# zhangyp15/MonoFlex

Measured on AMD Instinct MI355X. Metric: images/sec at 1280x384, DLA-34+DCNv2 forward+decode, higher is better.
Workload: dtype bf16; 1 GPU; DLA-34+DCNv2+9 heads+edge fusion forward + NMS/top-K/3D decode, batch 8 per GPU, 1280x384, bf16 (BASELINE.json configs[1]); batch_per_gpu=8, launch=hipGraph, parallelism=replicas x1 (no collective on the inference path), sub_batch_streams=1, detections_last_step=400, h2d_excluded=True, d2h_excluded=True

## Files before the change

### include/monoflex_hip.h

```cpp
#ifndef MONOFLEX_HIP_H
#define MONOFLEX_HIP_H

#include <stddef.h>
#include <stdint.h>

#ifdef __cplusplus
extern "C" {
#endif

#define MFX_ABI_VERSION 3

enum { MFX_F32 = 0, MFX_BF16 = 1, MFX_F16 = 2 ,
       MFX_F16X2 = 3  };
enum { MFX_ACT_NONE = 0, MFX_ACT_RELU = 1, MFX_ACT_LEAKY = 2 , MFX_ACT_DCN_OFFMASK = 3  };
enum { MFX_OK = 0, MFX_ERR_ARG = -1, MFX_ERR_UNSUPPORTED = -2, MFX_ERR_LAUNCH = -3, MFX_ERR_WORKSPACE = -4 };

int mfx_abi_version(void);
const char* mfx_last_error(void);
int mfx_set_option(const char* name, int value);
int mfx_reset_options(void);
int mfx_commit_options(void);
long mfx_get_counter(const char* name);

int mfx_f16x2_range_check(int reset);


size_t mfx_dcn_v2_workspace_bytes(int B, int C, int H, int W, int Cout, int kh, int kw,
                                  int stride_h, int stride_w, int pad_h, int pad_w, int dil_h, int dil_w,
                                  int backward);
size_t mfx_dcn_v2_workspace_bytes_g(int B, int C, int H, int W, int Cout, int kh, int kw,
                                    int stride_h, int stride_w, int pad_h, int pad_w, int dil_h, int dil_w,
                                    int deformable_group, int backward);

int mfx_dcn_v2_forward(const float* input, const float* weight, const float* bias,
                       const float* offset, const float* mask, float* output,
                       int B, int C, int H, int W, int Cout, int kh, int kw,
                       int stride_h, int stride_w, int pad_h, int pad_w, int dil_h, int dil_w,
                       int deformable_group, void* workspace, size_t workspace_bytes, void* stream);

int mfx_dcn_v2_backward(const float* input, const float* weight, const float* bias,
                        const float* offset, const float* mask, const float* grad_output,
                        float* grad_input, float* grad_offset, float* grad_mask,
                        float* grad_weight, float* grad_bias,
                        int B, int C, int H, int W, int Cout, int kh, int kw,
                        int stride_h, int stride_w, int pad_h, int pad_w, int dil_h, int dil_w,
                        int deformable_group, void* workspace, size_t workspace_bytes, void* stream);

int mfx_dcn_v2_psroi_pooling_forward(const float* input, const float* bbox, const float* trans, float* output, float* output_count,
                                     int B, int C, int H, int W, int N, int trans_rois, int trans_channels,
                                     int no_trans, float spatial_scale, int output_dim, int group_size, int pooled_size, int part_size,
                                     int sample_per_part, float trans_std, void* stream);

int mfx_dcn_v2_psroi_pooling_backward(const float* out_grad, const float* input, const float* bbox, const float* trans, const float* top_count,
                                      float* grad_input, float* grad_trans,
                                      int B, int C, int H, int W, int N, int trans_rois, int trans_channels,
                                      int no_trans, float spatial_scale, int output_dim, int group_size, int pooled_size, int part_size,
                                      int sample_per_part, float trans_std, void* stream);


#define MFX_MAX_SEG 9

typedef struct {
    const void* x;
    const void* w;
    const void* w_frag;
    const float* scale;
    const float* shift;
    const void* res;
    void* y;
    const int32_t* rowmap;
    int32_t B, H, W;
    int32_t x_pixstride;
    int32_t Ck;
    int32_t kh, kw, stride, pad_h, pad_w, dil_w;
    int32_t Ho, Wo;
    int32_t M;
    int32_t Cout;
    int32_t Cout_pad;
    int32_t K_pad;
    int32_t ldy, ldres;
    int32_t act;
    int32_t dtype, out_dtype;
    void* workspace;
    int64_t workspace_bytes;
    float* stats;
    int stats_ncopy;
    int* stats_done;
    const void* w_frag_pair;
} mfx_conv_desc;
int mfx_conv2d_nhwc(const mfx_conv_desc* d, void* stream);

typedef struct {
    const void* src[MFX_MAX_SEG];
    int32_t stride[MFX_MAX_SEG];
    int32_t off[MFX_MAX_SEG];
    int32_t nseg, Cseg;
    const void* w; const float* scale; const float* shift; const void* res; void* y;
    int32_t M, Cout, Cout_pad, K_pad, ldy, ldres, act, dtype;
} mfx_cat_desc;
int mfx_cat_conv1x1_nhwc(const mfx_cat_desc* d, void* stream);

typedef struct {
    const void* x; const float* offmask; const void* w; const float* scale; const float* shift; void* y;
    const void* w_frag;
    int32_t B, H, W, C;
    int32_t kh, kw, stride, pad, dil;
    int32_t Ho, Wo, Cout, Cout_pad, K_pad, ldy, act, dtype;
    const void* w_frag_f16;
    void* workspace;
    int64_t workspace_bytes;
    const void* off_w_frag_f16;
    const float* off_shift;
    float* offmask_out;
    int32_t nonsquare, stride_w, pad_w, dil_w;
    const void* w_pair_f16;
} mfx_dcn_desc;
int mfx_dcn_nhwc(const mfx_dcn_desc* d, void* stream);
int mfx_dcn_fuses_offset_conv(const mfx_dcn_desc* d);
int mfx_dcn_module_group(const mfx_conv_desc* off, const mfx_dcn_desc* dcn, int n, void* stream);

int mfx_dcn_sample_nhwc(const void* P, const float* offmask, const float* scale, const float* shift, void* y,
                        int B, int H, int W, int N, int ldy, int act, int dtype, void* stream);
int mfx_project_nhwc(const void* x, const void* w, void* y, int M, int K, int N, int ldx, int ldy, int dtype, void* stream);

int mfx_stem_conv7x7_nchw(const float* images, const void* w, const float* scale, const float* shift, void* y,
                          int B, int H, int W, int Cout, int K_pad, int act, int dtype, void* stream);

int mfx_f1_fused(const float* images, const void* w_stem, const float* sc_stem, const float* sh_stem,
                 const void* w_l0, const float* sc_l0, const float* sh_l0, const void* w_l1, const float* sc_l1, const float* sh_l1,
                 void* y, int B, int H, int W, int stem_kpad , int dtype, void* stream);

int mfx_maxpool2x2_nhwc(const void* x, void* y, int B, int H, int W, int C, int dtype, void* stream);

int mfx_upsample_add_nhwc(const void* x, const float* w, const void* skip, void* y,
                          int B, int H, int W, int C, int f, int dtype, void* stream);

int mfx_nchw_to_nhwc(const float* x, void* y, int B, int C, int H, int W, int ldy, int dtype, void* stream);
int mfx_nhwc_to_nchw(const void* x, float* y, int B, int C, int H, int W, int ldx, int dtype, void* stream);
int mfx_pack_image_nhwc4(const float* x, void* y, int B, int H, int W, int pad_h, int pad_w_left, int pad_w_right,
                         int dtype, void* stream);

typedef struct {
    const void* x;
    const void* w1;
    const float* scale1; const float* shift1;
    const void* w2;
    const float* bias2;
    float* out;
    float* planar;
    int32_t B, H, W, nbranch, K_pad, ld_out, dtype, planar_c;
    int32_t ch_off[16]; int32_t c_out[16];
    float w2_scale[16];
    const void* w1_32; const void* w2_32;
} mfx_heads_desc;
int mfx_heads_fused(const mfx_heads_desc* d, void* stream);
int mfx_heads_fused_act(const mfx_heads_desc* d, int act, void* stream);

int mfx_edge_scatter_add(float* out, int ld_out, int ch_off, int C, const float* v, int ldv,
                         const int32_t* edge_xy, const int32_t* edge_len, int B, int L, int H, int W,
                         float* planar , void* stream);

typedef struct {
    const void* x;
    const int32_t* edge_xy;
    const void* w_trunk;
    const float* scale_trunk; const float* shift_trunk;
    const void* w_conv;
    const float* scale_conv; const float* shift_conv;
    const void* w_out;
    const float* bias_out;
    float* out;
    int32_t B, H, W, C, L, head_conv, ksize, relu , dtype;
} mfx_edge_chain_desc;
int mfx_edge_chain(const mfx_edge_chain_desc* d, void* stream);
int mfx_edge_chain_act(const mfx_edge_chain_desc* d, int act, void* stream);
int mfx_edge_chain_applies(const mfx_edge_chain_desc* d);
int mfx_edge_chain_ks(const mfx_edge_chain_desc* d, int act, void* stream);
int mfx_edge_chain_ks_applies(const mfx_edge_chain_desc* d);

size_t mfx_decode_topk_workspace_bytes(int ncls, int B, int K);
int mfx_decode_topk(const float* hmap, long b_stride, long c_stride, long p_stride, int ncls, int B, int H, int W, int K,
                    float* scores, int32_t* index, void* workspace, size_t workspace_bytes, void* stream);

int mfx_decode_boxes(const float* hmap, int ld, int reg_off, const float* scores, const int32_t* index,
                     int ncls, int B, int H, int W, int K, const float* calib, const int32_t* pad,
                     const int32_t* img_size, float threshold, float* det, float* topk, int32_t* valid,
                     void* stream);
enum { MFX_DEPTH_SOFT = 0, MFX_DEPTH_HARD = 1, MFX_DEPTH_MEAN = 2, MFX_DEPTH_DIRECT = 3, MFX_DEPTH_KEYPOINTS_AVG = 4,
       MFX_DEPTH_KEYPOINTS_CENTER = 5, MFX_DEPTH_KEYPOINTS_02 = 6, MFX_DEPTH_KEYPOINTS_13 = 7 };
int mfx_decode_boxes_mode(const float* hmap, int ld, int reg_off, const float* scores, const int32_t* index,
                          int ncls, int B, int H, int W, int K, const float* calib, const int32_t* pad,
                          const int32_t* img_size, float threshold, int depth_mode, float* det, float* topk, int32_t* valid,
                          void* stream);
typedef struct mfx_decode_cfg {
    float dim_mean[9], dim_std[9];
    float depth_ref[2], depth_range[2];
    float down_ratio, eps;
    int depth_decode;
    int dim_exp, dim_use_std;
    int uncertainty_as_conf;
    int output_depth;
} mfx_decode_cfg;
int mfx_decode_boxes_cfg(const float* hmap, int ld, int reg_off, const float* scores, const int32_t* index,
                         int ncls, int B, int H, int W, int K, const float* calib, const int32_t* pad,
                         const int32_t* img_size, float threshold, const mfx_decode_cfg* cfg, float* det, float* topk, int32_t* valid,
                         float* unc, void* stream);
typedef struct mfx_head_layout {
    int ch[9];
    int reg_width;
} mfx_head_layout;
int mfx_decode_boxes_heads(const float* hmap, int ld, int reg_off, const float* scores, const int32_t* index,
                           int ncls, int B, int H, int W, int K, const float* calib, const int32_t* pad,
                           const int32_t* img_size, float threshold, const mfx_decode_cfg* cfg, const mfx_head_layout* heads,
                           float* det, float* topk, int32_t* valid, float* unc, void* stream);
enum { MFX_DEPTH_ORACLE = 8 };
int mfx_decode_boxes_multi(const float* hmap, int ld, int reg_off, const float* scores, const int32_t* index,
                           int ncls, int B, int H, int W, int K, const float* calib, const int32_t* pad,
                           const int32_t* img_size, float threshold, const mfx_decode_cfg* cfg, const mfx_head_layout* heads,
                           uint32_t modes, const float* gt_rows, int M, float* det, float* topk, int32_t* valid, float* unc,
                           int32_t* oracle_choice, void* stream);


int mfx_conv_wgrad_nhwc(const void* x, const void* dy, float* dw, int B, int H, int W, int x_pixstride, int Ck,
                        int kh, int kw, int stride, int pad_h, int pad_w, int Ho, int Wo, int Cout, int ldy,
                        int dtype, void* stream);
int mfx_conv_wgrad_nhwc_dil(const void* x, const void* dy, float* dw, int B, int H, int W, int x_pixstride, int Ck,
                            int kh, int kw, int stride, int pad_h, int pad_w, int dil_w, int Ho, int Wo, int Cout, int ldy,
                            int dtype, void* stream);
int mfx_conv_wgrad_oihw(const void* x, const void* dy, float* dw, int B, int H, int W, int x_pixstride, int Ck,
                        int kh, int kw, int stride, int pad_h, int pad_w, int Ho, int Wo, int Cout, int ldy,
                        int Cout_real, int Cin_real, int dtype, void* workspace, size_t workspace_bytes, void* stream);
int mfx_stem_wgrad_bf16(const void* xp, const void* dy, float* dw, int B, int H, int W, int Hp, int Wp, void* workspace,
                        size_t workspace_bytes, void* stream);
int mfx_stem_wgrad_16(const void* xp, const void* dy, float* dw, int B, int H, int W, int Hp, int Wp, int dtype, void* workspace,
                      size_t workspace_bytes, void* stream);
int mfx_pack_conv_weight(const float* w_oihw, int Cout, int Cin, int kh, int kw, int mode, void* packed, void* frag,
                         int rows_pad, int K_pad, int ck, int dtype, void* stream);
int mfx_pack_chunk_elems(void);
typedef struct mfx_pack_desc {
    const float* w;
    void* packed;
    void* frag;
    int Cout, Cin, kh, kw, mode, rows_pad, K_pad, ck;
} mfx_pack_desc;
int mfx_pack_conv_weights_batched(const mfx_pack_desc* descs_dev, const long long* prefix_dev, int n, long long total_chunks,
                                  int dtype, void* stream);
typedef struct mfx_adamw_desc {
    void* p;
    const void* g;
    void* m;
    void* v;
    float* step;
    long long numel;
    int group;
    int pad_;
} mfx_adamw_desc;
typedef struct mfx_adamw_group {
    const float* lr;
    float beta1, beta2, eps, weight_decay;
} mfx_adamw_group;
int mfx_adamw_chunk_elems(void);
int mfx_adamw_multi(const mfx_adamw_desc* descs_dev, const long long* prefix_dev, int n, long long total_chunks,
                    const mfx_adamw_group* groups_dev, const float* found_inf, void* stream);
#define MFX_OPTIM_ADAMW 0
#define MFX_OPTIM_ADAM_L2 1
int mfx_optim_multi(const mfx_adamw_desc* descs_dev, const long long* prefix_dev, int n, long long total_chunks,
                    const mfx_adamw_group* groups_dev, int rule, const float* grad_coef, const float* found_inf, void* stream);
#define MFX_OPTIM_ADAM_TRUE_WD 2
int mfx_optim_multi_sched(const mfx_adamw_desc* descs_dev, const long long* prefix_dev, int n, long long total_chunks,
                          const mfx_adamw_group* groups_dev, const float* const* beta1_dev, int rule, const float* grad_coef, const float* found_inf,
                          void* stream);
size_t mfx_grad_norm_workspace_bytes(long long total_chunks);
// ... 226 lines not shown
```

### monoflex_amd/csrc/dcn_lds.hip

```cpp
#include "../../include/monoflex_hip.h"
#include "err.h"
#include "internal.h"
#include "igemm.h"
#include "dcn_sample_math.h"

namespace mfx {

struct DcnLGeom { int B, H, W, C, tiles_x, tiles_y, nslice, fsteps_pair, fsteps_far, cpt_far; };
struct DcnLOffArgs { const u32x4* wfm; const float* shift; float* om_out; };

typedef _Float16 lh2_t __attribute__((ext_vector_type(2)));
typedef _Float16 lh8_t __attribute__((ext_vector_type(8)));

__device__ __forceinline__ uint32_t l_bf2_to_h2(uint32_t d) {
    return __builtin_bit_cast(uint32_t, __builtin_amdgcn_cvt_pkrtz(__uint_as_float(d << 16), __uint_as_float(d & 0xffff0000u)));
}
template <typename TX> __device__ __forceinline__ u32x4 l_to_h8(const u32x4& v);
template <> __device__ __forceinline__ u32x4 l_to_h8<bf16_t>(const u32x4& v) { return u32x4{l_bf2_to_h2(v.x), l_bf2_to_h2(v.y), l_bf2_to_h2(v.z), l_bf2_to_h2(v.w)}; }
template <> __device__ __forceinline__ u32x4 l_to_h8<half_t>(const u32x4& v) { return v; }

#ifdef MFX_PROBES
__device__ unsigned long long mfx_dcn_lds_probe[1024 * 4 * 16];
#define LPROBE(k) do { if (lane == 0 && blockIdx.x < 1024) mfx_dcn_lds_probe[(blockIdx.x * 4 + wv) * 16 + (k)] = (unsigned long long)clock64(); } while (0)
#else
#define LPROBE(k) do { } while (0)
#endif

template <int R, int TR> struct DcnLSmem {
    static constexpr int PW = 16 + 2 * (R + 1), PH = TR + 2 * (R + 1);
    static constexpr int PB = 48;
    static constexpr int patch_bytes = PW * PH * PB;
    static constexpr int NPIX = TR * 16;
    static constexpr int NG = 9 * NPIX;
    static constexpr int GW_OFF = patch_bytes;
    static constexpr int GB_OFF = GW_OFF + (NG + 64) * 8;
    static constexpr int bytes = GB_OFF + (NG + 64) * 4;
    static constexpr int ZBYTES = (TR + 2) * 18 * 144;
    static constexpr int TBUF_OFF = (ZBYTES + 4 * 2304 <= patch_bytes) ? ZBYTES : GB_OFF;
    static_assert(ZBYTES <= patch_bytes && (TBUF_OFF != GB_OFF || 4 * 2304 <= (NG + 64) * 4), "offset-conv scratch fits");
};

template <int R, int TR, typename TX, bool OF>
__global__ __launch_bounds__(256, TR == 8 ? 3 : 2) void dcn_lds_kernel(const TX* __restrict__ x, const float* __restrict__ om, const u32x4* __restrict__ wpair,
                                                        const u32x4* __restrict__ wfar, DcnLGeom g, EpiArgs ep, DcnLOffArgs oa) {
    using SM = DcnLSmem<R, TR>;
    constexpr int PW = SM::PW, PH = SM::PH, PB = SM::PB, FM = TR / 4, FN = 4, NPIX = SM::NPIX;
    constexpr int OWN = 4 / FM;
    constexpr int TPT = (9 + OWN - 1) / OWN;
    constexpr int ROWB = PW * PB;
    extern __shared__ __attribute__((aligned(16))) char smem[];
    const int tid = threadIdx.x, lane = tid & 63;
    const int wv = __builtin_amdgcn_readfirstlane(tid >> 6);
    const int xl = lane & 15, kq = lane >> 4;

    LPROBE(0);
    int tile = xcd_remap(blockIdx.x, gridDim.x);
    const int tx = tile % g.tiles_x; tile /= g.tiles_x;
    const int ty = tile % g.tiles_y, b = tile / g.tiles_y;
    const int ty0 = ty * TR, tx0 = tx * 16;
    const int py0 = ty0 - (R + 1), px0 = tx0 - (R + 1);
    const TX* xb = x + (size_t)b * g.H * g.W * g.C;
    const char* xbb = reinterpret_cast<const char*>(xb);

    const int oi = kq % FM, tg = kq / FM;
    const int opix = (wv * FM + oi) * 16 + xl;
    const int yo = ty0 + wv * FM + oi, xo = tx0 + xl;
    const bool own_ok = yo < g.H && xo < g.W;

    constexpr int PU = PW * PH * 2 / 256;
    static_assert(PW * PH * 2 % 256 == 0, "patch chunks per thread");
    uint32_t poff[PU]; uint32_t pin = 0;
#pragma unroll
    for (int u = 0; u < PU; ++u) {
        const int idx = u * 256 + tid, p = idx >> 1, col = idx & 1;
        const int ry = p / PW, rx = p - ry * PW;
        const int gy = py0 + ry, gx = px0 + rx;
        const bool in = gy >= 0 && gy < g.H && gx >= 0 && gx < g.W;
        const int cy = min(max(gy, 0), g.H - 1), cx = min(max(gx, 0), g.W - 1);
        poff[u] = (uint32_t)((cy * g.W + cx) * g.C + col * 8) * 2u;
        pin |= in ? (1u << u) : 0u;
    }
    const int pw_addr = (tid >> 1) * PB + (tid & 1) * 16;
    u32x4 pr[PU];
    auto patch_fetch = [&](int sl) {
#pragma unroll
        for (int u = 0; u < PU; ++u) pr[u] = *reinterpret_cast<const u32x4*>(xbb + poff[u] + (uint32_t)sl * 32u);
    };
    auto patch_write = [&]() {
#pragma unroll
        for (int u = 0; u < PU; ++u) {
            const u32x4 v = (pin >> u) & 1u ? pr[u] : u32x4{0u, 0u, 0u, 0u};
            *reinterpret_cast<u32x4*>(smem + pw_addr + u * (128 * PB)) = l_to_h8<TX>(v);
        }
    };

    float odh[TPT], odw[TPT], omk[TPT];
    const int tap0 = TPT * tg;
    if constexpr (!OF) {
        const float* r = om + ((size_t)(b * g.H + min(yo, g.H - 1)) * g.W + min(xo, g.W - 1)) * dcns::kRow;
#pragma unroll
        for (int tt = 0; tt < TPT; ++tt) {
            const int tap = min(tap0 + tt, 8);
            odh[tt] = r[dcns::off_h(tap)]; odw[tt] = r[dcns::off_w(tap)]; omk[tt] = r[dcns::mask_at(tap)];
        }
        patch_fetch(0);
    } else {
        constexpr int ZW = 18, ZPS = 144, TLD = 36;
        float* tbuf = reinterpret_cast<float*>(smem + SM::TBUF_OFF) + wv * (16 * TLD);
        {
            constexpr int ZN = (TR + 2) * ZW * 8, ZU = (ZN + 255) / 256;
#pragma unroll
            for (int base = 0; base < ZN; base += 256 * ZU) {
                u32x4 zr[ZU];
#pragma unroll
                for (int u = 0; u < ZU; ++u) {
                    int idx = base + u * 256 + tid;
                    if (base + u * 256 + 256 > ZN) idx = idx < ZN ? idx : ZN - 1;
                    const int p = idx >> 3, col = idx & 7;
                    const int ry = p / ZW, rx = p - ry * ZW;
                    const int gy = ty0 - 1 + ry, gx = tx0 - 1 + rx;
                    const bool in = gy >= 0 && gy < g.H && gx >= 0 && gx < g.W;
                    const int cy = min(max(gy, 0), g.H - 1), cx = min(max(gx, 0), g.W - 1);
                    const u32x4 v = *reinterpret_cast<const u32x4*>(xb + (uint32_t)((cy * g.W + cx) * g.C + col * 8));
                    zr[u] = in ? v : u32x4{0u, 0u, 0u, 0u};
                }
#pragma unroll
                for (int u = 0; u < ZU; ++u) {
                    const int idx = base + u * 256 + tid;
                    if (base + u * 256 + 256 <= ZN || idx < ZN) *reinterpret_cast<u32x4*>(smem + (idx >> 3) * ZPS + ((idx & 7) << 4)) = l_to_h8<TX>(zr[u]);
                }
            }
        }
        f32x4 ao[FM][2];
#pragma unroll
        for (int i = 0; i < FM; ++i) { ao[i][0] = f32x4{0.f, 0.f, 0.f, 0.f}; ao[i][1] = f32x4{0.f, 0.f, 0.f, 0.f}; }
        constexpr int OR = 6;
        u32x4 ow[OR][2];
        const u32x4* owl = oa.wfm + lane;
#pragma unroll
        for (int u = 0; u < OR - 1; ++u) { ow[u][0] = owl[(0 * 18 + u) * 64]; ow[u][1] = owl[(1 * 18 + u) * 64]; }
        patch_fetch(0);
        __syncthreads();
        LPROBE(1);
#pragma unroll
        for (int s_ = 0; s_ < 18; ++s_) {
            if (s_ + OR - 1 < 18) { ow[(s_ + OR - 1) % OR][0] = owl[(0 * 18 + s_ + OR - 1) * 64]; ow[(s_ + OR - 1) % OR][1] = owl[(1 * 18 + s_ + OR - 1) * 64]; }
            const int tap = s_ >> 1, th = tap / 3, tw = tap - th * 3;
            const char* ap = smem + ((wv * FM + th) * ZW + xl + tw) * ZPS + ((s_ & 1) * 32 + kq * 8) * 2;
#pragma unroll
            for (int i = 0; i < FM; ++i) {
                const u32x4 af = *reinterpret_cast<const u32x4*>(ap + i * ZW * ZPS);
#pragma unroll
                for (int j = 0; j < 2; ++j)
                    ao[i][j] = __builtin_amdgcn_mfma_f32_16x16x32_f16(__builtin_bit_cast(lh8_t, af), __builtin_bit_cast(lh8_t, ow[s_ % OR][j]), ao[i][j], 0, 0, 0);
            }
        }
        LPROBE(2);
        const float b0 = oa.shift[xl], b1 = oa.shift[16 + xl];
#pragma unroll
        for (int i = 0; i < FM; ++i) {
#pragma unroll
            for (int r = 0; r < 4; ++r) {
                float v0 = ao[i][0][r] + b0, v1 = ao[i][1][r] + b1;
                if (xl >= 2) v1 = 1.f / (1.f + __expf(-v1));
                tbuf[(kq * 4 + r) * TLD + xl] = v0;
                tbuf[(kq * 4 + r) * TLD + 16 + xl] = (xl < 11) ? v1 : 0.f;
            }
            __builtin_amdgcn_wave_barrier();
            if (oi == i) {
#pragma unroll
                for (int tt = 0; tt < TPT; ++tt) {
                    const int tap = min(tap0 + tt, 8);
                    const float2 d2 = *reinterpret_cast<const float2*>(tbuf + xl * TLD + dcns::off_h(tap));
                    odh[tt] = d2.x; odw[tt] = d2.y; omk[tt] = tbuf[xl * TLD + dcns::mask_at(tap)];
                }
                if (oa.om_out && own_ok && tg == 0) {
                    float* o = oa.om_out + ((size_t)(b * g.H + yo) * g.W + xo) * dcns::kRow;
#pragma unroll
                    for (int q = 0; q < 32; q += 4) *reinterpret_cast<f32x4*>(o + q) = *reinterpret_cast<const f32x4*>(tbuf + xl * TLD + q);
                }
            }
            __builtin_amdgcn_wave_barrier();
        }
    }

    LPROBE(3);
    uint32_t gb[TPT];
    unsigned long long farm[TPT];
#pragma unroll
    for (int tt = 0; tt < TPT; ++tt) {
        const int tap = tap0 + tt;
        const bool has = tap < 9;
        const float mk = (own_ok && has) ? omk[tt] : 0.f;
        const dcns::Tap t = dcns::tap3x3(tap);
        const float h = dcns::pos3x3(yo, t.th, odh[tt]), w = dcns::pos3x3(xo, t.tw, odw[tt]);
        const dcns::Sample s = dcns::sample(h, w);
        const float lh = s.lh, lw = s.lw, hh = s.hh, hw_ = s.hw;
        const int h0 = s.h0, w0 = s.w0;
        const float m_ = dcns::inside(h, w, g.H, g.W) ? mk : 0.f;
        uint32_t wa = __builtin_bit_cast(uint32_t, __builtin_amdgcn_cvt_pkrtz(hh * hw_ * m_, hh * lw * m_));
        uint32_t wb_ = __builtin_bit_cast(uint32_t, __builtin_amdgcn_cvt_pkrtz(lh * hw_ * m_, lh * lw * m_));
        const int ry = h0 - py0, rx = w0 - px0;
        const bool in_patch = ry >= 0 && ry + 1 < PH && rx >= 0 && rx + 1 < PW;
        const bool live = m_ != 0.f;
        const bool far = live && !in_patch;
        uint32_t base = in_patch ? (uint32_t)((ry * PW + rx) * PB) : 0u;
        if (far) { base = 0x80000000u | (uint32_t)(h0 + 32) | ((uint32_t)(w0 + 32) << 16); wa |= 0x80008000u; wb_ |= 0x80008000u; }
        if (!live) { wa = 0u; wb_ = 0u; }
        if (has) *reinterpret_cast<uint2*>(smem + SM::GW_OFF + (tap * NPIX + opix) * 8) = uint2{wa, wb_};
        gb[tt] = base;
        farm[tt] = __builtin_amdgcn_ballot_w64(far);
    }
    if (tid < 4) *reinterpret_cast<uint2*>(smem + SM::GW_OFF + (SM::NG + 16 * tid) * 8) = uint2{0u, 0u};
    LPROBE(4);
    __syncthreads();
    LPROBE(5);
#pragma unroll
    for (int tt = 0; tt < TPT; ++tt)
        if (tt + TPT * tg < 9) *reinterpret_cast<uint32_t*>(smem + SM::GB_OFF + ((tt + TPT * tg) * NPIX + opix) * 4) = gb[tt];
    if (tid < 4) *reinterpret_cast<uint32_t*>(smem + SM::GB_OFF + (SM::NG + 16 * tid) * 4) = 0u;
    patch_write();
    __syncthreads();
    LPROBE(6);

    f32x4 acc[FM][FN];
#pragma unroll
    for (int i = 0; i < FM; ++i)
#pragma unroll
        for (int j = 0; j < FN; ++j) acc[i][j] = f32x4{0.f, 0.f, 0.f, 0.f};

    const int gent = (kq >> 1) * NPIX + wv * (FM * 16) + xl;
    const int gw_a = SM::GW_OFF + gent * 8, gb_a = SM::GB_OFF + gent * 4;
    const int gw_z = (kq >> 1) ? SM::GW_OFF + (SM::NG - 8 * NPIX) * 8 : gw_a;
    const int gb_z = (kq >> 1) ? SM::GB_OFF + (SM::NG - 8 * NPIX) * 4 : gb_a;
    const int ccol = (kq & 1) * 16;
    const u32x4* wpl = wpair + lane;
    auto wfetch = [&](int step, u32x4 (&wf)[FN]) {
#pragma unroll
        for (int j = 0; j < FN; ++j) wf[j] = wpl[((size_t)j * g.fsteps_pair + step) * 64];
    };
    u32x4 wq[2][FN];
    wfetch(0, wq[0]);

    constexpr int NF = 5 * FM;
    for (int sl = 0; sl < g.nslice; ++sl) {
        if (sl + 1 < g.nslice) patch_fetch(sl + 1);
        uint2 gwv[3]; uint32_t gbv[3];
        u32x4 cv[2][4];
        auto geo_read = [&](int f, int slot) {
            const int j = f / FM, i = f % FM;
            if (j < 4) {
                gwv[slot] = *reinterpret_cast<const uint2*>(smem + gw_a + (2 * NPIX * j + 16 * i) * 8);
                gbv[slot] = *reinterpret_cast<const uint32_t*>(smem + gb_a + (2 * NPIX * j + 16 * i) * 4);
            } else {
                gwv[slot] = *reinterpret_cast<const uint2*>(smem + gw_z + (8 * NPIX + 16 * i) * 8);
                gbv[slot] = *reinterpret_cast<const uint32_t*>(smem + gb_z + (8 * NPIX + 16 * i) * 4);
            }
        };
        auto corner_read = [&](int slot_g, int slot_c) {
            const int base = max((int)gbv[slot_g], 0) + ccol;
            cv[slot_c][0] = *reinterpret_cast<const u32x4*>(smem + base);
            cv[slot_c][1] = *reinterpret_cast<const u32x4*>(smem + base + PB);
            cv[slot_c][2] = *reinterpret_cast<const u32x4*>(smem + base + ROWB);
            cv[slot_c][3] = *reinterpret_cast<const u32x4*>(smem + base + ROWB + PB);
        };
        auto blend = [&](int slot_g, int slot_c) -> u32x4 {
            typedef short ls2_t __attribute__((ext_vector_type(2)));
            const ls2_t z2 = {0, 0};
            const lh2_t wa = __builtin_bit_cast(lh2_t, __builtin_elementwise_max(__builtin_bit_cast(ls2_t, gwv[slot_g].x), z2));
            const lh2_t wb_ = __builtin_bit_cast(lh2_t, __builtin_elementwise_max(__builtin_bit_cast(ls2_t, gwv[slot_g].y), z2));
            const lh2_t w0 = {wa[0], wa[0]}, w1 = {wa[1], wa[1]}, w2 = {wb_[0], wb_[0]}, w3 = {wb_[1], wb_[1]};
            u32x4 o;
#pragma unroll
            for (int d = 0; d < 4; ++d) {
                const uint32_t a0 = cv[slot_c][0][d], a1 = cv[slot_c][1][d], a2 = cv[slot_c][2][d], a3 = cv[slot_c][3][d];
                const lh2_t r = __builtin_bit_cast(lh2_t, a0) * w0 + __builtin_bit_cast(lh2_t, a1) * w1 +
                                __builtin_bit_cast(lh2_t, a2) * w2 + __builtin_bit_cast(lh2_t, a3) * w3;
                o[d] = __builtin_bit_cast(uint32_t, r);
            }
            return o;
        };
        geo_read(0, 0);
        geo_read(1, 1);
        corner_read(0, 0);
#pragma unroll
        for (int f = 0; f < NF; ++f) {
            const int j = f / FM, i = f % FM;
            if (i == 0) {
                const int nstep = sl * 5 + j + 1;
                wfetch(min(nstep, g.fsteps_pair - 1), wq[(j + 1) & 1]);
            }
            if (f + 2 < NF) geo_read(f + 2, (f + 2) % 3);
            if (f + 1 < NF) corner_read((f + 1) % 3, (f + 1) & 1);
            __builtin_amdgcn_sched_barrier(0);
            const u32x4 af = blend(f % 3, f & 1);
#pragma unroll
            for (int n = 0; n < FN; ++n)
                acc[i][n] = __builtin_amdgcn_mfma_f32_16x16x32_f16(__builtin_bit_cast(lh8_t, af), __builtin_bit_cast(lh8_t, wq[j & 1][n]), acc[i][n], 0, 0, 0);
            __builtin_amdgcn_sched_barrier(0);
        }
#pragma unroll
        for (int n = 0; n < FN; ++n) wq[0][n] = wq[1][n];
        if (sl < 4) LPROBE(7 + 2 * sl);
        if (sl + 1 < g.nslice) {
            __syncthreads();
            patch_write();
            __syncthreads();
        }
        if (sl < 3) LPROBE(8 + 2 * sl);
    }

    __syncthreads();
    float sc[FN], sh[FN];
#pragma unroll
    for (int j = 0; j < FN; ++j) {
        sc[j] = ep.scale ? ep.scale[j * 16 + xl] : 1.f;
        sh[j] = ep.shift ? ep.shift[j * 16 + xl] : 0.f;
    }
    {
        unsigned long long any = 0;
#pragma unroll
        for (int tt = 0; tt < TPT; ++tt) any |= farm[tt];
        if (any) {
            const u32x4* wfl = wfar + lane;
            for (int tap = 0; tap < 9; ++tap) {
                const int ftt = tap % TPT, ftg = tap / TPT;
                unsigned long long fm_ = 0;
#pragma unroll
                for (int t = 0; t < TPT; ++t) fm_ = (t == ftt) ? farm[t] : fm_;
                fm_ >>= (ftg * FM) * 16;
                if (!(fm_ & (FM == 4 ? ~0ull : 0xffffffffull))) continue;
#pragma unroll
                for (int i = 0; i < FM; ++i) {
                    if (!((fm_ >> (16 * i)) & 0xffffull)) continue;
                    const int ent = tap * NPIX + (wv * FM + i) * 16 + xl;
                    const uint2 gw = *reinterpret_cast<const uint2*>(smem + SM::GW_OFF + ent * 8);
                    const uint32_t gbase = *reinterpret_cast<const uint32_t*>(smem + SM::GB_OFF + ent * 4);
                    const bool isfar = (gbase >> 31) != 0u;
                    const int h0 = (int)(gbase & 0xffffu) - 32, w0 = (int)((gbase >> 16) & 0x7fffu) - 32;
                    const uint32_t wau = isfar ? (gw.x & 0x7fff7fffu) : 0u, wbu = isfar ? (gw.y & 0x7fff7fffu) : 0u;
                    const lh2_t wa = __builtin_bit_cast(lh2_t, wau), wb_ = __builtin_bit_cast(lh2_t, wbu);
                    const lh2_t w0_ = {wa[0], wa[0]}, w1_ = {wa[1], wa[1]}, w2_ = {wb_[0], wb_[0]}, w3_ = {wb_[1], wb_[1]};
                    for (int ks = 0; ks < g.cpt_far; ++ks) {
                        u32x4 v[4];
#pragma unroll
                        for (int q = 0; q < 4; ++q) {
                            const int hc = h0 + (q >> 1), wc = w0 + (q & 1);
                            const bool ok = isfar && hc >= 0 && hc < g.H && wc >= 0 && wc < g.W;
                            v[q] = u32x4{0u, 0u, 0u, 0u};
                            if (ok) v[q] = l_to_h8<TX>(*reinterpret_cast<const u32x4*>(xb + ((size_t)hc * g.W + wc) * g.C + ks * 32 + kq * 8));
                        }
                        u32x4 af;
#pragma unroll
                        for (int d = 0; d < 4; ++d) {
                            const uint32_t a0 = v[0][d], a1 = v[1][d], a2 = v[2][d], a3 = v[3][d];
                            const lh2_t r = __builtin_bit_cast(lh2_t, a0) * w0_ + __builtin_bit_cast(lh2_t, a1) * w1_ +
                                            __builtin_bit_cast(lh2_t, a2) * w2_ + __builtin_bit_cast(lh2_t, a3) * w3_;
                            af[d] = __builtin_bit_cast(uint32_t, r);
                        }
#pragma unroll
                        for (int n = 0; n < FN; ++n) {
                            const u32x4 wf = wfl[((size_t)n * g.fsteps_far + tap * g.cpt_far + ks) * 64];
                            acc[i][n] = __builtin_amdgcn_mfma_f32_16x16x32_f16(__builtin_bit_cast(lh8_t, af), __builtin_bit_cast(lh8_t, wf), acc[i][n], 0, 0, 0);
                        }
                    }
                }
            }
        }
    }

    LPROBE(14);
    constexpr int LDS_ = FN * 16 + 4;
    constexpr int GPR = FN * 16 / 8;
    float* stage = reinterpret_cast<float*>(smem) + wv * (16 * LDS_);
    TX* y = reinterpret_cast<TX*>(ep.y);
#pragma unroll
    for (int i = 0; i < FM; ++i) {
#pragma unroll
        for (int j = 0; j < FN; ++j)
#pragma unroll
            for (int r = 0; r < 4; ++r) stage[(kq * 4 + r) * LDS_ + j * 16 + xl] = acc[i][j][r] * sc[j] + sh[j];
        __builtin_amdgcn_wave_barrier();
        const int yg = ty0 + wv * FM + i;
        for (int it = lane; it < 16 * GPR; it += 64) {
            const int px = it / GPR, ng = it - px * GPR;
            const int gx = tx0 + px, gn = ng * 8;
            if (yg < g.H && gx < g.W && gn < ep.Cout) {
                float v[8];
#pragma unroll
                for (int e = 0; e < 8; e += 4) {
                    const f32x4 t = *reinterpret_cast<const f32x4*>(stage + px * LDS_ + ng * 8 + e);
                    v[e] = t[0]; v[e + 1] = t[1]; v[e + 2] = t[2]; v[e + 3] = t[3];
                }
                apply_act_chunk<8>(v, ep.act, gn);
                *reinterpret_cast<u32x4*>(y + ((size_t)(b * g.H + yg) * g.W + gx) * ep.ldy + gn) = ElemTraits<TX>::pack(v);
            }
        }
        __builtin_amdgcn_wave_barrier();
    }
    LPROBE(15);
}

#ifdef MFX_PROBES
}
extern "C" int mfx_dcn_lds_probe_read(unsigned long long* host, int n) {
    return hipMemcpyFromSymbol(host, HIP_SYMBOL(mfx::mfx_dcn_lds_probe), sizeof(unsigned long long) * (size_t)n) == hipSuccess ? 0 : -1;
}
namespace mfx {
#endif

template <int R>
__global__ __launch_bounds__(256, 2) void dcn_lds_split_kernel(const float* __restrict__ x, const float* __restrict__ om, const u32x4* __restrict__ wpair,
                                                              const u32x4* __restrict__ wfar, size_t pair_lo, size_t far_lo, DcnLGeom g, EpiArgs ep) {
    constexpr int TR = 8, FM = 2, FN = 4, NPIX = TR * 16, OWN = 2, TPT = 5;
    constexpr int PW = 16 + 2 * (R + 1), PH = TR + 2 * (R + 1), PB = 80, ROWB = PW * PB;
    constexpr int patch_bytes = PW * PH * PB, NG = 9 * NPIX, GT_OFF = patch_bytes;
    extern __shared__ __attribute__((aligned(16))) char smem[];
    const int tid = threadIdx.x, lane = tid & 63;
    const int wv = __builtin_amdgcn_readfirstlane(tid >> 6);
    const int xl = lane & 15, kq = lane >> 4;

    int tile = xcd_remap(blockIdx.x, gridDim.x);
    const int tx = tile % g.tiles_x; tile /= g.tiles_x;
    const int ty = tile % g.tiles_y, b = tile / g.tiles_y;
    const int ty0 = ty * TR, tx0 = tx * 16;
    const int py0 = ty0 - (R + 1), px0 = tx0 - (R + 1);
    const float* xb = x + (size_t)b * g.H * g.W * g.C;
    const char* xbb = reinterpret_cast<const char*>(xb);

    const int oi = kq % FM, tg = kq / FM;
    const int opix = (wv * FM + oi) * 16 + xl;
    const int yo = ty0 + wv * FM + oi, xo = tx0 + xl;
    const bool own_ok = yo < g.H && xo < g.W;

    constexpr int PU = PW * PH * 4 / 256;
    static_assert(PW * PH * 4 % 256 == 0, "patch chunks per thread");
    auto patch_load = [&](int sl) {
#pragma unroll
        for (int half = 0; half < 2; ++half) {
            u32x4 pr[PU / 2];
#pragma unroll
            for (int u = 0; u < PU / 2; ++u) {
                const int idx = (half * (PU / 2) + u) * 256 + tid, p = idx >> 2, col = idx & 3;
                const int ry = p / PW, rx = p - ry * PW;
                const int gy = py0 + ry, gx = px0 + rx;
                const bool in = gy >= 0 && gy < g.H && gx >= 0 && gx < g.W;
                const int cy = min(max(gy, 0), g.H - 1), cx = min(max(gx, 0), g.W - 1);
                const u32x4 v = *reinterpret_cast<const u32x4*>(xbb + (uint32_t)(((cy * g.W + cx) * g.C + sl * 16 + col * 4) * 4));
                pr[u] = in ? v : u32x4{0u, 0u, 0u, 0u};
            }
#pragma unroll
            for (int u = 0; u < PU / 2; ++u) {
                const int idx = (half * (PU / 2) + u) * 256 + tid;
                *reinterpret_cast<u32x4*>(smem + (idx >> 2) * PB + (idx & 3) * 16) = pr[u];
            }
        }
    };

    {
        const float* r = om + ((size_t)(b * g.H + min(yo, g.H - 1)) * g.W + min(xo, g.W - 1)) * dcns::kRow;
        const int tap0 = TPT * tg;
        float odh[TPT], odw[TPT], omk[TPT];
#pragma unroll
        for (int tt = 0; tt < TPT; ++tt) {
            const int tap = min(tap0 + tt, 8);
            odh[tt] = r[dcns::off_h(tap)]; odw[tt] = r[dcns::off_w(tap)]; omk[tt] = r[dcns::mask_at(tap)];
        }
        patch_load(0);
#pragma unroll
        for (int tt = 0; tt < TPT; ++tt) {
            const int tap = tap0 + tt;
            const bool has = tap < 9;
            const float mk = (own_ok && has) ? omk[tt] : 0.f;
            const dcns::Tap t = dcns::tap3x3(tap);
            const float h = dcns::pos3x3(yo, t.th, odh[tt]), w = dcns::pos3x3(xo, t.tw, odw[tt]);
            const dcns::Sample s = dcns::sample(h, w);
            const int h0 = s.h0, w0 = s.w0;
            const float m_ = dcns::inside(h, w, g.H, g.W) ? mk : 0.f;
            const int ry = h0 - py0, rx = w0 - px0;
            const bool in_patch = ry >= 0 && ry + 1 < PH && rx >= 0 && rx + 1 < PW;
            const bool far = m_ != 0.f && !in_patch;
            uint32_t base = in_patch ? (uint32_t)((ry * PW + rx) * PB) : 0u;
            if (far) base = 0x80000000u | (uint32_t)(h0 + 32) | ((uint32_t)(w0 + 32) << 16);
            if (has) *reinterpret_cast<f32x4*>(smem + GT_OFF + (tap * NPIX + opix) * 16) = f32x4{s.lh, s.lw, far ? -m_ : m_, __uint_as_float(base)};
        }
        if (tid < FM) *reinterpret_cast<f32x4*>(smem + GT_OFF + (NG + 16 * tid) * 16) = f32x4{0.f, 0.f, 0.f, 0.f};
    }
    unsigned long long farm[TPT];
    __syncthreads();
    {
#pragma unroll
        for (int tt = 0; tt < TPT; ++tt) {
            const int tap = TPT * tg + tt;
            const float mk = tap < 9 ? reinterpret_cast<const float*>(smem + GT_OFF + (min(tap, 8) * NPIX + opix) * 16)[2] : 0.f;
            farm[tt] = __builtin_amdgcn_ballot_w64(mk < 0.f);
        }
    }

    f32x4 acc[FM][FN];
#pragma unroll
    for (int i = 0; i < FM; ++i)
#pragma unroll
        for (int j = 0; j < FN; ++j) acc[i][j] = f32x4{0.f, 0.f, 0.f, 0.f};

    const int gent = (kq >> 1) * NPIX + wv * (FM * 16) + xl;
    const int gt_a = GT_OFF + gent * 16;
    const int gt_z = (kq >> 1) ? GT_OFF + (NG - 8 * NPIX) * 16 : gt_a;
    const int ccol = (kq & 1) * 32;
    const u32x4* wph = wpair + lane;
    const u32x4* wpl = wpair + pair_lo + lane;
    auto wfetch = [&](int step, u32x4 (&wh)[FN], u32x4 (&wl)[FN]) {
#pragma unroll
        for (int j = 0; j < FN; ++j) { wh[j] = wph[((size_t)j * g.fsteps_pair + step) * 64]; wl[j] = wpl[((size_t)j * g.fsteps_pair + step) * 64]; }
    };
    u32x4 wqh[2][FN], wql[2][FN];
    wfetch(0, wqh[0], wql[0]);

    constexpr int NF = 5 * FM;
    for (int sl = 0; sl < g.nslice; ++sl) {
        f32x4 gv[3];
        u32x4 cv[2][4][2];
        auto geo_read = [&](int f, int slot) {
            const int j = f / FM, i = f % FM;
            gv[slot] = j < 4 ? *reinterpret_cast<const f32x4*>(smem + gt_a + (2 * NPIX * j + 16 * i) * 16)
                             : *reinterpret_cast<const f32x4*>(smem + gt_z + (8 * NPIX + 16 * i) * 16);
        };
        auto corner_read = [&](int slot_g, int slot_c) {
            const int base = max((int)__float_as_uint(gv[slot_g][3]), 0) + ccol;
#pragma unroll
            for (int q = 0; q < 4; ++q) {
                cv[slot_c][q][0] = *reinterpret_cast<const u32x4*>(smem + base + (q >> 1) * ROWB + (q & 1) * PB);
                cv[slot_c][q][1] = *reinterpret_cast<const u32x4*>(smem + base + (q >> 1) * ROWB + (q & 1) * PB + 16);
            }
        };
        auto blend = [&](int slot_g, int slot_c, u32x4& ah, u32x4& al) {
            const float lh = gv[slot_g][0], lw = gv[slot_g][1], m_ = fmaxf(gv[slot_g][2], 0.f);
            const float hh = 1.f - lh, hw_ = 1.f - lw;
            const float w0 = hh * hw_ * m_, w1 = hh * lw * m_, w2 = lh * hw_ * m_, w3 = lh * lw * m_;
            u32x4 sp[2];
#pragma unroll
            for (int c2 = 0; c2 < 2; ++c2) {
                float o[4];
#pragma unroll
                for (int e = 0; e < 4; e += 2) {
                    f32x2 t = f32x2{__uint_as_float(cv[slot_c][0][c2][e]), __uint_as_float(cv[slot_c][0][c2][e + 1])} * w0;
                    t = __builtin_elementwise_fma(f32x2{__uint_as_float(cv[slot_c][1][c2][e]), __uint_as_float(cv[slot_c][1][c2][e + 1])}, f32x2{w1, w1}, t);
                    t = __builtin_elementwise_fma(f32x2{__uint_as_float(cv[slot_c][2][c2][e]), __uint_as_float(cv[slot_c][2][c2][e + 1])}, f32x2{w2, w2}, t);
                    t = __builtin_elementwise_fma(f32x2{__uint_as_float(cv[slot_c][3][c2][e]), __uint_as_float(cv[slot_c][3][c2][e + 1])}, f32x2{w3, w3}, t);
                    o[e] = t[0]; o[e + 1] = t[1];
                }
                sp[c2] = lds_operand<f32s_t>(ElemTraits<float>::pack(o));
            }
            ah = u32x4{sp[0].x, sp[0].y, sp[1].x, sp[1].y};
            al = u32x4{sp[0].z, sp[0].w, sp[1].z, sp[1].w};
        };
        geo_read(0, 0);
        geo_read(1, 1);
        corner_read(0, 0);
#pragma unroll
        for (int f = 0; f < NF; ++f) {
            const int j = f / FM, i = f % FM;
            if (i == 0) wfetch(min(sl * 5 + j + 1, g.fsteps_pair - 1), wqh[(j + 1) & 1], wql[(j + 1) & 1]);
            if (f + 2 < NF) geo_read(f + 2, (f + 2) % 3);
            if (f + 1 < NF) corner_read((f + 1) % 3, (f + 1) & 1);
            __builtin_amdgcn_sched_barrier(0);
            u32x4 ah, al;
            blend(f % 3, f & 1, ah, al);
#pragma unroll
            for (int n = 0; n < FN; ++n) {
                acc[i][n] = __builtin_amdgcn_mfma_f32_16x16x32_f16(__builtin_bit_cast(lh8_t, ah), __builtin_bit_cast(lh8_t, wqh[j & 1][n]), acc[i][n], 0, 0, 0);
                acc[i][n] = __builtin_amdgcn_mfma_f32_16x16x32_f16(__builtin_bit_cast(lh8_t, ah), __builtin_bit_cast(lh8_t, wql[j & 1][n]), acc[i][n], 0, 0, 0);
                acc[i][n] = __builtin_amdgcn_mfma_f32_16x16x32_f16(__builtin_bit_cast(lh8_t, al), __builtin_bit_cast(lh8_t, wqh[j & 1][n]), acc[i][n], 0, 0, 0);
            }
            __builtin_amdgcn_sched_barrier(0);
        }
#pragma unroll
        for (int n = 0; n < FN; ++n) { wqh[0][n] = wqh[1][n]; wql[0][n] = wql[1][n]; }
        __syncthreads();
        if (sl + 1 < g.nslice) {
            patch_load(sl + 1);
            __syncthreads();
        }
    }

    float sc[FN], sh[FN];
#pragma unroll
    for (int j = 0; j < FN; ++j) {
        sc[j] = ep.scale ? ep.scale[j * 16 + xl] : 1.f;
        sh[j] = ep.shift ? ep.shift[j * 16 + xl] : 0.f;
    }
    {
        unsigned long long any = 0;
#pragma unroll
        for (int tt = 0; tt < TPT; ++tt) any |= farm[tt];
        if (any) {
            const u32x4* wfh = wfar + lane;
            const u32x4* wfl = wfar + far_lo + lane;
            for (int tap = 0; tap < 9; ++tap) {
                const int ftt = tap % TPT, ftg = tap / TPT;
                unsigned long long fm_ = 0;
#pragma unroll
                for (int t = 0; t < TPT; ++t) fm_ = (t == ftt) ? farm[t] : fm_;
                fm_ >>= (ftg * FM) * 16;
                if (!(fm_ & 0xffffffffull)) continue;
#pragma unroll
                for (int i = 0; i < FM; ++i) {
                    if (!((fm_ >> (16 * i)) & 0xffffull)) continue;
                    const f32x4 ge = *reinterpret_cast<const f32x4*>(smem + GT_OFF + (tap * NPIX + (wv * FM + i) * 16 + xl) * 16);
                    const uint32_t gbase = __float_as_uint(ge[3]);
                    const bool isfar = ge[2] < 0.f;
                    const int h0 = (int)(gbase & 0xffffu) - 32, w0 = (int)((gbase >> 16) & 0x7fffu) - 32;
                    const float m_ = isfar ? -ge[2] : 0.f, lh = ge[0], lw = ge[1], hh = 1.f - lh, hw_ = 1.f - lw;
                    const float wq4[4] = {hh * hw_ * m_, hh * lw * m_, lh * hw_ * m_, lh * lw * m_};
                    for (int ks = 0; ks < g.cpt_far; ++ks) {
                        float o[8];
#pragma unroll
                        for (int e = 0; e < 8; ++e) o[e] = 0.f;
#pragma unroll
                        for (int q = 0; q < 4; ++q) {
                            const int hc = h0 + (q >> 1), wc = w0 + (q & 1);
                            const bool ok = isfar && hc >= 0 && hc < g.H && wc >= 0 && wc < g.W;
                            if (ok) {
                                const float* p = xb + ((size_t)hc * g.W + wc) * g.C + ks * 32 + kq * 8;
                                const f32x4 a = *reinterpret_cast<const f32x4*>(p), c4 = *reinterpret_cast<const f32x4*>(p + 4);
#pragma unroll
                                for (int e = 0; e < 4; ++e) { o[e] = fmaf(wq4[q], a[e], o[e]); o[4 + e] = fmaf(wq4[q], c4[e], o[4 + e]); }
                            }
                        }
                        const float o0[4] = {o[0], o[1], o[2], o[3]}, o1[4] = {o[4], o[5], o[6], o[7]};
                        const u32x4 s0 = lds_operand<f32s_t>(ElemTraits<float>::pack(o0)), s1 = lds_operand<f32s_t>(ElemTraits<float>::pack(o1));
                        const u32x4 ah = {s0.x, s0.y, s1.x, s1.y}, al = {s0.z, s0.w, s1.z, s1.w};
#pragma unroll
                        for (int n = 0; n < FN; ++n) {
                            const size_t wi = ((size_t)n * g.fsteps_far + tap * g.cpt_far + ks) * 64;
                            const u32x4 wh = wfh[wi], wl = wfl[wi];
                            acc[i][n] = __builtin_amdgcn_mfma_f32_16x16x32_f16(__builtin_bit_cast(lh8_t, ah), __builtin_bit_cast(lh8_t, wh), acc[i][n], 0, 0, 0);
                            acc[i][n] = __builtin_amdgcn_mfma_f32_16x16x32_f16(__builtin_bit_cast(lh8_t, ah), __builtin_bit_cast(lh8_t, wl), acc[i][n], 0, 0, 0);
                            acc[i][n] = __builtin_amdgcn_mfma_f32_16x16x32_f16(__builtin_bit_cast(lh8_t, al), __builtin_bit_cast(lh8_t, wh), acc[i][n], 0, 0, 0);
                        }
                    }
                }
            }
        }
    }

    constexpr int LDS_ = FN * 16 + 4;
    float* stage = reinterpret_cast<float*>(smem) + wv * (16 * LDS_);
    float* y = reinterpret_cast<float*>(ep.y);
#pragma unroll
    for (int i = 0; i < FM; ++i) {
#pragma unroll
        for (int j = 0; j < FN; ++j)
#pragma unroll
            for (int r = 0; r < 4; ++r) stage[(kq * 4 + r) * LDS_ + j * 16 + xl] = acc[i][j][r] * sc[j] + sh[j];
        __builtin_amdgcn_wave_barrier();
        const int yg = ty0 + wv * FM + i;
        for (int it = lane; it < 16 * 16; it += 64) {
            const int px = it >> 4, ng = it & 15;
            const int gx = tx0 + px, gn = ng * 4;
            if (yg < g.H && gx < g.W && gn < ep.Cout) {
                float v[4];
                const f32x4 t = *reinterpret_cast<const f32x4*>(stage + px * LDS_ + gn);
                v[0] = t[0]; v[1] = t[1]; v[2] = t[2]; v[3] = t[3];
                apply_act_chunk<4>(v, ep.act, gn);
                *reinterpret_cast<f32x4*>(y + ((size_t)(b * g.H + yg) * g.W + gx) * ep.ldy + gn) = f32x4{v[0], v[1], v[2], v[3]};
            }
        }
        __builtin_amdgcn_wave_barrier();
    }
}


static bool dcn_lds_shape_ok(const mfx_dcn_desc* d) {
    if (!d->w_pair_f16 || !d->w_frag_f16 || (d->dtype != MFX_BF16 && d->dtype != MFX_F16)) return false;
    if (d->kh != 3 || d->kw != 3 || d->stride != 1 || d->pad != 1 || d->dil != 1 || d->Ho != d->H || d->Wo != d->W || d->nonsquare) return false;
    if (d->C % 32 != 0 || d->K_pad != 9 * d->C || d->Cout_pad != 64) return false;
    return true;
}
static bool dcn_lds_auto(const mfx_dcn_desc* d) {
    if (!g_opt_dcn_lds || !dcn_lds_shape_ok(d)) return false;
    if (g_opt_dcn_lds >= 2) return true;
    return d->C == 64 && (long)d->B * d->H * d->W >= 65536;
}
bool dcn_lds_takes_16bit(const mfx_dcn_desc* d) { return dcn_lds_auto(d); }
bool dcn_lds_fuses_offset_conv(const mfx_dcn_desc* d) {
    return g_opt_dcn_fuse_off && d->off_w_frag_f16 && d->off_shift && d->C == 64 && dcn_lds_auto(d);
}

template <int TR, typename TX, bool OF> static int launch_dcn_lds(const mfx_dcn_desc* d, hipStream_t st) {
    constexpr int R = 7;
    DcnLGeom g;
    g.B = d->B; g.H = d->H; g.W = d->W; g.C = d->C;
    g.tiles_x = (d->W + 15) / 16; g.tiles_y = (d->H + TR - 1) / TR;
    g.nslice = d->C / 16; g.fsteps_pair = g.nslice * 5; g.fsteps_far = d->K_pad / 32; g.cpt_far = d->C / 32;
    EpiArgs ep;
    ep.scale = d->scale; ep.shift = d->shift; ep.res = nullptr; ep.y = d->y; ep.ldy = d->ldy; ep.ldres = 0;
    ep.Cout = d->Cout; ep.act = d->act; ep.K_pad = d->K_pad; ep.nk = 0; ep.tiles_n = 1;
    const int tiles = d->B * g.tiles_y * g.tiles_x;
    constexpr int smem = DcnLSmem<R, TR>::bytes;
    static bool attr_done = false;
    if (!attr_done) {
        MFX_HIP_CHECK(hipFuncSetAttribute(reinterpret_cast<const void*>(&dcn_lds_kernel<R, TR, TX, OF>), hipFuncAttributeMaxDynamicSharedMemorySize, smem));
        attr_done = true;
    }
    DcnLOffArgs oa;
    oa.wfm = reinterpret_cast<const u32x4*>(d->off_w_frag_f16); oa.shift = d->off_shift; oa.om_out = d->offmask_out;
    if (!OF && !d->offmask) return mfx_fail(MFX_ERR_ARG, "dcn: offmask is NULL and this kernel does not compute the offsets itself");
    hipLaunchKernelGGL((dcn_lds_kernel<R, TR, TX, OF>), dim3(tiles), dim3(256), smem, st, reinterpret_cast<const TX*>(d->x), d->offmask,
                       reinterpret_cast<const u32x4*>(d->w_pair_f16), reinterpret_cast<const u32x4*>(d->w_frag_f16), g, ep, oa);
    MFX_HIP_CHECK(hipGetLastError());
    return MFX_OK;
}

static int launch_dcn_lds_split(const mfx_dcn_desc* d, hipStream_t st) {
    constexpr int R = 7, TR = 8;
    DcnLGeom g;
    g.B = d->B; g.H = d->H; g.W = d->W; g.C = d->C;
    g.tiles_x = (d->W + 15) / 16; g.tiles_y = (d->H + TR - 1) / TR;
    g.nslice = d->C / 16; g.fsteps_pair = g.nslice * 5; g.fsteps_far = d->K_pad / 32; g.cpt_far = d->C / 32;
    EpiArgs ep;
    ep.scale = d->scale; ep.shift = d->shift; ep.res = nullptr; ep.y = d->y; ep.ldy = d->ldy; ep.ldres = 0;
    ep.Cout = d->Cout; ep.act = d->act; ep.K_pad = d->K_pad; ep.nk = 0; ep.tiles_n = 1;
    constexpr int smem = (16 + 2 * (R + 1)) * (TR + 2 * (R + 1)) * 80 + (9 * TR * 16 + 32) * 16;
    static bool attr_done = false;
    if (!attr_done) {
        MFX_HIP_CHECK(hipFuncSetAttribute(reinterpret_cast<const void*>(&dcn_lds_split_kernel<R>), hipFuncAttributeMaxDynamicSharedMemorySize, smem));
        attr_done = true;
    }
    if (!d->offmask) return mfx_fail(MFX_ERR_ARG, "dcn: offmask is NULL (the split-precision LDS kernel does not compute the offsets itself)");
    const size_t pair_lo = (size_t)(d->Cout_pad / 16) * g.fsteps_pair * 64, far_lo = (size_t)(d->Cout_pad / 16) * g.fsteps_far * 64;
    hipLaunchKernelGGL((dcn_lds_split_kernel<R>), dim3(d->B * g.tiles_y * g.tiles_x), dim3(256), smem, st, reinterpret_cast<const float*>(d->x), d->offmask,
                       reinterpret_cast<const u32x4*>(d->w_pair_f16), reinterpret_cast<const u32x4*>(d->w_frag_f16), pair_lo, far_lo, g, ep);
    MFX_HIP_CHECK(hipGetLastError());
    return MFX_OK;
}

int try_dcn_lds(const mfx_dcn_desc* d, hipStream_t st) {
    if (d->dtype == MFX_F16X2) {
        if (!g_opt_dcn_lds || !d->w_pair_f16 || !d->w_frag_f16 || d->nonsquare) return 0;
        if (d->kh != 3 || d->kw != 3 || d->stride != 1 || d->pad != 1 || d->dil != 1 || d->Ho != d->H || d->Wo != d->W) return 0;
        if (d->C % 32 != 0 || d->K_pad != 9 * d->C || d->Cout_pad != 64 || d->Cout % 4 != 0) return 0;
        if (g_opt_dcn_lds < 2 && !(d->C == 64 && (long)d->B * d->H * d->W >= 65536)) return 0;
        const int rc = launch_dcn_lds_split(d, st);
        return rc == MFX_OK ? 1 : rc;
    }
    if (!dcn_lds_auto(d)) return 0;
    const bool of = dcn_lds_fuses_offset_conv(d);
    int rc;
    if (g_opt_dcn_lds_rows == 16) {
        if (d->dtype == MFX_F16) rc = of ? launch_dcn_lds<16, half_t, true>(d, st) : launch_dcn_lds<16, half_t, false>(d, st);
        else rc = of ? launch_dcn_lds<16, bf16_t, true>(d, st) : launch_dcn_lds<16, bf16_t, false>(d, st);
    } else {
        if (d->dtype == MFX_F16) rc = of ? launch_dcn_lds<8, half_t, true>(d, st) : launch_dcn_lds<8, half_t, false>(d, st);
        else rc = of ? launch_dcn_lds<8, bf16_t, true>(d, st) : launch_dcn_lds<8, bf16_t, false>(d, st);
    }
    return rc == MFX_OK ? 1 : rc;
}

}

MFX_RANGE_FLAG_ACCESSOR(dcn_lds)
```

### monoflex_amd/csrc/misc_kernels.hip

```cpp
#include "../../include/monoflex_hip.h"
#include "common.h"
#include "err.h"

namespace mfx {

static inline int cdiv_i(long a, long b) { return (int)((a + b - 1) / b); }

template <typename T>
__global__ void maxpool2x2_kernel(const T* x, T* y, int B, int H, int W, int C) {
    constexpr int E = ElemTraits<T>::ELEMS;
    const int Ho = H / 2, Wo = W / 2, CG = C / E;
    const long total = (long)B * Ho * Wo * CG;
    for (long i = blockIdx.x * (long)blockDim.x + threadIdx.x; i < total; i += (long)gridDim.x * blockDim.x) {
        const int cg = (int)(i % CG);
        long p = i / CG;
        const int ow = (int)(p % Wo); p /= Wo;
        const int oh = (int)(p % Ho);
        const int b = (int)(p / Ho);
        const T* src = x + ((size_t)(b * H + oh * 2) * W + ow * 2) * C + cg * E;
        float a[E], t[E];
        ElemTraits<T>::unpack(*reinterpret_cast<const u32x4*>(src), a);
        ElemTraits<T>::unpack(*reinterpret_cast<const u32x4*>(src + C), t);
#pragma unroll
        for (int e = 0; e < E; ++e) a[e] = fmaxf(a[e], t[e]);
        ElemTraits<T>::unpack(*reinterpret_cast<const u32x4*>(src + (size_t)W * C), t);
#pragma unroll
        for (int e = 0; e < E; ++e) a[e] = fmaxf(a[e], t[e]);
        ElemTraits<T>::unpack(*reinterpret_cast<const u32x4*>(src + (size_t)W * C + C), t);
#pragma unroll
        for (int e = 0; e < E; ++e) a[e] = fmaxf(a[e], t[e]);
        *reinterpret_cast<u32x4*>(y + ((size_t)(b * Ho + oh) * Wo + ow) * C + cg * E) = ElemTraits<T>::pack(a);
    }
}

template <typename T, int F = 0>
__global__ void upsample_add_kernel(const T* __restrict__ x, const float* __restrict__ w, const T* __restrict__ skip, T* __restrict__ y,
                                    int B, int H, int W, int C, int f_rt) {
    constexpr int E = ElemTraits<T>::ELEMS;
    const int f = F > 0 ? F : f_rt;
    const int Ho = H * f, Wo = W * f, CG = C / E, p_ = f / 2, k = 2 * f;
    const long total = (long)B * Ho * Wo * CG;
    for (long i = blockIdx.x * (long)blockDim.x + threadIdx.x; i < total; i += (long)gridDim.x * blockDim.x) {
        const int cg = (int)(i % CG);
        long p = i / CG;
        const int ow = (int)(p % Wo); p /= Wo;
        const int oh = (int)(p % Ho);
        const int b = (int)(p / Ho);
        float acc[E];
#pragma unroll
        for (int e = 0; e < E; ++e) acc[e] = 0.f;
        const int th = oh + p_, tw = ow + p_;
        const size_t o = ((size_t)(b * Ho + oh) * Wo + ow) * C + cg * E;
        u32x4 sv = {0u, 0u, 0u, 0u};
        if (skip) sv = *reinterpret_cast<const u32x4*>(skip + o);
        u32x4 xv[2][2]; f32x4 wv[2][2][E / 4];
#pragma unroll
        for (int a = 0; a < 2; ++a) {
            const int kh = th % f + a * f, dh = th - kh, ih = dh / f;
            const bool vh = dh >= 0 && ih < H;
            const int ihc = min(max(ih, 0), H - 1);
#pragma unroll
            for (int c2 = 0; c2 < 2; ++c2) {
                const int kw = tw % f + c2 * f, dw = tw - kw, iw = dw / f;
                const bool vw = dw >= 0 && iw < W;
                const int iwc = min(max(iw, 0), W - 1);
                const u32x4 v = *reinterpret_cast<const u32x4*>(x + ((size_t)(b * H + ihc) * W + iwc) * C + cg * E);
                xv[a][c2] = (vh && vw) ? v : u32x4{0u, 0u, 0u, 0u};
                const float* wp = w + (size_t)(kh * k + kw) * C + cg * E;
#pragma unroll
                for (int e = 0; e < E; e += 4) wv[a][c2][e / 4] = *reinterpret_cast<const f32x4*>(wp + e);
            }
        }
#pragma unroll
        for (int a = 1; a >= 0; --a)
#pragma unroll
            for (int c2 = 1; c2 >= 0; --c2) {
                float v[E];
                ElemTraits<T>::unpack(xv[a][c2], v);
#pragma unroll
                for (int e = 0; e < E; e += 4) {
                    const f32x4 w4 = wv[a][c2][e / 4];
                    acc[e] += v[e] * w4[0]; acc[e + 1] += v[e + 1] * w4[1]; acc[e + 2] += v[e + 2] * w4[2]; acc[e + 3] += v[e + 3] * w4[3];
                }
            }
        if (skip) {
            float s[E];
            ElemTraits<T>::unpack(sv, s);
#pragma unroll
            for (int e = 0; e < E; ++e) acc[e] += s[e];
        }
        *reinterpret_cast<u32x4*>(y + o) = ElemTraits<T>::pack(acc);
    }
}

template <typename T>
__global__ void nchw_to_nhwc_kernel(const float* x, T* y, int C, int HW, int ldy) {
    __shared__ float tile[32][33];
    const int b = blockIdx.z, p0 = blockIdx.x * 32, c0 = blockIdx.y * 32;
    const int tx = threadIdx.x, ty = threadIdx.y;
#pragma unroll
    for (int j = 0; j < 32; j += 8) {
        const int c = c0 + ty + j, p = p0 + tx;
        tile[ty + j][tx] = (c < C && p < HW) ? x[((size_t)b * C + c) * HW + p] : 0.f;
    }
    __syncthreads();
#pragma unroll
    for (int j = 0; j < 32; j += 8) {
        const int p = p0 + ty + j, c = c0 + tx;
        if (p < HW && c < ldy) ElemTraits<T>::store(y + ((size_t)b * HW + p) * ldy + c, c < C ? tile[tx][ty + j] : 0.f);
    }
}
template <typename T>
__global__ void nhwc_to_nchw_kernel(const T* x, float* y, int C, int HW, int ldx) {
    __shared__ float tile[32][33];
    const int b = blockIdx.z, p0 = blockIdx.x * 32, c0 = blockIdx.y * 32;
    const int tx = threadIdx.x, ty = threadIdx.y;
#pragma unroll
    for (int j = 0; j < 32; j += 8) {
        const int p = p0 + ty + j, c = c0 + tx;
        tile[ty + j][tx] = (p < HW && c < C) ? ElemTraits<T>::load(x + ((size_t)b * HW + p) * ldx + c) : 0.f;
    }
    __syncthreads();
#pragma unroll
    for (int j = 0; j < 32; j += 8) {
        const int c = c0 + ty + j, p = p0 + tx;
        if (c < C && p < HW) y[((size_t)b * C + c) * HW + p] = tile[tx][ty + j];
    }
}

template <typename T>
__global__ void pack_image_kernel(const float* x, T* y, int B, int H, int W, int ph, int pwl, int pwr) {
    const int Hp = H + 2 * ph, Wp = W + pwl + pwr;
    const long total = (long)B * Hp * Wp;
    for (long i = blockIdx.x * (long)blockDim.x + threadIdx.x; i < total; i += (long)gridDim.x * blockDim.x) {
        const int wp = (int)(i % Wp);
        long p = i / Wp;
        const int hp = (int)(p % Hp);
        const int b = (int)(p / Hp);
        const int h = hp - ph, w = wp - pwl;
        float v[4] = {0.f, 0.f, 0.f, 0.f};
        if (h >= 0 && h < H && w >= 0 && w < W) {
            const size_t o = ((size_t)b * 3 * H + h) * W + w;
            v[0] = x[o]; v[1] = x[o + (size_t)H * W]; v[2] = x[o + 2 * (size_t)H * W];
        }
        T* d = y + (size_t)i * 4;
#pragma unroll
        for (int e = 0; e < 4; ++e) ElemTraits<T>::store(d + e, v[e]);
    }
}

__global__ void edge_scatter_add_kernel(float* out, int ld_out, int ch_off, int C, const float* v, int ldv,
                                        const int* edge_xy, const int* edge_len, int B, int L, int H, int W, float* planar) {
    const int total = B * L * C;
    for (int i = blockIdx.x * blockDim.x + threadIdx.x; i < total; i += gridDim.x * blockDim.x) {
        const int c = i % C, j = (i / C) % L, b = i / (C * L);
        if (j >= edge_len[b]) continue;
        const int x = edge_xy[(b * L + j) * 2], y = edge_xy[(b * L + j) * 2 + 1];
        const float add = v[(size_t)(b * L + j) * ldv + c];
        out[((size_t)(b * H + y) * W + x) * ld_out + ch_off + c] += add;
        if (planar) planar[((size_t)b * C + c) * H * W + y * W + x] += add;
    }
}

}
using namespace mfx;

#define MFX_GRID(total, threads) dim3((unsigned)(cdiv_i((total), (threads)) < 16384 ? cdiv_i((total), (threads)) : 16384))

extern "C" int mfx_maxpool2x2_nhwc(const void* x, void* y, int B, int H, int W, int C, int dtype, void* stream) {
    if (!x || !y) return mfx_fail(MFX_ERR_ARG, "maxpool: null pointer");
    const int E = dtype == MFX_F32 ? 4 : 8;
    if (C % E != 0 || (H & 1) || (W & 1)) return mfx_fail(MFX_ERR_ARG, "maxpool: C must be a multiple of 16 bytes, H/W even");
    const long total = (long)B * (H / 2) * (W / 2) * (C / E);
    if (total == 0) return MFX_OK;
    hipStream_t st = reinterpret_cast<hipStream_t>(stream);
    if (dtype == MFX_F32) hipLaunchKernelGGL(maxpool2x2_kernel<float>, MFX_GRID(total, 256), dim3(256), 0, st, (const float*)x, (float*)y, B, H, W, C);
    else if (dtype == MFX_F16) hipLaunchKernelGGL(maxpool2x2_kernel<half_t>, MFX_GRID(total, 256), dim3(256), 0, st, (const half_t*)x, (half_t*)y, B, H, W, C);
    else hipLaunchKernelGGL(maxpool2x2_kernel<bf16_t>, MFX_GRID(total, 256), dim3(256), 0, st, (const bf16_t*)x, (bf16_t*)y, B, H, W, C);
    MFX_HIP_CHECK(hipGetLastError());
    return MFX_OK;
}

extern "C" int mfx_upsample_add_nhwc(const void* x, const float* w, const void* skip, void* y,
                                     int B, int H, int W, int C, int f, int dtype, void* stream) {
    if (!x || !w || !y) return mfx_fail(MFX_ERR_ARG, "upsample: null pointer");
    const int E = dtype == MFX_F32 ? 4 : 8;
    if (C % E != 0 || f < 1) return mfx_fail(MFX_ERR_ARG, "upsample: bad C or f");
    const long total = (long)B * H * f * W * f * (C / E);
    if (total == 0) return MFX_OK;
    hipStream_t st = reinterpret_cast<hipStream_t>(stream);
#define MFX_UP_LAUNCH(T, F_)                                                                                                                   \
    hipLaunchKernelGGL((upsample_add_kernel<T, F_>), MFX_GRID(total, 256), dim3(256), 0, st, (const T*)x, w, (const T*)skip, (T*)y, B, H, W, C, f)
#define MFX_UP_DISPATCH(T)                                                                                                                     \
    do { if (f == 2) MFX_UP_LAUNCH(T, 2); else if (f == 4) MFX_UP_LAUNCH(T, 4); else MFX_UP_LAUNCH(T, 0); } while (0)
    if (dtype == MFX_F32) MFX_UP_DISPATCH(float);
    else if (dtype == MFX_F16) MFX_UP_DISPATCH(half_t);
    else MFX_UP_DISPATCH(bf16_t);
#undef MFX_UP_DISPATCH
#undef MFX_UP_LAUNCH
    MFX_HIP_CHECK(hipGetLastError());
    return MFX_OK;
}

extern "C" int mfx_nchw_to_nhwc(const float* x, void* y, int B, int C, int H, int W, int ldy, int dtype, void* stream) {
    if (!x || !y || ldy < C) return mfx_fail(MFX_ERR_ARG, "nchw_to_nhwc: bad arguments");
    if (B * C * H * W == 0) return MFX_OK;
    hipStream_t st = reinterpret_cast<hipStream_t>(stream);
    dim3 grid(cdiv_i((long)H * W, 32), cdiv_i(ldy, 32), B), block(32, 8);
    if (dtype == MFX_F32) hipLaunchKernelGGL(nchw_to_nhwc_kernel<float>, grid, block, 0, st, x, (float*)y, C, H * W, ldy);
    else if (dtype == MFX_F16) hipLaunchKernelGGL(nchw_to_nhwc_kernel<half_t>, grid, block, 0, st, x, (half_t*)y, C, H * W, ldy);
    else hipLaunchKernelGGL(nchw_to_nhwc_kernel<bf16_t>, grid, block, 0, st, x, (bf16_t*)y, C, H * W, ldy);
    MFX_HIP_CHECK(hipGetLastError());
    return MFX_OK;
}

extern "C" int mfx_nhwc_to_nchw(const void* x, float* y, int B, int C, int H, int W, int ldx, int dtype, void* stream) {
    if (!x || !y || ldx < C) return mfx_fail(MFX_ERR_ARG, "nhwc_to_nchw: bad arguments");
    if (B * C * H * W == 0) return MFX_OK;
    hipStream_t st = reinterpret_cast<hipStream_t>(stream);
    dim3 grid(cdiv_i((long)H * W, 32), cdiv_i(C, 32), B), block(32, 8);
    if (dtype == MFX_F32) hipLaunchKernelGGL(nhwc_to_nchw_kernel<float>, grid, block, 0, st, (const float*)x, y, C, H * W, ldx);
    else if (dtype == MFX_F16) hipLaunchKernelGGL(nhwc_to_nchw_kernel<half_t>, grid, block, 0, st, (const half_t*)x, y, C, H * W, ldx);
    else hipLaunchKernelGGL(nhwc_to_nchw_kernel<bf16_t>, grid, block, 0, st, (const bf16_t*)x, y, C, H * W, ldx);
    MFX_HIP_CHECK(hipGetLastError());
    return MFX_OK;
}

extern "C" int mfx_pack_image_nhwc4(const float* x, void* y, int B, int H, int W, int pad_h, int pad_w_left,
                                    int pad_w_right, int dtype, void* stream) {
    if (!x || !y) return mfx_fail(MFX_ERR_ARG, "pack_image: null pointer");
    const long total = (long)B * (H + 2 * pad_h) * (W + pad_w_left + pad_w_right);
    if (total == 0) return MFX_OK;
    hipStream_t st = reinterpret_cast<hipStream_t>(stream);
    if (dtype == MFX_F32) hipLaunchKernelGGL(pack_image_kernel<float>, MFX_GRID(total, 256), dim3(256), 0, st, x, (float*)y, B, H, W, pad_h, pad_w_left, pad_w_right);
    else if (dtype == MFX_F16) hipLaunchKernelGGL(pack_image_kernel<half_t>, MFX_GRID(total, 256), dim3(256), 0, st, x, (half_t*)y, B, H, W, pad_h, pad_w_left, pad_w_right);
    else hipLaunchKernelGGL(pack_image_kernel<bf16_t>, MFX_GRID(total, 256), dim3(256), 0, st, x, (bf16_t*)y, B, H, W, pad_h, pad_w_left, pad_w_right);
    MFX_HIP_CHECK(hipGetLastError());
    return MFX_OK;
}

extern "C" int mfx_edge_scatter_add(float* out, int ld_out, int ch_off, int C, const float* v, int ldv,
                                    const int32_t* edge_xy, const int32_t* edge_len, int B, int L, int H, int W,
                                    float* planar, void* stream) {
    if (!out || !v || !edge_xy || !edge_len) return mfx_fail(MFX_ERR_ARG, "edge_scatter_add: null pointer");
// ... 8 lines not shown
```

### monoflex_amd/csrc/options.h

```cpp
#pragma once

#define MFX_NOLO (-2147483647 - 1)
#define MFX_NOHI 2147483647

#define MFX_OPTION_LIST(X) \
     \
    X(conv_tile, 0, MFX_NOLO, MFX_NOHI, "implicit-GEMM tile of mfx_conv2d_nhwc: 0 = automatic, else a tile id (conv_kernels.hip: 1 = 256x16, 2 = 256x32, 3 = 128x64, " \
        "4 = 64x64, 5 = 128x128, 6 = 64x128, 7 = 256x64, 8 = 256x128 / 8 waves, 9 = 128x128 / 8 waves), taken where it fits Cout_pad") \
    X(dcn_tile, 0, MFX_NOLO, MFX_NOHI, "the same for the fused gather DCN kernel") \
    X(cat_tile, 0, MFX_NOLO, MFX_NOHI, "the same for mfx_cat_conv1x1_nhwc") \
    X(kc, 0, MFX_NOLO, MFX_NOHI, "16-byte chunks per LDS row of the implicit-GEMM main loop: 0 = automatic (8 where K_pad allows), 4 = force 4") \
    X(ksplit, 0, MFX_NOLO, MFX_NOHI, "split-K of mfx_conv2d_nhwc: 0 = automatic (never: measured neutral-to-slower on DLA level4/5), 1 = never split, " \
        "n = force n splits where legal") \
    X(dcn_ksplit, 0, MFX_NOLO, MFX_NOHI, "the same for the fused DCN kernel") \
    X(halo, 1, MFX_NOLO, MFX_NOHI, "LDS-staged halo kernels for 3x3 convs: 0 = generic kernel only, 1 = automatic, >= 2 = force variant (value - 1)") \
    X(halo_cg, 0, MFX_NOLO, MFX_NOHI, "max channels per patch pass of the halo kernel (0 = default)") \
    X(halo_s2, 1, MFX_NOLO, MFX_NOHI, "0 = stride-2 3x3 convs stay on the generic implicit-GEMM kernel") \
    X(halo_pair, 1, MFX_NOLO, MFX_NOHI, "split precision walks K in step pairs where mfx_conv_desc.w_frag_pair is given (0 = two mma_chunk per pair)") \
    X(halo_cw, 1, MFX_NOLO, MFX_NOHI, "0 = conv3x3_wave_kernel only, 1 = the compile-time-geometry kernel (conv_cw.hip) where an instantiation exists") \
    X(cw_rows6, 1, MFX_NOLO, MFX_NOHI, "0 = 8-row tiles everywhere in conv_cw.hip (1: 6-row tiles where Ho % 6 == 0, Ho % 8 != 0, Ho <= 48)") \
    X(halo_cws, 1, MFX_NOLO, MFX_NOHI, "0 = conv3x3_wave_kernel<f32s_t> only, 1 = the compile-time-geometry split-precision kernel (conv_cws.hip) where an instantiation exists") \
     \
    X(dcn_wave, 1, MFX_NOLO, MFX_NOHI, "0 = first-generation kernel only, 1 = automatic, 2.. = force variant") \
    X(dcn_patch, 1, MFX_NOLO, MFX_NOHI, "LDS-patch DCN kernel: 0 = off, 1 = automatic, 2 = force (FM 4), 3 = force FM 2, 4 = force FM 1, 5-7 = wide margin FM 4/2/1, " \
        "8 = padded layout") \
    X(dcn_patch_fn8, 1, MFX_NOLO, MFX_NOHI, "1 = one workgroup of the LDS-patch kernel covers 128 output channels where Cout_pad % 128 == 0") \
    X(dcn_fuse_off, 1, MFX_NOLO, MFX_NOHI, "1 = the LDS-patch kernel computes the offset/mask conv itself where the caller supplies its weights") \
    X(dcn_lds, 1, MFX_NOLO, MFX_NOHI, "0 = off, 1 = automatic (64 -> 64 on large 16-bit maps), 2 = wherever the kernel applies") \
    X(dcn_lds_rows, 16, MFX_NOLO, MFX_NOHI, "tile rows, 16 | 8 (three workgroups per CU; measured slower: 2.570 vs 2.551 ms per step, profiles/r06_dcn_lds.md)") \
    X(dcn_group, 1, 0, 1, "1 = mfx_dcn_module_group runs same-shape 16-bit gather-kernel DCN modules as one offset-conv launch and one gather launch " \
        "(bit-identical output), 0 = it refuses every group and the caller launches module by module") \
     \
    X(heads_persist, 1, MFX_NOLO, MFX_NOHI, "1 = one workgroup per resident slot (n > 1: n workgroups), each a contiguous range of (tile, branch) units; " \
        "0 = one workgroup per tile.  B=8 bf16: 516 -> 503 us (tools/probes/heads_probe.py), bit-identical output") \
    X(heads_mfma32, 0, MFX_NOLO, MFX_NOHI, "1 = the v_mfma_f32_32x32x16 form of the kernel where the caller supplies its packs (mfx_heads_desc.w1_32 / w2_32)") \
    X(heads_planes, 0, MFX_NOLO, MFX_NOHI, "1 = four k-group planes (no LDS bank conflicts: 48 % -> 11 % of the LDS cycles, LDS-active cycles -42 %), " \
        "0 = one 144-byte record per pixel.  Same kernel time (555 vs 555 us, A/B in one run): not LDS-bound") \
    X(edge_chain, 1, MFX_NOLO, MFX_NOHI, "1 = the edge fusion's conv chain (trunk, Conv1d, 1x1 of both branches) as one kernel where mfx_edge_chain applies " \
        "(edge_chain.hip: 16-bit modes, bit-identical output), 0 = five mfx_conv2d_nhwc launches") \
    X(topk_strips, 8, MFX_NOLO, MFX_NOHI, "row strips per (class, image) map when a workspace is supplied; 1 = single-workgroup kernel") \
    X(topk_merge_z, 16, MFX_NOLO, MFX_NOHI, "workgroups per (class, image) map in the merge; values outside 1..64 are an error") \
    X(topk_merge_threads, 512, MFX_NOLO, MFX_NOHI, "their size; must be a multiple of 64 in 64..512 (the merge ranks by whole wavefronts; 512 = its __launch_bounds__)") \
     \
    X(wgrad_mfma, 1, MFX_NOLO, MFX_NOHI, "0 = VALU kernel for bf16 too, 1 = 64x64 MFMA tiles, 3 = 128x128 where they fit") \
    X(wgrad_blocks, 600, MFX_NOLO, MFX_NOHI, "target workgroup count of the MFMA weight-gradient kernel (measured, B=8 step: 64 -> 146 ms, 150 -> 90, 300 -> 78, " \
        "600 -> 73, 2048 -> 75, 8192 -> 81: the tile atomics of every slab cost more than the extra workgroups hide)") \
    X(wgrad_ws, 1, MFX_NOLO, MFX_NOHI, "0 = always accumulate the tiles with atomics") \
    X(wgrad_ws_blocks, 1200, MFX_NOLO, MFX_NOHI, "target workgroup count when partial tiles go to the workspace (step: 1200 -> 58.0 ms, 2400 -> 58.3, 4800 -> 58.6; " \
        "atomics: 59.6)") \
    X(wgrad_min_m, 128, MFX_NOLO, MFX_NOHI, "fewest pixels of a slab of the MFMA weight-gradient kernel.  r06: 1024 left the 1x1 / Root layers of the 24x80 and 12x40 " \
        "maps with 8-16 slabs (120-240 workgroups of 32 iterations each: 31 us per layer for 4 GFLOP); same-box step 17.50 (1024) / 17.31 (512) / 17.27 (256) / " \
        "17.23-17.31 (128) / 17.26 (64) ms") \
    X(wgrad_tr, 1, MFX_NOLO, MFX_NOHI, "0 = first-generation kernel everywhere (2: the transposed-read kernel also where Cout % 128 != 0)") \
    X(wgrad_tr_blocks, 512, 1, MFX_NOHI, "target workgroup count (tiles x pixel slabs)") \
    X(wgrad_patch, 1, MFX_NOLO, MFX_NOHI, "0 = off (the 3x3 / s1 / p1 weight-gradient form with the input patch in LDS)") \
    X(wgrad_patch_blocks, 256, 1, MFX_NOHI, "target workgroup count") \
    X(wgrad_patch_waves, 12, MFX_NOLO, MFX_NOHI, "6 (64 x 96 block per wave) or 12 (64 x 48)") \
    X(stem_wgrad_blocks, 512, 1, MFX_NOHI, "target workgroup count of the stem's weight-gradient kernel (mfx_stem_wgrad_16)") \
     \
    X(bn_apply_blocks, 1024, MFX_NOLO, MFX_NOHI, "workgroup cap of the two-launch forms' streaming kernels") \
    X(bn_blocks, 768, MFX_NOLO, MFX_NOHI, "target workgroup count of the column reductions (BN statistics / backward sums / bias sums)") \
    X(bn_onepass, 3, MFX_NOLO, MFX_NOHI, "bit 0 = backward, bit 1 = forward in one launch where the map fits (0 = the two-launch forms everywhere)") \
    X(bn_onepass_min_chunks, 200000, MFX_NOLO, MFX_NOHI, "smaller maps keep the two launches (backward)") \
    X(bn_onepass_fwd_min_chunks, 900000, MFX_NOLO, MFX_NOHI, "the same for the forward") \
    X(bn_onepass_grid, 0, MFX_NOLO, MFX_NOHI, "workgroup cap (0 = by map size, see bn_onepass_plan)") \
     \
    X(dcn_wgrad_m, 512, 64, MFX_NOHI, "pixels per workgroup slab of the DCN weight-gradient kernel (step: 512 -> 73.1 ms, 2048 -> 73.8, 8192 -> 83.6)") \
    X(ext_bwd_fast, 1, MFX_NOLO, MFX_NOHI, "0 = the first-generation scatter backward for every geometry of the `_ext` boundary") \
    X(dcn_bt_fuse_blocks, 170, MFX_NOLO, MFX_NOHI, "workgroups per tap group of the fused kernel; a value <= 0 means 170") \
    X(dcn_bt_fly_bias, 1, MFX_NOLO, MFX_NOHI, "the gcol-free sample kernel also sums grad_bias from the dy rows it loads (0: a separate column-sum pass)") \
    X(dcn_bt_gcol_as, 1, MFX_NOLO, MFX_NOHI, "d(columns) = dy . W^T of the 16-bit layers on the activation-stationary GEMM (gemm_as.hip); 0: the tiled 1x1 kernel") \
    X(dcn_bt_fly, 1, MFX_NOLO, MFX_NOHI, "64 -> 64 16-bit layers rebuild d(columns) from dy inside both consumers (no [M][9C] matrix in memory)") \
    X(dcn_bt_fuse_wgrad, 1, MFX_NOLO, MFX_NOHI, "64 -> 64 bf16 layers accumulate grad_weight inside the sample kernel (no columns in memory)") \
    X(dcn_bt_fuse_min_chunks, 1024, 1, MFX_NOHI, "fewer 32-pixel chunks than this keep the unfused kernels (tests lower it)") \
    X(dcn_bt_cs, 0, MFX_NOLO, MFX_NOHI, "channel slice of the tile kernel for C >= 128 (0 = by workgroup count, 64, 128)") \
    X(dcn_bt_cs_wgs, 1000, MFX_NOLO, MFX_NOHI, "below this many 128-channel workgroups the tile kernel takes 64-channel slices") \
     \
    X(deterministic, 0, MFX_NOLO, MFX_NOHI, "any non-zero value = 1: every floating-point reduction of the training path runs in a fixed order (single-writer partial " \
        "sums, one pixel slab per weight-gradient tile, 64-bit fixed-point accumulation of the DCN input gradient) so that two runs -- eager or replayed from a " \
        "hipGraph -- produce bit-identical results.  Slower; the default (0) keeps the atomics")

#define MFX_PROBE_OPTION_LIST(X) \
    X(dcn_bt_dbg, 0, MFX_NOLO, MFX_NOHI, "experiment switches of dcn_bwd_tile_kernel (0 in production)") \
    X(heads_dbg, 0, MFX_NOLO, MFX_NOHI, "timing probes of the bf16 heads kernel (see DBG in heads.hip)")

#define MFX_COUNTER_LIST(X) \
     \
    X(dcn_lds, "launches of the fourth-generation DCN kernel (dcn_lds.hip) on 16-bit maps") \
    X(dcn_lds_of, "those of dcn_lds that computed the offset/mask conv themselves") \
    X(dcn_lds_split, "launches of dcn_lds.hip in split precision (not counted in dcn_lds)") \
    X(dcn_patch, "launches of the third-generation, LDS-patch DCN kernel (dcn_patch.hip)") \
    X(dcn_wave, "launches of the second-generation DCN kernel (dcn_wave.hip)") \
    X(dcn_gather, "launches of the first-generation fused gather DCN kernel (conv_kernels.hip)") \
    X(dcn_group, "calls of mfx_dcn_module_group that ran a group (two launches: the grouped offset/mask conv, the grouped gather kernel; " \
        "neither is counted in conv_cw / dcn_gather)") \
    X(conv_cw, "launches of the compile-time-geometry 3x3 kernel (conv_cw.hip)") \
    X(conv_cws, "launches of its split-precision form (conv_cws.hip)") \
    X(conv_halo, "launches of the LDS-staged halo kernel (conv_halo.hip)") \
    X(conv_igemm, "launches of the generic implicit-GEMM kernel (conv_kernels.hip)") \
    X(conv_splitk, "those that ran split-K") \
    X(conv_bn_stats, "convolutions whose epilogue accumulated the BatchNorm statistics") \
    X(edge_chain, "launches of the edge fusion's one-kernel conv chain (edge_chain.hip)") \
    X(box_nms, "launches of the duplicate suppression (box_nms.hip): one per mfx_box_nms call that had rows, whatever B") \
    X(decode_multi, "launches of the several-modes-and-oracle box decode (decode_multi.hip): one per mfx_decode_boxes_multi call with B > 0") \
     \
    X(wgrad_patch, "weight gradients by the LDS-patch kernel (wgrad_tr.hip)") \
    X(wgrad_tr, "weight gradients by the transposed-read kernel (wgrad_tr.hip)") \
    X(wgrad_mfma, "weight gradients by the first-generation MFMA kernel (train_kernels.hip)") \
    X(wgrad_valu, "weight gradients by the VALU kernel") \
    X(wgrad_reduce, "launches of the pass that sums their partial tiles (wgrad_reduce_kernel)") \
    X(stem_wgrad, "launches of the stem's weight-gradient kernel") \
    X(bn_fwd_onepass, "train-mode BatchNorm forwards in one launch") \
    X(bn_bwd_onepass, "BatchNorm backwards in one launch") \
    X(bn_fwd_two, "BatchNorm forwards in the two-launch form") \
    X(bn_bwd_two, "BatchNorm backwards in the two-launch form") \
    X(dcn_bt_fly, "DCN backward calls that took the gcol-free form") \
    X(dcn_bt_fused, "launches of dcn_bwd_sample_wgrad_kernel") \
    X(dcn_bt_tile, "launches of dcn_bwd_tile_kernel") \
    X(dcn_bt_sample, "launches of dcn_bwd_sample_kernel") \
    X(dcn_bt_far, "launches of dcn_bwd_far_kernel + dcn_bwd_far_fly_kernel") \
    X(gram, "phase calls of mfx_gram_heads on 16-bit maps") \
    X(adamw_multi, "calls of mfx_adamw_multi") \
    X(optim_multi, "calls of mfx_optim_multi (the one-launch update with a rule / a gradient coefficient)") \
    X(optim_multi_sched, "calls of mfx_optim_multi_sched (the one-launch update reading beta1 from the device)") \
    X(grad_norm_multi, "calls of mfx_grad_norm_multi")

#define MFX_DECLARE_OPTION(name, def, lo, hi, doc) extern int g_opt_##name;
#define MFX_DECLARE_COUNTER(name, doc) extern long g_cnt_##name;
MFX_OPTION_LIST(MFX_DECLARE_OPTION)
MFX_PROBE_OPTION_LIST(MFX_DECLARE_OPTION)
MFX_COUNTER_LIST(MFX_DECLARE_COUNTER)
#undef MFX_DECLARE_OPTION
#undef MFX_DECLARE_COUNTER
```

### monoflex_amd/lib.py

```python
import ctypes
import os

HERE = os.path.dirname(os.path.abspath(__file__))
LIB_PATH = os.environ.get("MFX_LIB_PATH") or os.path.join(HERE, "csrc", "libmonoflex_hip.so")

MFX_F32, MFX_BF16, MFX_F16, MFX_F16X2 = 0, 1, 2, 3
ACT_NONE, ACT_RELU, ACT_LEAKY, ACT_DCN_OFFMASK = 0, 1, 2, 3
MAX_SEG = 9

c_int, c_void_p, c_float, c_size_t = ctypes.c_int32, ctypes.c_void_p, ctypes.c_float, ctypes.c_size_t


class ConvDesc(ctypes.Structure):
    _fields_ = [("x", c_void_p), ("w", c_void_p), ("w_frag", c_void_p), ("scale", c_void_p), ("shift", c_void_p), ("res", c_void_p),
                ("y", c_void_p), ("rowmap", c_void_p),
                ("B", c_int), ("H", c_int), ("W", c_int), ("x_pixstride", c_int), ("Ck", c_int),
                ("kh", c_int), ("kw", c_int), ("stride", c_int), ("pad_h", c_int), ("pad_w", c_int), ("dil_w", c_int),
                ("Ho", c_int), ("Wo", c_int), ("M", c_int), ("Cout", c_int), ("Cout_pad", c_int), ("K_pad", c_int),
                ("ldy", c_int), ("ldres", c_int), ("act", c_int), ("dtype", c_int), ("out_dtype", c_int),
                ("workspace", c_void_p), ("workspace_bytes", ctypes.c_int64),
                ("stats", c_void_p), ("stats_ncopy", c_int), ("stats_done", ctypes.POINTER(c_int)), ("w_frag_pair", c_void_p)]


class CatDesc(ctypes.Structure):
    _fields_ = [("src", c_void_p * MAX_SEG), ("stride", c_int * MAX_SEG), ("off", c_int * MAX_SEG),
                ("nseg", c_int), ("Cseg", c_int),
                ("w", c_void_p), ("scale", c_void_p), ("shift", c_void_p), ("res", c_void_p), ("y", c_void_p),
                ("M", c_int), ("Cout", c_int), ("Cout_pad", c_int), ("K_pad", c_int), ("ldy", c_int),
                ("ldres", c_int), ("act", c_int), ("dtype", c_int)]


class DcnDesc(ctypes.Structure):
    _fields_ = [("x", c_void_p), ("offmask", c_void_p), ("w", c_void_p), ("scale", c_void_p), ("shift", c_void_p),
                ("y", c_void_p), ("w_frag", c_void_p),
                ("B", c_int), ("H", c_int), ("W", c_int), ("C", c_int),
                ("kh", c_int), ("kw", c_int), ("stride", c_int), ("pad", c_int), ("dil", c_int),
                ("Ho", c_int), ("Wo", c_int), ("Cout", c_int), ("Cout_pad", c_int), ("K_pad", c_int),
                ("ldy", c_int), ("act", c_int), ("dtype", c_int), ("w_frag_f16", c_void_p),
                ("workspace", c_void_p), ("workspace_bytes", ctypes.c_int64),
                ("off_w_frag_f16", c_void_p), ("off_shift", c_void_p), ("offmask_out", c_void_p),
                ("nonsquare", c_int), ("stride_w", c_int), ("pad_w", c_int), ("dil_w", c_int), ("w_pair_f16", c_void_p)]


class HeadsDesc(ctypes.Structure):
    _fields_ = [("x", c_void_p), ("w1", c_void_p), ("scale1", c_void_p), ("shift1", c_void_p), ("w2", c_void_p),
                ("bias2", c_void_p), ("out", c_void_p), ("planar", c_void_p),
                ("B", c_int), ("H", c_int), ("W", c_int), ("nbranch", c_int), ("K_pad", c_int), ("ld_out", c_int),
                ("dtype", c_int), ("planar_c", c_int), ("ch_off", c_int * 16), ("c_out", c_int * 16), ("w2_scale", ctypes.c_float * 16),
                ("w1_32", c_void_p), ("w2_32", c_void_p)]


class EdgeChainDesc(ctypes.Structure):
    _fields_ = [(n, c_void_p) for n in ("x", "edge_xy", "w_trunk", "scale_trunk", "shift_trunk", "w_conv", "scale_conv", "shift_conv",
                                        "w_out", "bias_out", "out")] + \
        [(n, c_int) for n in ("B", "H", "W", "C", "L", "head_conv", "ksize", "relu", "dtype")]


class KittiDesc(ctypes.Structure):
    _fields_ = [(n, c_void_p) for n in (
        "records", "n_obj", "P", "img_wh", "flip", "hm", "cls_ids", "target_centers", "keypoints", "keypoints_depth_mask",
        "dimensions", "locations", "reg_mask", "reg_weight", "offset_3D", "bboxes", "gt_bboxes", "rotys", "trunc_mask", "alphas",
        "orientations", "occlusions", "truncations", "pad_size", "edge_indices", "edge_len", "P_out", "heat_radius", "status")] + \
        [(n, c_int) for n in ("B", "max_objs", "in_w", "in_h", "down", "num_classes")] + \
        [(n, ctypes.c_double) for n in ("filter_trunc", "filter_size", "edge_ratio")]


class KittiEncodeCfg(ctypes.Structure):
    _fields_ = [(n, ctypes.c_int32) for n in ("consider_outside_objs", "adjust_boundary_heatmap", "keypoint_visible_modify",
                                              "heatmap_center_2d")]


class KittiEvalDesc(ctypes.Structure):
    _fields_ = [(n, c_void_p) for n in ("gt", "dt", "gt_off", "dt_off", "pair_off", "classes", "min_overlaps", "overlaps", "tp_scores",
                                        "num_valid_gt", "thresholds", "num_thresholds", "pr")] + \
        [(n, c_int) for n in ("B", "n_gt", "n_dt", "num_classes", "num_k", "compute_aos")] + [("n_pairs", ctypes.c_int64)]


class AdamWDesc(ctypes.Structure):
    _fields_ = [("p", c_void_p), ("g", c_void_p), ("m", c_void_p), ("v", c_void_p), ("step", c_void_p), ("numel", ctypes.c_longlong),
                ("group", c_int), ("pad_", c_int)]


class AdamWGroup(ctypes.Structure):
    _fields_ = [("lr", c_void_p), ("beta1", c_float), ("beta2", c_float), ("eps", c_float), ("weight_decay", c_float)]


class PackDesc(ctypes.Structure):
    _fields_ = [("w", c_void_p), ("packed", c_void_p), ("frag", c_void_p)] + \
        [(n, c_int) for n in ("Cout", "Cin", "kh", "kw", "mode", "rows_pad", "K_pad", "ck")]


HEAD_MAX_BRANCH = 8


class HeadSparseDesc(ctypes.Structure):
    _fields_ = [(n, c_int) for n in ("nbranch", "N", "B", "H", "W", "C", "dtype", "ld_out")] + [("rows", c_void_p)] + \
        [(n, c_void_p * HEAD_MAX_BRANCH) for n in ("y", "mean", "rstd", "gamma", "beta", "w2", "b2")] + \
        [("k", c_int * HEAD_MAX_BRANCH), ("out_off", c_int * HEAD_MAX_BRANCH), ("out", c_void_p), ("dout", c_void_p), ("g", c_void_p)] + \
        [(n, c_void_p * HEAD_MAX_BRANCH) for n in ("sums", "dw2", "db2", "dx")] + [("arena", c_void_p), ("arena_bytes", c_size_t)]


class GramDesc(ctypes.Structure):
    _fields_ = [("x", c_void_p), ("rows", c_void_p), ("extra_rows", c_void_p)] + \
        [(n, c_int) for n in ("B", "H", "W", "C", "N", "Ne", "F", "nbranch", "extra_branch", "ld_out", "dtype", "nring", "ring_width", "arena_bytes")] + \
        [("momentum", c_float), ("Mt", c_float)] + \
        [(n, c_void_p * HEAD_MAX_BRANCH) for n in ("wk", "gamma", "beta", "w2", "b2", "run_mean", "run_var", "nbt", "dgamma", "dbeta", "dw2", "db2", "dwt")] + \
        [("eps", c_float * HEAD_MAX_BRANCH), ("k", c_int * HEAD_MAX_BRANCH), ("off", c_int * HEAD_MAX_BRANCH)] + \
        [(n, c_void_p) for n in ("A", "Wkc", "WkT", "R5", "S0", "P", "csA", "G", "m", "Tm", "sums", "stat", "Y", "Ye", "act", "act_e", "out",
                                 "dout", "dact_e", "dYh", "dYl", "dYeh", "dYel", "dsum", "ds", "scal", "Dw16", "dm", "dGs", "Kx", "Gn16", "cscale", "cshift",
                                 "dAf", "dArows", "dx", "ring_inv", "ring_idx", "dwo", "dwe")]


OBJ_ROW, OBJ_TERMS, OBJ_VALUES = 72, 10, 24


class ObjectLossCfg(ctypes.Structure):
    _fields_ = [("w", c_float * OBJ_TERMS), ("dim_mean", c_float * 9), ("dim_std", c_float * 9), ("dim_weight", c_float * 3),
                ("depth_ref", c_float * 2), ("depth_range", c_float * 2)] + \
        [(n, c_float) for n in ("unc_lo", "unc_hi", "down_ratio", "eps")] + \
        [(n, c_int) for n in ("depth_mode", "has_depth_range", "dim_exp", "dim_use_std", "iou_type", "corner_depth_mode",
                              "separate_trunc", "trunc_log", "modify_invalid")] + [("ch", c_int * 9), ("reg_width", c_int)]
    reg_loss = 0
    depth_loss = 0


class DecodeCfg(ctypes.Structure):
    _fields_ = [("dim_mean", c_float * 9), ("dim_std", c_float * 9), ("depth_ref", c_float * 2), ("depth_range", c_float * 2),
                ("down_ratio", c_float), ("eps", c_float)] + \
        [(n, c_int) for n in ("depth_decode", "dim_exp", "dim_use_std", "uncertainty_as_conf", "output_depth")]


class HeadLayout(ctypes.Structure):
    _fields_ = [("ch", c_int * 9), ("reg_width", c_int)]


_P, _I, _F, _S = c_void_p, c_int, c_float, c_size_t
SYMBOLS = {
    "mfx_abi_version": (_I, []),
    "mfx_last_error": (ctypes.c_char_p, []),
    "mfx_stem_conv7x7_nchw": (_I, [_P, _P, _P, _P, _P, _I, _I, _I, _I, _I, _I, _I, _P]),
    "mfx_f1_fused": (_I, [_P] * 11 + [_I, _I, _I, _I, _I, _P]),
    "mfx_set_option": (_I, [ctypes.c_char_p, _I]),
    "mfx_reset_options": (_I, []),
    "mfx_commit_options": (_I, []),
    "mfx_get_counter": (ctypes.c_long, [ctypes.c_char_p]),
    "mfx_f16x2_range_check": (ctypes.c_int, [ctypes.c_int]),
    "mfx_dcn_v2_workspace_bytes": (_S, [_I] * 14),
    "mfx_dcn_v2_workspace_bytes_g": (_S, [_I] * 15),
    "mfx_dcn_v2_forward": (_I, [_P] * 6 + [_I] * 14 + [_P, _S, _P]),
    "mfx_dcn_v2_backward": (_I, [_P] * 11 + [_I] * 14 + [_P, _S, _P]),
    "mfx_dcn_v2_psroi_pooling_forward": (_I, [_P] * 5 + [_I] * 8 + [_F] + [_I] * 5 + [_F, _P]),
    "mfx_dcn_v2_psroi_pooling_backward": (_I, [_P] * 7 + [_I] * 8 + [_F] + [_I] * 5 + [_F, _P]),
    "mfx_conv2d_nhwc": (_I, [ctypes.POINTER(ConvDesc), _P]),
    "mfx_cat_conv1x1_nhwc": (_I, [ctypes.POINTER(CatDesc), _P]),
    "mfx_dcn_nhwc": (_I, [ctypes.POINTER(DcnDesc), _P]),
    "mfx_dcn_sample_nhwc": (_I, [_P, _P, _P, _P, _P, _I, _I, _I, _I, _I, _I, _I, _P]),
    "mfx_project_nhwc": (_I, [_P, _P, _P, _I, _I, _I, _I, _I, _I, _P]),
    "mfx_maxpool2x2_nhwc": (_I, [_P, _P, _I, _I, _I, _I, _I, _P]),
    "mfx_upsample_add_nhwc": (_I, [_P, _P, _P, _P, _I, _I, _I, _I, _I, _I, _P]),
    "mfx_nchw_to_nhwc": (_I, [_P, _P, _I, _I, _I, _I, _I, _I, _P]),
    "mfx_nhwc_to_nchw": (_I, [_P, _P, _I, _I, _I, _I, _I, _I, _P]),
    "mfx_pack_image_nhwc4": (_I, [_P, _P, _I, _I, _I, _I, _I, _I, _I, _P]),
    "mfx_heads_fused": (_I, [ctypes.POINTER(HeadsDesc), _P]),
    "mfx_heads_fused_act": (_I, [ctypes.POINTER(HeadsDesc), _I, _P]),
    "mfx_dcn_fuses_offset_conv": (_I, [ctypes.POINTER(DcnDesc)]),
    "mfx_dcn_module_group": (_I, [ctypes.POINTER(ConvDesc), ctypes.POINTER(DcnDesc), _I, _P]),
    "mfx_edge_scatter_add": (_I, [_P, _I, _I, _I, _P, _I, _P, _P, _I, _I, _I, _I, _P, _P]),
    "mfx_edge_chain": (_I, [ctypes.POINTER(EdgeChainDesc), _P]),
    "mfx_edge_chain_act": (_I, [ctypes.POINTER(EdgeChainDesc), _I, _P]),
    "mfx_edge_chain_applies": (_I, [ctypes.POINTER(EdgeChainDesc)]),
    "mfx_edge_chain_ks": (_I, [ctypes.POINTER(EdgeChainDesc), _I, _P]),
    "mfx_edge_chain_ks_applies": (_I, [ctypes.POINTER(EdgeChainDesc)]),
    "mfx_decode_topk_workspace_bytes": (_S, [_I, _I, _I]),
    "mfx_decode_topk": (_I, [_P, ctypes.c_long, ctypes.c_long, ctypes.c_long, _I, _I, _I, _I, _I, _P, _P, _P, _S, _P]),
    "mfx_conv_wgrad_nhwc": (_I, [_P, _P, _P] + [_I] * 15 + [_P]),
    "mfx_conv_wgrad_nhwc_dil": (_I, [_P, _P, _P] + [_I] * 16 + [_P]),
    "mfx_conv_wgrad_oihw": (_I, [_P, _P, _P] + [_I] * 17 + [_P, _S, _P]),
    "mfx_pack_conv_weight": (_I, [_P, _I, _I, _I, _I, _I, _P, _P, _I, _I, _I, _I, _P]),
    "mfx_adamw_chunk_elems": (_I, []),
    "mfx_adamw_multi": (_I, [_P, _P, _I, ctypes.c_longlong, _P, _P, _P]),
    "mfx_optim_multi": (_I, [_P, _P, _I, ctypes.c_longlong, _P, _I, _P, _P, _P]),
    "mfx_optim_multi_sched": (_I, [_P, _P, _I, ctypes.c_longlong, _P, _P, _I, _P, _P, _P]),
    "mfx_grad_norm_workspace_bytes": (_S, [ctypes.c_longlong]),
    "mfx_grad_norm_multi": (_I, [_P, _P, _I, ctypes.c_longlong, _F, _P, _S, _P, _P, _P]),
    "mfx_colsum": (_I, [_P, _P, ctypes.c_long, _I, _I, _I, _P]),
    "mfx_colsum_add": (_I, [_P, _P, ctypes.c_long, _I, _I, _I, _P]),
    "mfx_bn_stats": (_I, [_P, _P, _P, ctypes.c_long, _I, _I, _P]),
    "mfx_bn_finalize": (_I, [_P, _P, _P, _P, _P, _P, _F, _F, ctypes.c_long, _P, _P, _P, _P, _I, _P]),
    "mfx_bn_act_fwd": (_I, [_P, _P, _P, _P, _P, ctypes.c_long, _I, _I, _I, _P]),
    "mfx_bn_act_bwd": (_I, [_P] * 10 + [ctypes.c_long, _I, _I, _I, _P]),
    "mfx_stem_wgrad_bf16": (_I, [_P, _P, _P, _I, _I, _I, _I, _I, _P, _S, _P]),
    "mfx_stem_wgrad_16": (_I, [_P, _P, _P, _I, _I, _I, _I, _I, _I, _P, _S, _P]),
    "mfx_pack_chunk_elems": (_I, []),
    "mfx_pack_conv_weights_batched": (_I, [_P, _P, _I, ctypes.c_longlong, _I, _P]),
    "mfx_head_sparse_fwd": (_I, [ctypes.POINTER(HeadSparseDesc), _P]),
    "mfx_head_sparse_bwd": (_I, [ctypes.POINTER(HeadSparseDesc), _P]),
    "mfx_gram_heads": (_I, [ctypes.POINTER(GramDesc), _I, _P]),
    "mfx_head_sparse_fwd_act": (_I, [ctypes.POINTER(HeadSparseDesc), _I, _P]),
    "mfx_head_sparse_bwd_act": (_I, [ctypes.POINTER(HeadSparseDesc), _I, _P]),
    "mfx_gram_heads_act": (_I, [ctypes.POINTER(GramDesc), _I, _I, _P]),
    "mfx_bn_train_stats": (_I, [_P] * 6 + [_F, _F, ctypes.c_long, _I, _I, _P, _P, _P, _I, _P]),
    "mfx_bn_scratch_bytes": (_S, []),
    "mfx_bn_ncopy": (_I, [_I]),
    "mfx_bn_train_fwd": (_I, [_P] * 8 + [_F, _F, ctypes.c_long, _I, _I, _I, _P, _P, _P, _I, _P]),
    "mfx_bn_train_bwd": (_I, [_P] * 11 + [ctypes.c_long, _I, _I, _I, _P, _P]),
    "mfx_bn_bwd_reduce": (_I, [_P] * 7 + [ctypes.c_long, _I, _I, _I, _P]),
    "mfx_bn_bwd_apply": (_I, [_P] * 10 + [ctypes.c_long, ctypes.c_long, _I, _I, _I, _P]),
    "mfx_maxpool2x2_bwd_nhwc": (_I, [_P, _P, _P, _I, _I, _I, _I, _I, _P]),
    "mfx_bn_onepass_stuck": (_I, [_I]),
    "mfx_upsample_bwd_workspace_bytes": (_S, [_I, _I, _I, _I]),
    "mfx_upsample_bwd_nhwc": (_I, [_P, _P, _P, _P, _P, _I, _I, _I, _I, _I, _I, _P, _S, _P]),
    "mfx_upsample_bwd_nhwc_oihw": (_I, [_P, _P, _P, _P, _P, _I, _I, _I, _I, _I, _I, _P, _S, _P]),
    "mfx_zero_insert2_nhwc": (_I, [_P, _P, _I, _I, _I, _I, _I, _I, _I, _P]),
    "mfx_dcn_backward_nhwc_workspace_bytes": (_S, [_I] * 10),
    "mfx_dcn_backward_nhwc": (_I, [_P] * 8 + [_I] * 10 + [_P, _S, _P]),
    "mfx_dcn_backward_nhwc_bf16": (_I, [_P] * 8 + [_I] * 10 + [_P, _S, _P]),
    "mfx_dcn_backward_v2_workspace_bytes": (_S, [_I] * 6),
    "mfx_dcn_backward_v2": (_I, [_P] * 8 + [_I] * 6 + [_P, _S, _P]),
    "mfx_dcn_backward_v2_rt": (_I, [_P] * 6 + [_I] + [_P] * 2 + [_I] * 6 + [_P, _S, _P]),
    "mfx_focal_loss": (_I, [_P, _P, _I, _I, _I, _I, _F, _F, _P, _P, _P]),
    "mfx_object_loss": (_I, [_P, _I, _I, _I, _I, _I, _P, _I, ctypes.POINTER(ObjectLossCfg), _P, _P, _P]),
    "mfx_object_loss_types": (_I, [_P, _I, _I, _I, _I, _I, _P, _I, ctypes.POINTER(ObjectLossCfg), _I, _I, _P, _P, _P]),
    "mfx_object_loss_backward": (_I, [_P, _P, _P, _I, _I, _I, _I, _P, _I, _I, _P]),
    "mfx_object_loss_backward_width": (_I, [_P, _P, _P, _I, _I, _I, _I, _P, _I, _I, _I, _P]),
    "mfx_box3d_iou_pairs": (_I, [_P, _P, _I, _I, _P, _P]),
    "mfx_box_nms": (_I, [_P, _P, _I, _I, _I, _F, _I, _P, _P]),
    "mfx_eval_diagnostics": (_I, [_P, _I, _I, _P, _I, _I, _I, _I, _P, _P, ctypes.POINTER(DecodeCfg), ctypes.POINTER(HeadLayout), _I, _P, _P, _P, _P]),
    "mfx_kitti_encode_targets": (_I, [ctypes.POINTER(KittiDesc), _P]),
    "mfx_kitti_encode_targets_views": (_I, [ctypes.POINTER(KittiDesc), _P, _P]),
    "mfx_kitti_encode_targets_cfg": (_I, [ctypes.POINTER(KittiDesc), _P, ctypes.POINTER(KittiEncodeCfg), _P]),
    "mfx_kitti_preprocess_u8": (_I, [_P, _P, _P, _P, _P, _I, _I, _I, ctypes.POINTER(c_float), ctypes.POINTER(c_float), _P]),
    "mfx_kitti_preprocess_u8_bgr": (_I, [_P, _P, _P, _P, _P, _I, _I, _I, ctypes.POINTER(c_float), ctypes.POINTER(c_float), _P]),
    "mfx_kitti_preprocess_u8_indexed": (_I, [_P, _P, _P, _P, _P, _P, _I, _I, _I, _I, ctypes.POINTER(c_float), ctypes.POINTER(c_float), _I, _P]),
    "mfx_kitti_encode_targets_indexed": (_I, [ctypes.POINTER(KittiDesc), _P, ctypes.c_int32, _P, ctypes.POINTER(KittiEncodeCfg), _P]),
    "mfx_kitti_eval_overlaps": (_I, [ctypes.POINTER(KittiEvalDesc), _P]),
    "mfx_kitti_eval_match_pass1": (_I, [ctypes.POINTER(KittiEvalDesc), _P]),
    "mfx_kitti_eval_thresholds": (_I, [ctypes.POINTER(KittiEvalDesc), _P, _P]),
    "mfx_kitti_eval_match_pass2": (_I, [ctypes.POINTER(KittiEvalDesc), _P]),
    "mfx_kitti_eval_pack_count": (_I, [_P, _I, _I, _I, _I, _P, _P, _P, _P]),
    "mfx_kitti_eval_pack_rows": (_I, [_P, _P, _I, _I, _I, _I, _P, _P, _P]),
    "mfx_decode_boxes": (_I, [_P, _I, _I, _P, _P, _I, _I, _I, _I, _I, _P, _P, _P, _F, _P, _P, _P, _P]),
    "mfx_decode_boxes_mode": (_I, [_P, _I, _I, _P, _P, _I, _I, _I, _I, _I, _P, _P, _P, _F, _I, _P, _P, _P, _P]),
    "mfx_decode_boxes_cfg": (_I, [_P, _I, _I, _P, _P, _I, _I, _I, _I, _I, _P, _P, _P, _F, ctypes.POINTER(DecodeCfg), _P, _P, _P, _P, _P]),
    "mfx_decode_boxes_heads": (_I, [_P, _I, _I, _P, _P, _I, _I, _I, _I, _I, _P, _P, _P, _F, ctypes.POINTER(DecodeCfg), ctypes.POINTER(HeadLayout),
                                    _P, _P, _P, _P, _P]),
    "mfx_decode_boxes_multi": (_I, [_P, _I, _I, _P, _P, _I, _I, _I, _I, _I, _P, _P, _P, _F, ctypes.POINTER(DecodeCfg), ctypes.POINTER(HeadLayout),
                                    ctypes.c_uint32, _P, _I, _P, _P, _P, _P, _P, _P]),
}

DEPTH_MODES = {"soft": 0, "hard": 1, "mean": 2, "direct": 3, "keypoints_avg": 4, "keypoints_center": 5, "keypoints_02": 6, "keypoints_13": 7}
DEPTH_ORACLE = 8

NMS_KINDS = {"2d": 1, "3d": 2}
NMS_MAX_ROWS = 128

DEPTH_DECODES = {"exp": 0, "linear": 1, "inv_sigmoid": 2}


def head_decode_settings(cfg):
    H = cfg.MODEL.HEAD
    return dict(depth_mode=H.DEPTH_MODE, depth_range=None if H.DEPTH_RANGE is None else tuple(float(v) for v in H.DEPTH_RANGE),
                depth_ref=tuple(float(v) for v in H.DEPTH_REFERENCE),
                dim_mean=tuple(tuple(float(v) for v in row) for row in H.DIMENSION_MEAN),
                dim_std=tuple(tuple(float(v) for v in row) for row in H.DIMENSION_STD),
                dim_modes=list(H.DIMENSION_REG), down_ratio=cfg.MODEL.BACKBONE.DOWN_RATIO, eps=1e-3)


HEAD_KEYS = ('2d_dim', '3d_offset', 'corner_offset', 'corner_uncertainty', '3d_dim', 'ori_cls', 'ori_offset', 'depth', 'depth_uncertainty')
HEAD_WIDTHS = dict(zip(HEAD_KEYS, (4, 2, 20, 3, 3, 8, 8, 1, 1)))
HEAD_OPTIONAL = ('depth_uncertainty', 'corner_offset', 'corner_uncertainty')
REG_LOSSES = ('L1', 'smooth_l1')
DEPTH_LOSSES = ('L1', 'log', 'inv_sig')
OPTIM_ADAMW, OPTIM_ADAM_L2 = 0, 1
OPTIM_ADAM_TRUE_WD = 2
CORNER_DEPTHS = ('direct', 'keypoint_mean', 'soft_combine', 'hard_combine')
LOSS_REQUIRED = ('hm_loss', 'bbox_loss', 'depth_loss', 'offset_loss', 'orien_loss', 'dims_loss')
LOSS_OPTIONAL = ('corner_loss', 'trunc_offset_loss', 'keypoint_loss', 'keypoint_depth_loss', 'weighted_avg_depth_loss')


class HeadSet:

    def __init__(self, regression_heads, regression_channels):
        names = [n for group in regression_heads for n in group]
        widths = [int(w) for group in regression_channels for w in group]
        if len(names) != len(widths) or [len(g) for g in regression_heads] != [len(g) for g in regression_channels]:
            raise NotImplementedError("head set: REGRESSION_HEADS and REGRESSION_CHANNELS do not pair up: %r / %r" % (regression_heads, regression_channels))
        bad = [n for n in names if n not in HEAD_KEYS] + [n for n in set(names) if names.count(n) > 1]
        if bad:
            raise NotImplementedError("head set: unknown or repeated regression keys %s (known: %s)" % (sorted(set(bad)), ", ".join(HEAD_KEYS)))
        missing = [k for k in HEAD_KEYS if k not in names and k not in HEAD_OPTIONAL]
        if missing:
            raise NotImplementedError("head set %s: the required keys %s are missing" % (names, missing))
        wrong = ["%s(%d)" % (n, w) for n, w in zip(names, widths) if HEAD_WIDTHS[n] != w]
        if wrong:
            raise NotImplementedError("head set: channel counts %s differ from the reference's %s" % (wrong, [HEAD_WIDTHS[n] for n in names]))
        self.names, self.widths = names, widths
        self.starts, start = {}, 0
        for n, w in zip(names, widths):
            self.starts[n] = start
            start += w
        self.R = start
        self.du, self.kp, self.cu = ('depth_uncertainty' in names), ('corner_offset' in names), ('corner_uncertainty' in names)
        if self.cu and not self.kp:
            raise NotImplementedError("head set %s: corner_uncertainty without corner_offset" % (names,))
        self.full = self.du and self.kp and self.cu

    def describe(self):
        return "head set (depth_uncertainty %d, corner_offset %d, corner_uncertainty %d; %d channels)" % (self.du, self.kp, self.cu, self.R)

    def ch(self, key):
        return self.starts.get(key, -1)

    def corner_depths(self):
        return CORNER_DEPTHS[:1] + (CORNER_DEPTHS[1:2] if self.kp else ()) + (CORNER_DEPTHS[2:] if self.full else ())

    def output_depths(self):
        out = ('direct',)
        if self.kp:
            out += ('keypoints_avg', 'keypoints_center', 'keypoints_02', 'keypoints_13')
# ... 130 lines not shown
```

### monoflex_amd/model/backbone/DCNv2/dcn_v2.py

```python
import math

import torch
from torch import nn
from torch.autograd import Function
from torch.autograd.function import once_differentiable
from torch.nn.modules.utils import _pair

from . import _ext as _backend
from .... import lib as L
from .... import ops


class _DCNv2(Function):
    @staticmethod
    def forward(ctx, input, offset, mask, weight, bias, stride, padding, dilation, deformable_groups):
        ctx.stride = _pair(stride)
        ctx.padding = _pair(padding)
        ctx.dilation = _pair(dilation)
        ctx.kernel_size = _pair(weight.shape[2:4])
        ctx.deformable_groups = deformable_groups
        output = _backend.dcn_v2_forward(input, weight, bias, offset, mask,
                                         ctx.kernel_size[0], ctx.kernel_size[1], ctx.stride[0], ctx.stride[1],
                                         ctx.padding[0], ctx.padding[1], ctx.dilation[0], ctx.dilation[1],
                                         ctx.deformable_groups)
        ctx.save_for_backward(input, offset, mask, weight, bias)
        return output

    @staticmethod
    @once_differentiable
    def backward(ctx, grad_output):
        input, offset, mask, weight, bias = ctx.saved_tensors
        grad_input, grad_offset, grad_mask, grad_weight, grad_bias = _backend.dcn_v2_backward(
            input, weight, bias, offset, mask, grad_output,
            ctx.kernel_size[0], ctx.kernel_size[1], ctx.stride[0], ctx.stride[1],
            ctx.padding[0], ctx.padding[1], ctx.dilation[0], ctx.dilation[1], ctx.deformable_groups)
        return grad_input, grad_offset, grad_mask, grad_weight, grad_bias, None, None, None, None


dcn_v2_conv = _DCNv2.apply


class DCNv2(nn.Module):
    def __init__(self, in_channels, out_channels, kernel_size, stride, padding, dilation=1, deformable_groups=1):
        super().__init__()
        self.in_channels, self.out_channels = in_channels, out_channels
        self.kernel_size, self.stride = _pair(kernel_size), _pair(stride)
        self.padding, self.dilation = _pair(padding), _pair(dilation)
        self.deformable_groups = deformable_groups
        self.weight = nn.Parameter(torch.Tensor(out_channels, in_channels, *self.kernel_size))
        self.bias = nn.Parameter(torch.Tensor(out_channels))
        self.reset_parameters()

    def reset_parameters(self):
        n = self.in_channels
        for k in self.kernel_size:
            n *= k
        stdv = 1.0 / math.sqrt(n)
        self.weight.data.uniform_(-stdv, stdv)
        self.bias.data.zero_()

    def forward(self, input, offset, mask):
        assert 2 * self.deformable_groups * self.kernel_size[0] * self.kernel_size[1] == offset.shape[1]
        assert self.deformable_groups * self.kernel_size[0] * self.kernel_size[1] == mask.shape[1]
        return dcn_v2_conv(input, offset, mask, self.weight, self.bias, self.stride, self.padding,
                           self.dilation, self.deformable_groups)


OFFSET_CONV_FP32 = [False]


class DCN(DCNv2):

    def __init__(self, in_channels, out_channels, kernel_size, stride, padding, dilation=1, deformable_groups=1):
        super().__init__(in_channels, out_channels, kernel_size, stride, padding, dilation, deformable_groups)
        channels_ = self.deformable_groups * 3 * self.kernel_size[0] * self.kernel_size[1]
        self.conv_offset_mask = nn.Conv2d(self.in_channels, channels_, kernel_size=self.kernel_size,
                                          stride=self.stride, padding=self.padding, bias=True)
        self.init_offset()
        self._packs = {}

    def init_offset(self):
        self.conv_offset_mask.weight.data.zero_()
        self.conv_offset_mask.bias.data.zero_()

    def packed_offset(self, dtype):
        key = ("off", dtype)
        if key not in self._packs:
            c = self.conv_offset_mask
            p = ops.pack_conv(c.weight, dtype, None, c.bias, stride=self.stride[0], pad=self.padding[0],
                              act=L.ACT_DCN_OFFMASK, cout=32)
            self._packs[key] = ops.add_f16_fragments(p, c.weight)
        return self._packs[key]

    def packed_main(self, dtype, bn=None, act=L.ACT_NONE):
        key = ("main", dtype, id(bn), act)
        if key not in self._packs:
            if bn is not None:
                scale, shift = ops.fold_bn(bn, self.bias)
            else:
                scale, shift = None, self.bias
            p = ops.pack_conv(self.weight, dtype, scale, shift, stride=self.stride[0], pad=self.padding[0], act=act)
            p.dil_w = self.dilation[0]
            ops.add_f16_fragments(p, self.weight)
            self._packs[key] = p
        return self._packs[key]

    def forward_nhwc(self, x, bn=None, act=L.ACT_NONE, done=None):
        if OFFSET_CONV_FP32[0] and x.dtype != torch.float32:
            offmask = ops.conv2d(x.float(), self.packed_offset(torch.float32), out_dtype=torch.float32)
        else:
            tag = ops.compute_tag(self, x.dtype)
            return ops.dcn_module(x, self.packed_offset(tag), self.packed_main(tag, bn, act), done=done)[0]
        return ops.dcn(x, offmask, self.packed_main(ops.compute_tag(self, x.dtype), bn, act))

    def forward_nhwc_train(self, x):
        from .... import autograd as AG
        c = self.conv_offset_mask
        return AG.dcn_module(x, c.weight, c.bias, self.weight, self.bias, self.stride[0], self.padding[0], self.dilation[0])

    def forward(self, input):
        from .... import autograd as AG
        kh, kw = self.kernel_size
        square = self.stride[0] == self.stride[1] and self.padding[0] == self.padding[1] and self.dilation[0] == self.dilation[1]
        recording = torch.is_grad_enabled() and (input.requires_grad or any(p.requires_grad for p in self.parameters()))
        if not square:
            raise RuntimeError("DCN: stride / padding / dilation must be square on this build (the MonoFlex model only builds square "
                               "3x3 DCNs, dla_dcn.py:391; `_ext.dcn_v2_forward` reports the same)")
        if self.deformable_groups == 1 and not recording:
            dtype = torch.float32 if input.dtype == torch.float32 else torch.bfloat16
            x = ops.nchw_to_nhwc(input, dtype)
            return ops.nhwc_to_nchw(self.forward_nhwc(x))
        x = input.float().permute(0, 2, 3, 1).contiguous()
        c = self.conv_offset_mask
        if self.deformable_groups == 1:
            y = AG.dcn_module(x, c.weight, c.bias, self.weight, self.bias, self.stride[0], self.padding[0], self.dilation[0])
            return y.permute(0, 3, 1, 2).contiguous()
        out = AG.conv2d(x, c.weight, c.bias, self.stride[0], self.padding[0], out_dtype=torch.float32).permute(0, 3, 1, 2)
        n = self.deformable_groups * kh * kw
        offset, mask = out[:, :2 * n].contiguous(), torch.sigmoid(out[:, 2 * n:3 * n]).contiguous()
        return dcn_v2_conv(input.float(), offset, mask, self.weight, self.bias, self.stride, self.padding, self.dilation, self.deformable_groups)


class _DCNv2Pooling(Function):

    @staticmethod
    def forward(ctx, input, rois, offset, spatial_scale, pooled_size, output_dim, no_trans, group_size=1, part_size=None,
                sample_per_part=4, trans_std=.0):
        ctx.geometry = (int(no_trans), spatial_scale, output_dim, group_size, pooled_size,
                        pooled_size if part_size is None else part_size, sample_per_part, trans_std)
        output, output_count = _backend.dcn_v2_psroi_pooling_forward(input, rois, offset, *ctx.geometry)
        ctx.save_for_backward(input, rois, offset, output_count)
        return output

    @staticmethod
    @once_differentiable
    def backward(ctx, grad_output):
        input, rois, offset, output_count = ctx.saved_tensors
        grad_input, grad_offset = _backend.dcn_v2_psroi_pooling_backward(grad_output, input, rois, offset, output_count, *ctx.geometry)
        return (grad_input, None, grad_offset) + (None,) * 8


dcn_v2_pooling = _DCNv2Pooling.apply


class DCNv2Pooling(nn.Module):

    def __init__(self, spatial_scale, pooled_size, output_dim, no_trans, group_size=1, part_size=None, sample_per_part=4, trans_std=.0):
        super().__init__()
        self.spatial_scale, self.pooled_size, self.output_dim, self.no_trans = spatial_scale, pooled_size, output_dim, no_trans
        self.group_size = group_size
        self.part_size = pooled_size if part_size is None else part_size
        self.sample_per_part, self.trans_std = sample_per_part, trans_std

    def _pool(self, input, rois, offset, no_trans):
        return dcn_v2_pooling(input, rois, offset, self.spatial_scale, self.pooled_size, self.output_dim, no_trans, self.group_size,
                              self.part_size, self.sample_per_part, self.trans_std)

    def forward(self, input, rois, offset):
        assert input.shape[1] == self.output_dim
        return self._pool(input, rois, input.new() if self.no_trans else offset, self.no_trans)


class DCNPooling(DCNv2Pooling):

    def __init__(self, spatial_scale, pooled_size, output_dim, no_trans, group_size=1, part_size=None, sample_per_part=4, trans_std=.0,
                 deform_fc_dim=1024):
        super().__init__(spatial_scale, pooled_size, output_dim, no_trans, group_size, part_size, sample_per_part, trans_std)
        self.deform_fc_dim = deform_fc_dim
        if not no_trans:
            bins = self.pooled_size * self.pooled_size
            self.offset_mask_fc = nn.Sequential(nn.Linear(bins * self.output_dim, self.deform_fc_dim), nn.ReLU(inplace=True),
                                                nn.Linear(self.deform_fc_dim, self.deform_fc_dim), nn.ReLU(inplace=True),
                                                nn.Linear(self.deform_fc_dim, bins * 3))
            self.offset_mask_fc[4].weight.data.zero_()
            self.offset_mask_fc[4].bias.data.zero_()

    def forward(self, input, rois):
        if self.no_trans:
            return self._pool(input, rois, input.new(), self.no_trans)
        n = rois.shape[0]
        plain = self._pool(input, rois, input.new(), True)
        offset_mask = self.offset_mask_fc(plain.view(n, -1)).view(n, 3, self.pooled_size, self.pooled_size)
        o1, o2, mask = torch.chunk(offset_mask, 3, dim=1)
        return self._pool(input, rois, torch.cat((o1, o2), dim=1), self.no_trans) * torch.sigmoid(mask)
```

### monoflex_amd/model/backbone/dla_dcn.py

```python
import math
import os

import numpy as np
import torch
from torch import nn

from ... import autograd as AG
from ... import lib as L
from ... import ops
from .DCNv2.dcn_v2 import DCN

BN_MOMENTUM = 0.1


def build_backbone(cfg):
    return DLASeg(base_name=cfg.MODEL.BACKBONE.CONV_BODY, pretrained=cfg.MODEL.PRETRAIN,
                  down_ratio=cfg.MODEL.BACKBONE.DOWN_RATIO, last_level=5)


def invalidate_packs(module):
    for m in module.modules():
        if hasattr(m, "_packs"):
            m._packs.clear()

# ... 74 lines not shown
            root_dim = 2 * out_channels
        if level_root:
            root_dim += in_channels
        if levels == 1:
            self.tree1 = block(in_channels, out_channels, stride, dilation=dilation)
            self.tree2 = block(out_channels, out_channels, 1, dilation=dilation)
        else:
            self.tree1 = Tree(levels - 1, block, in_channels, out_channels, stride, root_dim=0,
                              root_kernel_size=root_kernel_size, dilation=dilation, root_residual=root_residual)
            self.tree2 = Tree(levels - 1, block, out_channels, out_channels, root_dim=root_dim + out_channels,
                              root_kernel_size=root_kernel_size, dilation=dilation, root_residual=root_residual)
        if levels == 1:
            self.root = Root(root_dim, out_channels, root_kernel_size, root_residual)
        self.level_root, self.root_dim, self.levels = level_root, root_dim, levels
        self.downsample = nn.MaxPool2d(stride, stride=stride) if stride > 1 else None
        self.project = None
        if in_channels != out_channels:
            self.project = nn.Sequential(nn.Conv2d(in_channels, out_channels, kernel_size=1, stride=1, bias=False),
                                         nn.BatchNorm2d(out_channels, momentum=BN_MOMENTUM))

    def forward(self, x, residual=None, children=None, bottom=None):
        children = [] if children is None else children
        if bottom is None:
            if self.training:
                bottom = AG.MaxPool2x2Fn.apply(x) if self.downsample else x
            else:
                bottom = ops.maxpool2x2(x) if self.downsample else x
        if self.levels == 1:
            if not self.project:
                residual = bottom
            elif self.training:
                residual = _train_conv_bn(bottom, self.project[0], self.project[1], L.ACT_NONE)
            else:
                residual = ops.conv2d(bottom, _conv_bn(self, "proj", self.project[0], self.project[1], x.dtype, L.ACT_NONE))
        if self.level_root:
            children.append(bottom)
        if self.levels > 1 and isinstance(self.tree1, Tree) and self.tree1.downsample is not None and self.downsample is not None:
            x1 = self.tree1(x, residual, bottom=bottom)
        else:
            x1 = self.tree1(x, residual)
        if self.levels == 1:
            x2 = self.tree2(x1)
            return self.root(x2, x1, *children)
        children.append(x1)
        return self.tree2(x1, children=children)


class DLA(nn.Module):
    def __init__(self, levels, channels, num_classes=1000, block=BasicBlock, residual_root=False, linear_root=False):
        super().__init__()
        self.channels, self.num_classes = channels, num_classes
        self.base_layer = nn.Sequential(nn.Conv2d(3, channels[0], kernel_size=7, stride=1, padding=3, bias=False),
                                        nn.BatchNorm2d(channels[0], momentum=BN_MOMENTUM), nn.ReLU(inplace=True))
        self.level0 = self._make_conv_level(channels[0], channels[0], levels[0])
        self.level1 = self._make_conv_level(channels[0], channels[1], levels[1], stride=2)
        self.level2 = Tree(levels[2], block, channels[1], channels[2], 2, level_root=False, root_residual=residual_root)
        self.level3 = Tree(levels[3], block, channels[2], channels[3], 2, level_root=True, root_residual=residual_root)
        self.level4 = Tree(levels[4], block, channels[3], channels[4], 2, level_root=True, root_residual=residual_root)
        self.level5 = Tree(levels[5], block, channels[4], channels[5], 2, level_root=True, root_residual=residual_root)

    @staticmethod
    def _make_conv_level(inplanes, planes, convs, stride=1, dilation=1):
        modules = []
        for i in range(convs):
            modules.extend([nn.Conv2d(inplanes, planes, kernel_size=3, stride=stride if i == 0 else 1,
                                      padding=dilation, bias=False, dilation=dilation),
                            nn.BatchNorm2d(planes, momentum=BN_MOMENTUM), nn.ReLU(inplace=True)])
            inplanes = planes
        return nn.Sequential(*modules)

    def forward(self, images, dtype, cut=None):
        if self.training:
            return self._forward_train(images, dtype, cut)
        packs = self.__dict__.setdefault("_packs", {})
        tag = ops.compute_tag(self, dtype)
        if ("stem", tag) not in packs:
            scale, shift = ops.fold_bn(self.base_layer[1])
            packs[("stem", tag)] = ops.pack_stem(self.base_layer[0].weight, tag, scale, shift)
        B, _, H, W = images.shape
        if FUSE_F1[0] and ((dtype in (torch.bfloat16, torch.float16) and tag == dtype) or tag == ops.F16X2) and packs[("stem", tag)].Cout == 16 \
                and len(self.level0) == 3 and len(self.level1) == 3 and H % 2 == 0 and W % 2 == 0 and self.channels[:2] == [16, 32]:
            x = ops.f1_fused(images, packs[("stem", tag)], _conv_bn(self.level0, "c0", self.level0[0], self.level0[1], dtype, L.ACT_RELU),
                             _conv_bn(self.level1, "c0", self.level1[0], self.level1[1], dtype, L.ACT_RELU))
            y = [None, x]
            for i in range(2, 6):
                x = getattr(self, "level{}".format(i))(x)
                y.append(x)
            return y
        if (dtype in (torch.bfloat16, torch.float16) or tag == ops.F16X2) and packs[("stem", tag)].Cout == 16:
            x = ops.stem_conv(images, packs[("stem", tag)])
        else:
            x = ops.conv2d(ops.pack_image(images, dtype), packs[("stem", tag)], out_hw=(H, W))
        y = []
        for i in range(6):
            lvl = getattr(self, "level{}".format(i))
            if i < 2:
                for j in range(0, len(lvl), 3):
                    x = ops.conv2d(x, _conv_bn(lvl, "c%d" % j, lvl[j], lvl[j + 1], dtype, L.ACT_RELU))
            else:
                x = lvl(x)
            y.append(x)
        return y


def _dla_forward_train(self, images, dtype, cut=None):
    x = AG.bn_act(AG.StemConvFn.apply(images, self.base_layer[0].weight, dtype), self.base_layer[1], L.ACT_RELU)
    y = []
    for i in range(6):
        lvl = getattr(self, "level{}".format(i))
        if cut is not None and i == 4:
            x = cut("level3", [x])[0]
        if i < 2:
            for j in range(0, len(lvl), 3):
                x = _train_conv_bn(x, lvl[j], lvl[j + 1], L.ACT_RELU)
        else:
            x = lvl(x)
        y.append(x)
    return y


DLA._forward_train = _dla_forward_train


def dla34(pretrained=True, **kwargs):
    model = DLA([1, 1, 1, 2, 2, 1], [16, 32, 64, 128, 256, 512], block=BasicBlock, **kwargs)
    if pretrained:
        path = pretrained if isinstance(pretrained, str) else os.environ.get("MONOFLEX_DLA34_WEIGHTS", "")
        if not path or not os.path.exists(path):
            raise RuntimeError("dla34(pretrained=True) needs the ImageNet weights http://dl.yf.io/dla/models/imagenet/"
                               "dla34-ba72cf86.pth as a local file: set MONOFLEX_DLA34_WEIGHTS=<path> or MODEL.PRETRAIN "
                               "to the path (no network in this build), or set MODEL.PRETRAIN False and load a checkpoint")
        from ...utils.model_serialization import load_dla_imagenet
        load_dla_imagenet(model, path)
    return model


def fill_up_weights(up):
    w = up.weight.data
    f = math.ceil(w.size(2) / 2)
    c = (2 * f - 1 - f % 2) / (2.0 * f)
    for i in range(w.size(2)):
        for j in range(w.size(3)):
            w[0, 0, i, j] = (1 - math.fabs(i / f - c)) * (1 - math.fabs(j / f - c))
    for ch in range(1, w.size(0)):
        w[ch, 0, :, :] = w[0, 0, :, :]


class DeformConv(nn.Module):
    def __init__(self, chi, cho):
        super().__init__()
        self.actf = nn.Sequential(nn.BatchNorm2d(cho, momentum=BN_MOMENTUM), nn.ReLU(inplace=True))
        self.conv = DCN(chi, cho, kernel_size=(3, 3), stride=1, padding=1, dilation=1, deformable_groups=1)

    def forward(self, x, done=None):
        if self.training:
            return AG.bn_act(self.conv.forward_nhwc_train(x), self.actf[0], L.ACT_RELU)
        return self.conv.forward_nhwc(x, bn=self.actf[0], act=L.ACT_RELU, done=done)


class IDAUp(nn.Module):
    def __init__(self, o, channels, up_f):
        super().__init__()
        for i in range(1, len(channels)):
            c, f = channels[i], int(up_f[i])
            up = nn.ConvTranspose2d(o, o, f * 2, stride=f, padding=f // 2, output_padding=0, groups=o, bias=False)
            fill_up_weights(up)
            setattr(self, "proj_" + str(i), DeformConv(c, o))
            setattr(self, "up_" + str(i), up)
            setattr(self, "node_" + str(i), DeformConv(o, o))

    def forward(self, layers, startp, endp):
        packs = self.__dict__.setdefault("_packs", {})
        if not self.training and PARALLEL_PROJ[0] and endp - startp > 2 and layers[startp].is_cuda:
            return self._forward_parallel_proj(layers, startp, endp, packs)
        proj = {} if self.training else self._grouped_proj(layers, startp, endp)
        for i in range(startp + 1, endp):
            k = i - startp
            up = getattr(self, "up_" + str(k))
            if k not in packs:
                packs[k] = ops.pack_upsample(up.weight)
            t = getattr(self, "proj_" + str(k))(layers[i], done=proj.pop(k)) if k in proj else getattr(self, "proj_" + str(k))(layers[i])
            if self.training:
                t = AG.UpsampleAddFn.apply(t, up.weight, layers[i - 1], up.stride[0])
                layers[i] = getattr(self, "node_" + str(k))(t)
                continue
            t = ops.upsample_add(t, packs[k], up.stride[0], skip=layers[i - 1])
            layers[i] = getattr(self, "node_" + str(k))(t)


def _idaup_grouped_proj(self, layers, startp, endp):
    from .DCNv2 import dcn_v2
    out = {}
    if endp - startp < 3 or dcn_v2.OFFSET_CONV_FP32[0] or not layers[startp + 1].is_cuda:
        return out
    groups = {}
    for k in range(1, endp - startp):
        x, m = layers[startp + k], getattr(self, "proj_" + str(k))
        if x.dtype in (torch.bfloat16, torch.float16) and ops.compute_tag(m.conv, x.dtype) == x.dtype:
            groups.setdefault((tuple(x.shape), x.dtype, m.conv.out_channels), []).append(k)
    for ks in groups.values():
        for j in range(0, len(ks) - 1, 4):
            part = ks[j:j + 4]
            if len(part) < 2:
                continue
            mods = [getattr(self, "proj_" + str(k)) for k in part]
            xs = [layers[startp + k] for k in part]
            ys, oms = ops.dcn_module_group(xs, [m.conv.packed_offset(x.dtype) for m, x in zip(mods, xs)],
                                           [m.conv.packed_main(x.dtype, m.actf[0], L.ACT_RELU) for m, x in zip(mods, xs)])
            out.update(zip(part, zip(ys, oms)))
    return out


IDAUp._grouped_proj = _idaup_grouped_proj


def _idaup_forward_parallel_proj(self, layers, startp, endp, packs):
    cur = torch.cuda.current_stream()
    n = endp - startp - 1
    side = self.__dict__.setdefault("_side_streams", [])
    while len(side) < n - 1:
        side.append(torch.cuda.Stream())
    proj = [None] * n
    for k in range(2, n + 1):
        st = side[k - 2]
        st.wait_stream(cur)
        with torch.cuda.stream(st):
            proj[k - 1] = getattr(self, "proj_" + str(k))(layers[startp + k])
    proj[0] = self.proj_1(layers[startp + 1])
    for k in range(1, n + 1):
        i = startp + k
        up = getattr(self, "up_" + str(k))
        if k not in packs:
            packs[k] = ops.pack_upsample(up.weight)
        if k >= 2:
            cur.wait_stream(side[k - 2])
        t = ops.upsample_add(proj[k - 1], packs[k], up.stride[0], skip=layers[i - 1])
        layers[i] = getattr(self, "node_" + str(k))(t)


FUSE_F1 = [os.environ.get("MFX_FUSE_F1", "1") == "1"]

IDAUp._forward_parallel_proj = _idaup_forward_parallel_proj
PARALLEL_PROJ = [__import__("os").environ.get("MFX_PARALLEL_PROJ", "0") == "1"]


class DLAUp(nn.Module):
    def __init__(self, startp, channels, scales, in_channels=None):
        super().__init__()
        self.startp = startp
        if in_channels is None:
            in_channels = channels
        self.channels = channels
        channels = list(channels)
        in_channels = list(in_channels)
        scales = np.array(scales, dtype=int)
        for i in range(len(channels) - 1):
            j = -i - 2
            setattr(self, "ida_{}".format(i), IDAUp(channels[j], in_channels[j:], scales[j:] // scales[j]))
            scales[j + 1:] = scales[j]
            in_channels[j + 1:] = [channels[j] for _ in channels[j + 1:]]

    def forward(self, layers):
        out = [layers[-1]]
        for i in range(len(layers) - self.startp - 1):
            getattr(self, "ida_{}".format(i))(layers, len(layers) - i - 2, len(layers))
            out.insert(0, layers[-1])
        return out


class DLASeg(nn.Module):
    def __init__(self, base_name, pretrained, down_ratio, last_level):
        super().__init__()
        assert down_ratio in [2, 4, 8, 16]
        self.first_level = int(np.log2(down_ratio))
        self.last_level = last_level
        self.base = globals()[base_name](pretrained=pretrained)
        channels = self.base.channels
        scales = [2 ** i for i in range(len(channels[self.first_level:]))]
        self.dla_up = DLAUp(self.first_level, channels[self.first_level:], scales)
        self.out_channels = channels[self.first_level]
        self.ida_up = IDAUp(self.out_channels, channels[self.first_level:self.last_level],
                            [2 ** i for i in range(self.last_level - self.first_level)])
        self.compute_dtype = torch.float32

    def forward_nhwc(self, images, cut=None):
        cut = cut if (cut is not None and self.training) else None
        x = self.base(images, self.compute_dtype, cut) if cut is not None else self.base(images, self.compute_dtype)
        if cut is not None:
            x = cut("base", list(x))
        x = self.dla_up(list(x))
        y = [x[i] for i in range(self.last_level - self.first_level)]
        if cut is not None:
            y = cut("dla_up", y)
        self.ida_up(y, 0, len(y))
        return y[-1]

    def forward(self, images, cut=None):
        return self.forward_nhwc(images, cut).permute(0, 3, 1, 2)
```

### monoflex_amd/ops.py

```python
import ctypes
import os
from typing import Optional

import torch

from . import lib as L
from .packing import (F16X2, STEM_PAD_H, STEM_PAD_WL, STEM_PAD_WR, PackedCat, PackedConv, PackedEdgeChain, PackedHeads, _elems, _pad_rows_cols, _pow2,
                      _round_up, add_f16_fragments, cast_operand, compute_tag, cout_pad, dcn_pair_fragments, dcn_ps_pack, fold_bn, fragment_major,
                      pack_cat, pack_conv, pack_edge_chain, pack_heads, pack_stem, pack_upsample, pair_steps, split_chunks, split_halves, split_weight_scale,
                      storage_dtype)


def _stream():
    return ctypes.c_void_p(torch.cuda.current_stream().cuda_stream)


def _first_cuda_device(args):
    for a in args:
        if torch.is_tensor(a):
            if a.is_cuda:
                return a.device
        elif isinstance(a, (list, tuple)):
            d = _first_cuda_device(a)
            if d is not None:
                return d
    return None


def on_tensor_device(fn):
    import functools

    @functools.wraps(fn)
    def run(*args, **kwargs):
        dev = _first_cuda_device(args) or _first_cuda_device(tuple(kwargs.values()))
        if dev is None or dev.index == torch.cuda.current_device():
            return fn(*args, **kwargs)
        with torch.cuda.device(dev):
            return fn(*args, **kwargs)
    return run


def _dt(dtype):
    if dtype == torch.float32:
        return L.MFX_F32
    if dtype == torch.bfloat16:
        return L.MFX_BF16
    if dtype == torch.float16:
        return L.MFX_F16
    raise TypeError("MonoFlex HIP kernels take float32, bfloat16 or float16, got %s" % dtype)


def _ptr(t):
    return ctypes.c_void_p(t.data_ptr()) if t is not None else None


def _need_cuda(*ts):
    dev = None
    for t in ts:
        if t is None:
            continue
        if not t.is_cuda:
            raise RuntimeError("MonoFlex HIP operator called with a CPU tensor: the product path has no CPU "
                               "fallback (the CPU oracle lives in oracle/ and is test-only)")
        if dev is None:
            dev = t.device
        elif t.device != dev:
            raise RuntimeError("MonoFlex HIP operator: operands on different devices (%s and %s)" % (dev, t.device))


@on_tensor_device
def conv2d(x, p: PackedConv, res=None, out_dtype=None, rowmap=None, x_channels=None, x_ch_off=0,
           out_hw=None, in_hw=None, stats=None):
    _need_cuda(x, res, rowmap)
    B, H, W, Cx = x.shape
    if in_hw is not None:
        H, W = in_hw
    out_dtype = out_dtype or x.dtype
    if out_hw is None:
        Ho = (H + 2 * p.pad_h - ((p.kh - 1) + 1)) // p.stride + 1
        Wo = (W + 2 * p.pad_w - (p.dil_w * (p.kw - 1) + 1)) // p.stride + 1
    else:
        Ho, Wo = out_hw
    M = B * Ho * Wo if rowmap is None else rowmap.numel()
    y = torch.empty((B, Ho, Wo, p.Cout) if rowmap is None else (M, p.Cout), dtype=out_dtype, device=x.device)
    d = L.ConvDesc()
    d.x = x.data_ptr() + x_ch_off * x.element_size()
    d.w, d.scale, d.shift = p.w.data_ptr(), (p.scale.data_ptr() if p.scale is not None else None), \
        (p.shift.data_ptr() if p.shift is not None else None)
    d.w_frag = p.w_frag.data_ptr() if p.w_frag is not None else None
    d.w_frag_pair = p.w_frag_pair.data_ptr() if p.w_frag_pair is not None else None
    d.res = res.data_ptr() if res is not None else None
    d.y = y.data_ptr()
    d.rowmap = rowmap.data_ptr() if rowmap is not None else None
    d.B, d.H, d.W, d.x_pixstride, d.Ck = B, H, W, Cx, p.Ck
    d.kh, d.kw, d.stride, d.pad_h, d.pad_w, d.dil_w = p.kh, p.kw, p.stride, p.pad_h, p.pad_w, p.dil_w
    d.Ho, d.Wo, d.M, d.Cout, d.Cout_pad, d.K_pad = Ho, Wo, M, p.Cout, p.Cout_pad, p.K_pad
    d.ldy, d.ldres = p.Cout, (res.shape[-1] if res is not None else 0)
    d.act, d.dtype, d.out_dtype = p.act, (L.MFX_F16X2 if p.split else _dt(x.dtype)), _dt(out_dtype)
    if rowmap is None and M * p.Cout_pad <= SPLITK_MAX_ELEMS and p.K_pad * x.element_size() >= 2048:
        ws = _splitk_workspace(x.device)
        d.workspace, d.workspace_bytes = ws.data_ptr(), ws.numel() * 4
    if stats is not None:
        done = ctypes.c_int(0)
        d.stats, d.stats_ncopy, d.stats_done = stats.data_ptr(), L.load().mfx_bn_ncopy(p.Cout), ctypes.pointer(done)
        L.check(L.load().mfx_conv2d_nhwc(ctypes.byref(d), _stream()), "mfx_conv2d_nhwc")
        conv2d.last_stats_done = bool(done.value)
        return y
    L.check(L.load().mfx_conv2d_nhwc(ctypes.byref(d), _stream()), "mfx_conv2d_nhwc")
    return y


conv2d.last_stats_done = False


@on_tensor_device
def cat_conv1x1(srcs, p: PackedCat):
    _need_cuda(*srcs)
    B, H, W, _ = srcs[0].shape
    y = torch.empty((B, H, W, p.Cout), dtype=srcs[0].dtype, device=srcs[0].device)
    d = L.CatDesc()
    n = 0
    for s in srcs:
        C = s.shape[3]
        for part in range(C // p.Cseg):
            d.src[n], d.stride[n], d.off[n] = s.data_ptr(), C, part * p.Cseg
            n += 1
    d.nseg, d.Cseg = n, p.Cseg
    d.w, d.res, d.y = p.w.data_ptr(), None, y.data_ptr()
    d.scale = p.scale.data_ptr() if p.scale is not None else None
    d.shift = p.shift.data_ptr() if p.shift is not None else None
    d.M, d.Cout, d.Cout_pad, d.K_pad, d.ldy, d.ldres, d.act = B * H * W, p.Cout, p.Cout_pad, p.K_pad, p.Cout, 0, p.act
    d.dtype = L.MFX_F16X2 if p.split else _dt(y.dtype)
    L.check(L.load().mfx_cat_conv1x1_nhwc(ctypes.byref(d), _stream()), "mfx_cat_conv1x1_nhwc")
    return y


def _dcn_desc(x, offmask, p: PackedConv, y, off: Optional[PackedConv] = None, offmask_out=None):
    B, H, W, C = x.shape
    Ho, Wo = y.shape[1], y.shape[2]
    d = L.DcnDesc()
    d.x, d.w, d.y = x.data_ptr(), p.w.data_ptr(), y.data_ptr()
    d.offmask = offmask.data_ptr() if offmask is not None else None
    d.w_frag = p.w_frag.data_ptr() if p.w_frag is not None else None
    d.w_frag_f16 = p.w_frag_f16.data_ptr() if p.w_frag_f16 is not None else None
    d.w_pair_f16 = p.w_pair_f16.data_ptr() if p.w_pair_f16 is not None else None
    d.scale = p.scale.data_ptr() if p.scale is not None else None
    d.shift = p.shift.data_ptr() if p.shift is not None else None
    d.B, d.H, d.W, d.C = B, H, W, C
    d.kh, d.kw, d.stride, d.pad, d.dil = p.kh, p.kw, p.stride, p.pad_h, p.dil_w
    d.Ho, d.Wo, d.Cout, d.Cout_pad, d.K_pad, d.ldy, d.act = Ho, Wo, p.Cout, p.Cout_pad, p.K_pad, p.Cout, p.act
    d.dtype = L.MFX_F16X2 if p.split else _dt(x.dtype)
    if off is not None and off.w_frag_f16 is not None and off.shift is not None and off.Cout_pad == 32 and off.K_pad == 9 * C:
        d.off_w_frag_f16, d.off_shift = off.w_frag_f16.data_ptr(), off.shift.data_ptr()
        d.offmask_out = offmask_out.data_ptr() if offmask_out is not None else None
    return d


@on_tensor_device
def dcn(x, offmask, p: PackedConv):
    _need_cuda(x, offmask)
    B = x.shape[0]
    Ho, Wo = offmask.shape[1], offmask.shape[2]
    y = torch.empty((B, Ho, Wo, p.Cout), dtype=x.dtype, device=x.device)
    d = _dcn_desc(x, offmask, p, y)
    if B * Ho * Wo * p.Cout_pad <= SPLITK_MAX_ELEMS:
        ws = _splitk_workspace(x.device)
        d.workspace, d.workspace_bytes = ws.data_ptr(), ws.numel() * 4
    L.check(L.load().mfx_dcn_nhwc(ctypes.byref(d), _stream()), "mfx_dcn_nhwc")
    return y


DCN_PS = [os.environ.get("MFX_DCN_PS", "1") != "0"]
DCN_PS_MAX_BYTES = [int(os.environ.get("MFX_DCN_PS_MAX_MB", "24")) << 20]
PROJECT_AS = [os.environ.get("MFX_PROJECT_AS", "1") != "0"]


def dcn_ps_applies(x, p: PackedConv):
    B, H, W, C = x.shape
    if p.transient:
        return False
    return (DCN_PS[0] and x.dtype in (torch.bfloat16, torch.float16) and not p.split and p.kh == 3 and p.kw == 3 and p.stride == 1 and p.pad_h == 1
            and p.dil_w == 1 and p.K_pad == 9 * C and C >= 128 and p.Cout == p.Cout_pad and p.Cout in (64, 128, 256)
            and B * H * W * 9 * p.Cout * 2 <= DCN_PS_MAX_BYTES[0])


@on_tensor_device
def dcn_ps(x, offmask, p: PackedConv):
    _need_cuda(x, offmask)
    B, H, W, C = x.shape
    pp = dcn_ps_pack(p)
    if PROJECT_AS[0] and pp.K_pad == C and (C in (128, 512) or (C == 256 and 9 * p.Cout >= 2304)):
        proj = torch.empty((B, H, W, 9 * p.Cout), dtype=x.dtype, device=x.device)
        L.check(L.load().mfx_project_nhwc(_ptr(x), _ptr(pp.w), _ptr(proj), B * H * W, C, 9 * p.Cout, C, 9 * p.Cout, _dt(x.dtype), _stream()), "mfx_project_nhwc")
    else:
        proj = conv2d(x, pp)
    y = torch.empty((B, H, W, p.Cout), dtype=x.dtype, device=x.device)
    L.check(L.load().mfx_dcn_sample_nhwc(_ptr(proj), _ptr(offmask), _ptr(p.scale), _ptr(p.shift), _ptr(y), B, H, W, p.Cout, p.Cout, p.act,
                                         _dt(x.dtype), _stream()), "mfx_dcn_sample_nhwc")
    return y


@on_tensor_device
def dcn_module(x, p_off: PackedConv, p: PackedConv, need_offmask=False, done=None):
    _need_cuda(x)
    if done is not None:
        return done
    B, H, W, C = x.shape
    if p.stride == 1 and p.pad_h == 1 and p.kh == 3 and p.kw == 3:
        y = torch.empty((B, H, W, p.Cout), dtype=x.dtype, device=x.device)
        om = torch.empty((B, H, W, 32), dtype=torch.float32, device=x.device) if need_offmask else None
        d = _dcn_desc(x, None, p, y, off=p_off, offmask_out=om)
        if d.off_w_frag_f16 and L.load().mfx_dcn_fuses_offset_conv(ctypes.byref(d)):
            L.check(L.load().mfx_dcn_nhwc(ctypes.byref(d), _stream()), "mfx_dcn_nhwc")
            return y, om
    om = conv2d(x, p_off, out_dtype=torch.float32)
    if dcn_ps_applies(x, p):
        return dcn_ps(x, om, p), om
    return dcn(x, om, p), om


@on_tensor_device
def dcn_module_group(xs, p_offs, ps):
    _need_cuda(*xs)
    n = len(xs)
    x0, p0 = xs[0], ps[0]

    def same(a, b):
        return all(getattr(a, f) == getattr(b, f) for f in ("kh", "kw", "stride", "pad_h", "pad_w", "dil_w", "Ck", "Cout", "Cout_pad", "K_pad", "act", "split"))
    ok = (1 <= n <= 4 and x0.dtype in (torch.bfloat16, torch.float16) and not p0.split and p0.stride == 1 and p0.pad_h == 1 and p0.kh == 3 and p0.kw == 3
          and all(x.shape == x0.shape and x.dtype == x0.dtype and x.is_contiguous() for x in xs)
          and all(same(p, p0) for p in ps) and all(same(q, p_offs[0]) for q in p_offs)
          and all(q.w_frag is not None and q.Cout_pad == 32 for q in p_offs)
          and not any(dcn_ps_applies(x, p) for x, p in zip(xs, ps)))
    if ok:
        B, H, W, C = x0.shape
        offs, dcns = (L.ConvDesc * n)(), (L.DcnDesc * n)()
        ys = [torch.empty((B, H, W, p0.Cout), dtype=x0.dtype, device=x0.device) for _ in range(n)]
        oms = [torch.empty((B, H, W, 32), dtype=torch.float32, device=x0.device) for _ in range(n)]
        for i, (x, q, p) in enumerate(zip(xs, p_offs, ps)):
            d = offs[i]
            d.x, d.w, d.w_frag, d.y = x.data_ptr(), q.w.data_ptr(), q.w_frag.data_ptr(), oms[i].data_ptr()
            d.scale = q.scale.data_ptr() if q.scale is not None else None
            d.shift = q.shift.data_ptr() if q.shift is not None else None
            d.B, d.H, d.W, d.x_pixstride, d.Ck = B, H, W, C, q.Ck
            d.kh, d.kw, d.stride, d.pad_h, d.pad_w, d.dil_w = q.kh, q.kw, q.stride, q.pad_h, q.pad_w, q.dil_w
            d.Ho, d.Wo, d.M, d.Cout, d.Cout_pad, d.K_pad = H, W, B * H * W, q.Cout, q.Cout_pad, q.K_pad
            d.ldy, d.ldres, d.act, d.dtype, d.out_dtype = q.Cout, 0, q.act, _dt(x.dtype), L.MFX_F32
            dd = _dcn_desc(x, oms[i], p, ys[i])
            if B * H * W * p.Cout_pad <= SPLITK_MAX_ELEMS:
                ws = _splitk_workspace(x.device)
                dd.workspace, dd.workspace_bytes = ws.data_ptr(), ws.numel() * 4
            ctypes.memmove(ctypes.byref(dcns[i]), ctypes.byref(dd), ctypes.sizeof(L.DcnDesc))
        rc = L.load().mfx_dcn_module_group(offs, dcns, n, _stream())
        if rc == 0:
            return ys, oms
        if rc < 0:
            L.check(rc, "mfx_dcn_module_group")
    outs = [dcn_module(x, q, p) for x, q, p in zip(xs, p_offs, ps)]
    return [o[0] for o in outs], [o[1] for o in outs]


@on_tensor_device
def maxpool2x2(x):
    _need_cuda(x)
    B, H, W, C = x.shape
    y = torch.empty((B, H // 2, W // 2, C), dtype=x.dtype, device=x.device)
    L.check(L.load().mfx_maxpool2x2_nhwc(_ptr(x), _ptr(y), B, H, W, C, _dt(x.dtype), _stream()), "mfx_maxpool2x2_nhwc")
    return y


@on_tensor_device
def upsample_add(x, w_taps, f, skip=None):
    _need_cuda(x, w_taps, skip)
    B, H, W, C = x.shape
    y = torch.empty((B, H * f, W * f, C), dtype=x.dtype, device=x.device)
    L.check(L.load().mfx_upsample_add_nhwc(_ptr(x), _ptr(w_taps), _ptr(skip), _ptr(y), B, H, W, C, f, _dt(x.dtype), _stream()),
            "mfx_upsample_add_nhwc")
    return y


@on_tensor_device
def nchw_to_nhwc(x, dtype, channels=None):
    _need_cuda(x)
    x = x.float().contiguous()
    B, C, H, W = x.shape
    ld = channels or C
    y = torch.empty((B, H, W, ld), dtype=dtype, device=x.device)
    L.check(L.load().mfx_nchw_to_nhwc(_ptr(x), _ptr(y), B, C, H, W, ld, _dt(dtype), _stream()), "mfx_nchw_to_nhwc")
    return y


@on_tensor_device
def nhwc_to_nchw(x, channels=None):
    _need_cuda(x)
    B, H, W, ld = x.shape
    C = channels or ld
    y = torch.empty((B, C, H, W), dtype=torch.float32, device=x.device)
    L.check(L.load().mfx_nhwc_to_nchw(_ptr(x), _ptr(y), B, C, H, W, ld, _dt(x.dtype), _stream()), "mfx_nhwc_to_nchw")
    return y


@on_tensor_device
def pack_image(images, dtype):
    _need_cuda(images)
    images = images.float().contiguous()
    dtype = storage_dtype(dtype)
    B, C, H, W = images.shape
    assert C == 3
    y = torch.empty((B, H + 2 * STEM_PAD_H, W + STEM_PAD_WL + STEM_PAD_WR, 4), dtype=dtype, device=images.device)
    L.check(L.load().mfx_pack_image_nhwc4(_ptr(images), _ptr(y), B, H, W, STEM_PAD_H, STEM_PAD_WL, STEM_PAD_WR,
                                          _dt(dtype), _stream()), "mfx_pack_image_nhwc4")
    return y


@on_tensor_device
def stem_conv(images, p: PackedConv):
    _need_cuda(images)
    images = images.float().contiguous()
    B, C, H, W = images.shape
    assert C == 3 and p.w.dtype in (torch.bfloat16, torch.float16) and p.Cout == 16
    y = torch.empty((B, H, W, 16), dtype=torch.float32 if p.split else p.w.dtype, device=images.device)
    L.check(L.load().mfx_stem_conv7x7_nchw(_ptr(images), _ptr(p.w), _ptr(p.scale), _ptr(p.shift), _ptr(y), B, H, W, 16, p.K_pad, p.act,
                                           L.MFX_F16X2 if p.split else _dt(p.w.dtype), _stream()), "mfx_stem_conv7x7_nchw")
    return y


@on_tensor_device
def f1_fused(images, p_stem: PackedConv, p_l0: PackedConv, p_l1: PackedConv):
    _need_cuda(images)
    images = images.float().contiguous()
    B, C, H, W = images.shape
    split = p_stem.split
    dt = torch.float32 if split else p_stem.w.dtype
    assert C == 3 and (split or dt in (torch.bfloat16, torch.float16)) and p_stem.Cout == 16 and p_l0.Cout == 16 and p_l1.Cout == 32 and p_l1.stride == 2
    assert p_l0.split == split and p_l1.split == split
    for p in (p_l0, p_l1):
        if p.f1_w160 is None:
            assert p.K_pad >= 160 and p.Ck == 16
            p.f1_w160 = p.w[:, :160].contiguous()
    y = torch.empty((B, H // 2, W // 2, 32), dtype=dt, device=images.device)
    L.check(L.load().mfx_f1_fused(_ptr(images), _ptr(p_stem.w), _ptr(p_stem.scale), _ptr(p_stem.shift),
                                  _ptr(p_l0.f1_w160), _ptr(p_l0.scale), _ptr(p_l0.shift),
                                  _ptr(p_l1.f1_w160), _ptr(p_l1.scale), _ptr(p_l1.shift),
                                  _ptr(y), B, H, W, p_stem.K_pad, L.MFX_F16X2 if split else _dt(dt), _stream()), "mfx_f1_fused")
    return y


@on_tensor_device
def heads_fused(x, p: PackedHeads, planar_classes=0):
    _need_cuda(x)
    B, H, W, C = x.shape
    assert C == 64
    out = torch.empty((B, H, W, p.ld_out), dtype=torch.float32, device=x.device)
    planar = torch.empty((B, planar_classes, H * W), dtype=torch.float32, device=x.device) if planar_classes else None
    d = L.HeadsDesc()
    d.planar, d.planar_c = (planar.data_ptr() if planar is not None else None), planar_classes
    d.x, d.w1, d.scale1, d.shift1 = x.data_ptr(), p.w1.data_ptr(), p.scale1.data_ptr(), p.shift1.data_ptr()
    d.w2, d.bias2, d.out = p.w2.data_ptr(), p.bias2.data_ptr(), out.data_ptr()
    d.w1_32 = p.w1_32.data_ptr() if p.w1_32 is not None else None
    d.w2_32 = p.w2_32.data_ptr() if p.w2_32 is not None else None
    d.B, d.H, d.W, d.nbranch, d.K_pad, d.ld_out = B, H, W, len(p.c_out), p.K_pad, p.ld_out
    d.dtype = L.MFX_F16X2 if p.split else _dt(x.dtype)
    for i, (o, c) in enumerate(zip(p.ch_off, p.c_out)):
        d.ch_off[i], d.c_out[i] = o, c
        d.w2_scale[i] = p.w2_scale[i] if p.w2_scale is not None else 1.0
    L.check(L.load().mfx_heads_fused_act(ctypes.byref(d), p.act, _stream()), "mfx_heads_fused_act")
    return out, planar


@on_tensor_device
def edge_chain(x, edge_xy, p: PackedEdgeChain):
    _need_cuda(x, edge_xy)
    B, H, W, C = x.shape
    Lmax = edge_xy.shape[1]
    if edge_xy.dtype != torch.int32 or not edge_xy.is_contiguous() or not x.is_contiguous() or x.dtype != p.w_trunk.dtype:
        return None
    d = L.EdgeChainDesc()
    d.x, d.edge_xy = x.data_ptr(), edge_xy.data_ptr()
    d.w_trunk, d.scale_trunk, d.shift_trunk = p.w_trunk.data_ptr(), p.scale_trunk.data_ptr(), p.shift_trunk.data_ptr()
    d.w_conv, d.scale_conv, d.shift_conv = p.w_conv.data_ptr(), p.scale_conv.data_ptr(), p.shift_conv.data_ptr()
    d.w_out, d.bias_out = p.w_out.data_ptr(), p.bias_out.data_ptr()
    d.B, d.H, d.W, d.C, d.L, d.head_conv, d.ksize, d.relu, d.dtype = B, H, W, C, Lmax, 256, p.ksize, int(p.relu), _dt(x.dtype)
    lib = L.load()
    applies, run, name = (lib.mfx_edge_chain_applies, lib.mfx_edge_chain_act, "mfx_edge_chain_act") if p.ksize == 3 else \
        (lib.mfx_edge_chain_ks_applies, lib.mfx_edge_chain_ks, "mfx_edge_chain_ks")
    if not applies(ctypes.byref(d)):
        return None
    out = torch.empty((2, B, Lmax, 4), dtype=torch.float32, device=x.device)
    d.out = out.data_ptr()
    L.check(run(ctypes.byref(d), p.act_trunk, _stream()), name)
    return out


@on_tensor_device
def edge_scatter_add(out, ch_off, C, v, edge_xy, edge_len, planar=None):
    _need_cuda(out, v, edge_xy, edge_len, planar)
    B, H, W, ld = out.shape
    Lmax = edge_xy.shape[1]
    L.check(L.load().mfx_edge_scatter_add(_ptr(out), ld, ch_off, C, _ptr(v), v.shape[-1], _ptr(edge_xy), _ptr(edge_len),
                                          B, Lmax, H, W, _ptr(planar), _stream()), "mfx_edge_scatter_add")


@on_tensor_device
def decode_topk(hmap, ch_off, ncls, K, planar=None):
    _need_cuda(hmap, planar)
    B, H, W, ld = hmap.shape
    scores = torch.empty((B, ncls, K), dtype=torch.float32, device=hmap.device)
    index = torch.empty((B, ncls, K), dtype=torch.int32, device=hmap.device)
    if planar is not None:
        src, bs, cs, ps = planar.data_ptr(), ncls * H * W, H * W, 1
    else:
        src, bs, cs, ps = hmap.data_ptr() + 4 * ch_off, H * W * ld, 1, ld
    lib = L.load()
    ws = torch.empty(int(lib.mfx_decode_topk_workspace_bytes(ncls, B, K)), dtype=torch.uint8, device=hmap.device)
    L.check(lib.mfx_decode_topk(ctypes.c_void_p(src), bs, cs, ps, ncls, B, H, W, K, _ptr(scores), _ptr(index), _ptr(ws), ws.numel(),
                                _stream()), "mfx_decode_topk")
    return scores, index


@on_tensor_device
def decode_boxes(hmap, reg_off, scores, index, calib, pad, img_size, threshold, depth_mode="soft", cfg=None, return_unc=False, heads=None):
    _need_cuda(hmap, scores, index, calib, pad, img_size)
    if depth_mode not in L.DEPTH_MODES:
        raise ValueError("decode_boxes: output_depth %r is not one of %s" % (depth_mode, sorted(L.DEPTH_MODES)))
    if (return_unc or heads is not None) and cfg is None:
        raise ValueError("decode_boxes: return_unc / heads need a cfg (lib.decode_cfg)")
# ... 365 lines not shown
```

Before: 3345 images/s.

## Fuse stride-2/4 up-sample plus skip add into the LDS DCN kernel epilogue

Adds an UP template variant of the LDS DCN kernel. Its epilogue also reads the next level's projection, applies the transposed-conv up-sample taps and adds the freshly computed DCN output as the skip, writing the up-sampled sum in the same launch. The Python IDA-up path is reordered so the projections for the next stage are computed ahead and passed in as tails. This removes separate upsample_add launches and the re-read of the DCN output, but adds register pressure and extra global loads to the DCN epilogue. The rounding order is kept identical to the standalone kernel.

```diff
diff --git a/include/monoflex_hip.h b/include/monoflex_hip.h
--- a/include/monoflex_hip.h
+++ b/include/monoflex_hip.h
@@ -118,6 +118,15 @@
 int mfx_dcn_nhwc(const mfx_dcn_desc* d, void* stream);
 int mfx_dcn_fuses_offset_conv(const mfx_dcn_desc* d);
 int mfx_dcn_module_group(const mfx_conv_desc* off, const mfx_dcn_desc* dcn, int n, void* stream);
+
+typedef struct {
+    const void* p;
+    const float* w;
+    void* t;
+    int32_t f, Hp, Wp, C;
+} mfx_up_tail;
+int mfx_dcn_up_nhwc(const mfx_dcn_desc* d, const mfx_up_tail* ut, void* stream);
+int mfx_dcn_up_enabled(void);
 
 int mfx_dcn_sample_nhwc(const void* P, const float* offmask, const float* scale, const float* shift, void* y,
                         int B, int H, int W, int N, int ldy, int act, int dtype, void* stream);
diff --git a/monoflex_amd/csrc/dcn_lds.hip b/monoflex_amd/csrc/dcn_lds.hip
--- a/monoflex_amd/csrc/dcn_lds.hip
+++ b/monoflex_amd/csrc/dcn_lds.hip
@@ -3,11 +3,13 @@
 #include "internal.h"
 #include "igemm.h"
 #include "dcn_sample_math.h"
+#include "upsample_math.h"
 
 namespace mfx {
 
 struct DcnLGeom { int B, H, W, C, tiles_x, tiles_y, nslice, fsteps_pair, fsteps_far, cpt_far; };
 struct DcnLOffArgs { const u32x4* wfm; const float* shift; float* om_out; };
+struct DcnLUpArgs { const void* p; const float* w; void* t; int Hp, Wp; };
 
 typedef _Float16 lh2_t __attribute__((ext_vector_type(2)));
 typedef _Float16 lh8_t __attribute__((ext_vector_type(8)));
@@ -40,9 +42,10 @@
     static_assert(ZBYTES <= patch_bytes && (TBUF_OFF != GB_OFF || 4 * 2304 <= (NG + 64) * 4), "offset-conv scratch fits");
 };
 
-template <int R, int TR, typename TX, bool OF>
+template <int R, int TR, typename TX, bool OF, int UP = 0>
 __global__ __launch_bounds__(256, TR == 8 ? 3 : 2) void dcn_lds_kernel(const TX* __restrict__ x, const float* __restrict__ om, const u32x4* __restrict__ wpair,
-                                                        const u32x4* __restrict__ wfar, DcnLGeom g, EpiArgs ep, DcnLOffArgs oa) {
+                                                        const u32x4* __restrict__ wfar, DcnLGeom g, EpiArgs ep, DcnLOffArgs oa, DcnLUpArgs ua) {
+    static_assert(UP == 0 || ((UP == 2 || UP == 4) && TR == 16), "up-sample tail: stride 2 | 4 on 16-row tiles");
     using SM = DcnLSmem<R, TR>;
     constexpr int PW = SM::PW, PH = SM::PH, PB = SM::PB, FM = TR / 4, FN = 4, NPIX = SM::NPIX;
     constexpr int OWN = 4 / FM;
@@ -310,6 +313,42 @@
         if (sl < 3) LPROBE(8 + 2 * sl);
     }
 
+    constexpr int UN = UP > 0 ? 2 : 1;
+    u32x4 uxv[UN][2][2][2];
+    f32x4 uwv[UN][2][2][2];
+    int u_iw[2][2], u_kw[2]; bool u_vw[2][2];
+    const TX* up_p = nullptr;
+    auto up_load = [&](int i, int slot) {
+        const int yg = ty0 + wv * FM + i, ung = (lane & 7) * 8;
+#pragma unroll
+        for (int a = 0; a < 2; ++a) {
+            const ups::Tap th = ups::tap(yg, UP > 0 ? UP : 1, ua.Hp, a);
+#pragma unroll
+            for (int c = 0; c < 2; ++c) {
+                const float* wp = ua.w + (th.k * (2 * UP) + u_kw[c]) * 64 + ung;
+                uwv[slot][a][c][0] = *reinterpret_cast<const f32x4*>(wp);
+                uwv[slot][a][c][1] = *reinterpret_cast<const f32x4*>(wp + 4);
+#pragma unroll
+                for (int s = 0; s < 2; ++s) {
+                    const u32x4 v = *reinterpret_cast<const u32x4*>(up_p + ((size_t)th.ic * ua.Wp + u_iw[s][c]) * 64 + ung);
+                    uxv[slot][s][a][c] = (th.ok && u_vw[s][c]) ? v : u32x4{0u, 0u, 0u, 0u};
+                }
+            }
+        }
+    };
+    if constexpr (UP > 0) {
+        up_p = reinterpret_cast<const TX*>(ua.p) + (size_t)b * ua.Hp * ua.Wp * 64;
+#pragma unroll
+        for (int c = 0; c < 2; ++c) {
+#pragma unroll
+            for (int s = 0; s < 2; ++s) {
+                const ups::Tap tw = ups::tap(tx0 + s * 8 + (lane >> 3), UP, ua.Wp, c);
+                u_iw[s][c] = tw.ic; u_vw[s][c] = tw.ok; u_kw[c] = tw.k;
+            }
+        }
+        up_load(0, 0);
+    }
+
     __syncthreads();
     float sc[FN], sh[FN];
 #pragma unroll
@@ -376,12 +415,38 @@
     TX* y = reinterpret_cast<TX*>(ep.y);
 #pragma unroll
     for (int i = 0; i < FM; ++i) {
+        if constexpr (UP > 0) {
+            if (i + 1 < FM) up_load(i + 1, (i + 1) & 1);
+            __builtin_amdgcn_sched_barrier(0);
+        }
 #pragma unroll
         for (int j = 0; j < FN; ++j)
 #pragma unroll
             for (int r = 0; r < 4; ++r) stage[(kq * 4 + r) * LDS_ + j * 16 + xl] = acc[i][j][r] * sc[j] + sh[j];
         __builtin_amdgcn_wave_barrier();
         const int yg = ty0 + wv * FM + i;
+        if constexpr (UP > 0) {
+            static_assert(UP == 0 || GPR == 8, "up-sample tail: 64 output channels");
+            TX* t = reinterpret_cast<TX*>(ua.t);
+#pragma unroll
+            for (int s = 0; s < 2; ++s) {
+                const int px = s * 8 + (lane >> 3), ng = lane & 7;
+                const int gx = tx0 + px, gn = ng * 8;
+                if (yg < g.H && gx < g.W) {
+                    float v[8];
+#pragma unroll
+                    for (int e = 0; e < 8; e += 4) {
+                        const f32x4 q = *reinterpret_cast<const f32x4*>(stage + px * LDS_ + ng * 8 + e);
+                        v[e] = q[0]; v[e + 1] = q[1]; v[e + 2] = q[2]; v[e + 3] = q[3];
+                    }
+                    apply_act_chunk<8>(v, ep.act, gn);
+                    const u32x4 yv = ElemTraits<TX>::pack(v);
+                    const size_t pix = (size_t)(b * g.H + yg) * g.W + gx;
+                    *reinterpret_cast<u32x4*>(y + pix * ep.ldy + gn) = yv;
+                    *reinterpret_cast<u32x4*>(t + pix * 64 + gn) = ups::chunk<TX>(uxv[i & 1][s], uwv[i & 1], true, yv);
+                }
+            }
+        } else
         for (int it = lane; it < 16 * GPR; it += 64) {
             const int px = it / GPR, ng = it - px * GPR;
             const int gx = tx0 + px, gn = ng * 8;
@@ -687,7 +752,7 @@
     return g_opt_dcn_fuse_off && d->off_w_frag_f16 && d->off_shift && d->C == 64 && dcn_lds_auto(d);
 }
 
-template <int TR, typename TX, bool OF> static int launch_dcn_lds(const mfx_dcn_desc* d, hipStream_t st) {
+template <int TR, typename TX, bool OF, int UP = 0> static int launch_dcn_lds(const mfx_dcn_desc* d, hipStream_t st, const mfx_up_tail* ut = nullptr) {
     constexpr int R = 7;
     DcnLGeom g;
     g.B = d->B; g.H = d->H; g.W = d->W; g.C = d->C;
@@ -700,14 +765,16 @@
     constexpr int smem = DcnLSmem<R, TR>::bytes;
     static bool attr_done = false;
     if (!attr_done) {
-        MFX_HIP_CHECK(hipFuncSetAttribute(reinterpret_cast<const void*>(&dcn_lds_kernel<R, TR, TX, OF>), hipFuncAttributeMaxDynamicSharedMemorySize, smem));
+        MFX_HIP_CHECK(hipFuncSetAttribute(reinterpret_cast<const void*>(&dcn_lds_kernel<R, TR, TX, OF, UP>), hipFuncAttributeMaxDynamicSharedMemorySize, smem));
         attr_done = true;
     }
     DcnLOffArgs oa;
     oa.wfm = reinterpret_cast<const u32x4*>(d->off_w_frag_f16); oa.shift = d->off_shift; oa.om_out = d->offmask_out;
     if (!OF && !d->offmask) return mfx_fail(MFX_ERR_ARG, "dcn: offmask is NULL and this kernel does not compute the offsets itself");
-    hipLaunchKernelGGL((dcn_lds_kernel<R, TR, TX, OF>), dim3(tiles), dim3(256), smem, st, reinterpret_cast<const TX*>(d->x), d->offmask,
-                       reinterpret_cast<const u32x4*>(d->w_pair_f16), reinterpret_cast<const u32x4*>(d->w_frag_f16), g, ep, oa);
+    DcnLUpArgs ua;
+    ua.p = ut ? ut->p : nullptr; ua.w = ut ? ut->w : nullptr; ua.t = ut ? ut->t : nullptr; ua.Hp = ut ? ut->Hp : 0; ua.Wp = ut ? ut->Wp : 0;
+    hipLaunchKernelGGL((dcn_lds_kernel<R, TR, TX, OF, UP>), dim3(tiles), dim3(256), smem, st, reinterpret_cast<const TX*>(d->x), d->offmask,
+                       reinterpret_cast<const u32x4*>(d->w_pair_f16), reinterpret_cast<const u32x4*>(d->w_frag_f16), g, ep, oa, ua);
     MFX_HIP_CHECK(hipGetLastError());
     return MFX_OK;
 }
@@ -759,4 +826,28 @@
 
 }
 
+extern "C" int mfx_dcn_up_nhwc(const mfx_dcn_desc* d, const mfx_up_tail* ut, void* stream) {
+    using namespace mfx;
+    if (!d || !ut || !d->x || !d->w || !d->y || !ut->p || !ut->w || !ut->t) return mfx_fail(MFX_ERR_ARG, "dcn_up: null pointer");
+    if (!g_opt_dcn_up || (d->dtype != MFX_BF16 && d->dtype != MFX_F16) || d->nonsquare) return 1;
+    if (!dcn_lds_takes_16bit(d) || g_opt_dcn_lds_rows != 16) return 1;
+    if (d->Cout != 64 || d->ldy != 64 || d->B <= 0 || d->H <= 0 || d->W <= 0) return 1;
+    if ((ut->f != 2 && ut->f != 4) || ut->C != 64 || ut->Hp <= 0 || ut->Wp <= 0 || ut->Hp * ut->f != d->H || ut->Wp * ut->f != d->W) return 1;
+    if ((size_t)d->B * d->H * d->W * d->C * 2 >= ((size_t)1 << 32)) return 1;
+    const bool of = dcn_lds_fuses_offset_conv(d);
+    if (!of && !d->offmask) return 1;
+    hipStream_t st = reinterpret_cast<hipStream_t>(stream);
+    int rc;
+#define MFX_DCN_UP_LAUNCH(TX_, F_) (of ? launch_dcn_lds<16, TX_, true, F_>(d, st, ut) : launch_dcn_lds<16, TX_, false, F_>(d, st, ut))
+    if (d->dtype == MFX_F16) rc = ut->f == 2 ? MFX_DCN_UP_LAUNCH(half_t, 2) : MFX_DCN_UP_LAUNCH(half_t, 4);
+    else rc = ut->f == 2 ? MFX_DCN_UP_LAUNCH(bf16_t, 2) : MFX_DCN_UP_LAUNCH(bf16_t, 4);
+#undef MFX_DCN_UP_LAUNCH
+    if (rc != MFX_OK) return rc;
+    ++g_cnt_dcn_lds; ++g_cnt_dcn_lds_up;
+    if (of) ++g_cnt_dcn_lds_of;
+    return MFX_OK;
+}
+
+extern "C" int mfx_dcn_up_enabled(void) { return g_opt_dcn_up ? 1 : 0; }
+
 MFX_RANGE_FLAG_ACCESSOR(dcn_lds)
diff --git a/monoflex_amd/csrc/misc_kernels.hip b/monoflex_amd/csrc/misc_kernels.hip
--- a/monoflex_amd/csrc/misc_kernels.hip
+++ b/monoflex_amd/csrc/misc_kernels.hip
@@ -1,6 +1,7 @@
 #include "../../include/monoflex_hip.h"
 #include "common.h"
 #include "err.h"
+#include "upsample_math.h"
 
 namespace mfx {
 
@@ -38,7 +39,7 @@
                                     int B, int H, int W, int C, int f_rt) {
     constexpr int E = ElemTraits<T>::ELEMS;
     const int f = F > 0 ? F : f_rt;
-    const int Ho = H * f, Wo = W * f, CG = C / E, p_ = f / 2, k = 2 * f;
+    const int Ho = H * f, Wo = W * f, CG = C / E, k = 2 * f;
     const long total = (long)B * Ho * Wo * CG;
     for (long i = blockIdx.x * (long)blockDim.x + threadIdx.x; i < total; i += (long)gridDim.x * blockDim.x) {
         const int cg = (int)(i % CG);
@@ -46,50 +47,24 @@
         const int ow = (int)(p % Wo); p /= Wo;
         const int oh = (int)(p % Ho);
         const int b = (int)(p / Ho);
-        float acc[E];
-#pragma unroll
-        for (int e = 0; e < E; ++e) acc[e] = 0.f;
-        const int th = oh + p_, tw = ow + p_;
         const size_t o = ((size_t)(b * Ho + oh) * Wo + ow) * C + cg * E;
         u32x4 sv = {0u, 0u, 0u, 0u};
         if (skip) sv = *reinterpret_cast<const u32x4*>(skip + o);
         u32x4 xv[2][2]; f32x4 wv[2][2][E / 4];
 #pragma unroll
         for (int a = 0; a < 2; ++a) {
-            const int kh = th % f + a * f, dh = th - kh, ih = dh / f;
-            const bool vh = dh >= 0 && ih < H;
-            const int ihc = min(max(ih, 0), H - 1);
+            const ups::Tap th = ups::tap(oh, f, H, a);
 #pragma unroll
             for (int c2 = 0; c2 < 2; ++c2) {
-                const int kw = tw % f + c2 * f, dw = tw - kw, iw = dw / f;
-                const bool vw = dw >= 0 && iw < W;
-                const int iwc = min(max(iw, 0), W - 1);
-                const u32x4 v = *reinterpret_cast<const u32x4*>(x + ((size_t)(b * H + ihc) * W + iwc) * C + cg * E);
-                xv[a][c2] = (vh && vw) ? v : u32x4{0u, 0u, 0u, 0u};
-                const float* wp = w + (size_t)(kh * k + kw) * C + cg * E;
+                const ups::Tap tw = ups::tap(ow, f, W, c2);
+                const u32x4 v = *reinterpret_cast<const u32x4*>(x + ((size_t)(b * H + th.ic) * W + tw.ic) * C + cg * E);
+                xv[a][c2] = (th.ok && tw.ok) ? v : u32x4{0u, 0u, 0u, 0u};
+                const float* wp = w + (size_t)(th.k * k + tw.k) * C + cg * E;
 #pragma unroll
                 for (int e = 0; e < E; e += 4) wv[a][c2][e / 4] = *reinterpret_cast<const f32x4*>(wp + e);
             }
         }
-#pragma unroll
-        for (int a = 1; a >= 0; --a)
-#pragma unroll
-            for (int c2 = 1; c2 >= 0; --c2) {
-                float v[E];
-                ElemTraits<T>::unpack(xv[a][c2], v);
-#pragma unroll
-                for (int e = 0; e < E; e += 4) {
-                    const f32x4 w4 = wv[a][c2][e / 4];
-                    acc[e] += v[e] * w4[0]; acc[e + 1] += v[e + 1] * w4[1]; acc[e + 2] += v[e + 2] * w4[2]; acc[e + 3] += v[e + 3] * w4[3];
-                }
-            }
-        if (skip) {
-            float s[E];
-            ElemTraits<T>::unpack(sv, s);
-#pragma unroll
-            for (int e = 0; e < E; ++e) acc[e] += s[e];
-        }
-        *reinterpret_cast<u32x4*>(y + o) = ElemTraits<T>::pack(acc);
+        *reinterpret_cast<u32x4*>(y + o) = ups::chunk<T>(xv, wv, skip != nullptr, sv);
     }
 }
 
diff --git a/monoflex_amd/csrc/options.h b/monoflex_amd/csrc/options.h
--- a/monoflex_amd/csrc/options.h
+++ b/monoflex_amd/csrc/options.h
@@ -28,6 +28,8 @@
     X(dcn_fuse_off, 1, MFX_NOLO, MFX_NOHI, "1 = the LDS-patch kernel computes the offset/mask conv itself where the caller supplies its weights") \
     X(dcn_lds, 1, MFX_NOLO, MFX_NOHI, "0 = off, 1 = automatic (64 -> 64 on large 16-bit maps), 2 = wherever the kernel applies") \
     X(dcn_lds_rows, 16, MFX_NOLO, MFX_NOHI, "tile rows, 16 | 8 (three workgroups per CU; measured slower: 2.570 vs 2.551 ms per step, profiles/r06_dcn_lds.md)") \
+    X(dcn_up, 1, 0, 1, "1 = mfx_dcn_up_nhwc runs a 64 -> 64 LDS-kernel DCN node and the stride-2 / stride-4 up-sample + skip add that consumes it as one " \
+        "launch (bit-identical outputs), 0 = it refuses and the caller makes the two launches") \
     X(dcn_group, 1, 0, 1, "1 = mfx_dcn_module_group runs same-shape 16-bit gather-kernel DCN modules as one offset-conv launch and one gather launch " \
         "(bit-identical output), 0 = it refuses every group and the caller launches module by module") \
      \
@@ -88,6 +90,7 @@
      \
     X(dcn_lds, "launches of the fourth-generation DCN kernel (dcn_lds.hip) on 16-bit maps") \
     X(dcn_lds_of, "those of dcn_lds that computed the offset/mask conv themselves") \
+    X(dcn_lds_up, "those of dcn_lds that also wrote the up-sampled sum (mfx_dcn_up_nhwc)") \
     X(dcn_lds_split, "launches of dcn_lds.hip in split precision (not counted in dcn_lds)") \
     X(dcn_patch, "launches of the third-generation, LDS-patch DCN kernel (dcn_patch.hip)") \
     X(dcn_wave, "launches of the second-generation DCN kernel (dcn_wave.hip)") \
diff --git a/monoflex_amd/csrc/upsample_math.h b/monoflex_amd/csrc/upsample_math.h
--- /dev/null
+++ b/monoflex_amd/csrc/upsample_math.h
@@ -0,0 +1,57 @@
+#pragma once
+#include "common.h"
+
+namespace mfx {
+namespace ups {
+
+struct Tap { int k, ic; bool ok; };
+__device__ __forceinline__ Tap tap(int o, int f, int n, int a) {
+    const int t = o + f / 2;
+    Tap r;
+    r.k = t % f + a * f;
+    const int d = t - r.k, i = d / f;
+    r.ok = d >= 0 && i < n;
+    r.ic = min(max(i, 0), n - 1);
+    return r;
+}
+
+__device__ __forceinline__ float mul_then_add(float x, float w, float acc) {
+#pragma clang fp contract(off)
+    const float p = x * w;
+    return acc + p;
+}
+
+template <typename T>
+__device__ __forceinline__ u32x4 chunk(const u32x4 (&xv)[2][2], const f32x4 (&wv)[2][2][ElemTraits<T>::ELEMS / 4], bool has_skip, const u32x4& sv) {
+    constexpr int E = ElemTraits<T>::ELEMS;
+    float acc[E];
+#pragma unroll
+    for (int e = 0; e < E; ++e) acc[e] = 0.f;
+#pragma unroll
+    for (int a = 1; a >= 0; --a)
+#pragma unroll
+        for (int c = 1; c >= 0; --c) {
+            float v[E];
+            ElemTraits<T>::unpack(xv[a][c], v);
+#pragma unroll
+            for (int e = 0; e < E; e += 4) {
+                const f32x4 w4 = wv[a][c][e / 4];
+                acc[e] = fmaf(v[e], w4[0], acc[e]); acc[e + 1] = fmaf(v[e + 1], w4[1], acc[e + 1]);
+                if (E == 8 && e == 4) {
+                    acc[e + 2] = mul_then_add(v[e + 2], w4[2], acc[e + 2]); acc[e + 3] = mul_then_add(v[e + 3], w4[3], acc[e + 3]);
+                } else {
+                    acc[e + 2] = fmaf(v[e + 2], w4[2], acc[e + 2]); acc[e + 3] = fmaf(v[e + 3], w4[3], acc[e + 3]);
+                }
+            }
+        }
+    if (has_skip) {
+        float s[E];
+        ElemTraits<T>::unpack(sv, s);
+#pragma unroll
+        for (int e = 0; e < E; ++e) acc[e] = acc[e] + s[e];
+    }
+    return ElemTraits<T>::pack(acc);
+}
+
+}
+}
diff --git a/monoflex_amd/lib.py b/monoflex_amd/lib.py
--- a/monoflex_amd/lib.py
+++ b/monoflex_amd/lib.py
@@ -40,6 +40,10 @@
                 ("workspace", c_void_p), ("workspace_bytes", ctypes.c_int64),
                 ("off_w_frag_f16", c_void_p), ("off_shift", c_void_p), ("offmask_out", c_void_p),
                 ("nonsquare", c_int), ("stride_w", c_int), ("pad_w", c_int), ("dil_w", c_int), ("w_pair_f16", c_void_p)]
+
+
+class UpTailDesc(ctypes.Structure):
+    _fields_ = [("p", c_void_p), ("w", c_void_p), ("t", c_void_p), ("f", c_int), ("Hp", c_int), ("Wp", c_int), ("C", c_int)]
 
 
 class HeadsDesc(ctypes.Structure):
@@ -165,6 +169,8 @@
     "mfx_heads_fused_act": (_I, [ctypes.POINTER(HeadsDesc), _I, _P]),
     "mfx_dcn_fuses_offset_conv": (_I, [ctypes.POINTER(DcnDesc)]),
     "mfx_dcn_module_group": (_I, [ctypes.POINTER(ConvDesc), ctypes.POINTER(DcnDesc), _I, _P]),
+    "mfx_dcn_up_nhwc": (_I, [ctypes.POINTER(DcnDesc), ctypes.POINTER(UpTailDesc), _P]),
+    "mfx_dcn_up_enabled": (_I, []),
     "mfx_edge_scatter_add": (_I, [_P, _I, _I, _I, _P, _I, _P, _P, _I, _I, _I, _I, _P, _P]),
     "mfx_edge_chain": (_I, [ctypes.POINTER(EdgeChainDesc), _P]),
     "mfx_edge_chain_act": (_I, [ctypes.POINTER(EdgeChainDesc), _I, _P]),
diff --git a/monoflex_amd/model/backbone/DCNv2/dcn_v2.py b/monoflex_amd/model/backbone/DCNv2/dcn_v2.py
--- a/monoflex_amd/model/backbone/DCNv2/dcn_v2.py
+++ b/monoflex_amd/model/backbone/DCNv2/dcn_v2.py
@@ -105,12 +105,14 @@
             self._packs[key] = p
         return self._packs[key]
 
-    def forward_nhwc(self, x, bn=None, act=L.ACT_NONE, done=None):
+    def forward_nhwc(self, x, bn=None, act=L.ACT_NONE, done=None, up=None):
         if OFFSET_CONV_FP32[0] and x.dtype != torch.float32:
             offmask = ops.conv2d(x.float(), self.packed_offset(torch.float32), out_dtype=torch.float32)
         else:
             tag = ops.compute_tag(self, x.dtype)
-            return ops.dcn_module(x, self.packed_offset(tag), self.packed_main(tag, bn, act), done=done)[0]
+            if up is None:
+                return ops.dcn_module(x, self.packed_offset(tag), self.packed_main(tag, bn, act), done=done)[0]
+            return ops.dcn_module(x, self.packed_offset(tag), self.packed_main(tag, bn, act), done=done, up=up)[0]
         return ops.dcn(x, offmask, self.packed_main(ops.compute_tag(self, x.dtype), bn, act))
 
     def forward_nhwc_train(self, x):
diff --git a/monoflex_amd/model/backbone/dla_dcn.py b/monoflex_amd/model/backbone/dla_dcn.py
--- a/monoflex_amd/model/backbone/dla_dcn.py
+++ b/monoflex_amd/model/backbone/dla_dcn.py
@@ -250,10 +250,10 @@
         self.actf = nn.Sequential(nn.BatchNorm2d(cho, momentum=BN_MOMENTUM), nn.ReLU(inplace=True))
         self.conv = DCN(chi, cho, kernel_size=(3, 3), stride=1, padding=1, dilation=1, deformable_groups=1)
 
-    def forward(self, x, done=None):
+    def forward(self, x, done=None, up=None):
         if self.training:
             return AG.bn_act(self.conv.forward_nhwc_train(x), self.actf[0], L.ACT_RELU)
-        return self.conv.forward_nhwc(x, bn=self.actf[0], act=L.ACT_RELU, done=done)
+        return self.conv.forward_nhwc(x, bn=self.actf[0], act=L.ACT_RELU, done=done, up=up)
 
 
 class IDAUp(nn.Module):
@@ -267,23 +267,39 @@
             setattr(self, "up_" + str(i), up)
             setattr(self, "node_" + str(i), DeformConv(o, o))
 
-    def forward(self, layers, startp, endp):
+    def up_pack(self, k):
+        packs = self.__dict__.setdefault("_packs", {})
+        if k not in packs:
+            packs[k] = ops.pack_upsample(getattr(self, "up_" + str(k)).weight)
+        return packs[k]
+
+    def forward(self, layers, startp, endp, ahead=None, last_tail=None):
         packs = self.__dict__.setdefault("_packs", {})
         if not self.training and PARALLEL_PROJ[0] and endp - startp > 2 and layers[startp].is_cuda:
             return self._forward_parallel_proj(layers, startp, endp, packs)
         proj = {} if self.training else self._grouped_proj(layers, startp, endp)
+        t_done = None
+        if ahead and not self.training:
+            proj.update({k: v for k, v in ahead.items() if k != "t1"})
+            t_done = ahead.get("t1")
+        tails = not self.training and layers[startp].is_cuda and ops.dcn_up_enabled()
         for i in range(startp + 1, endp):
             k = i - startp
             up = getattr(self, "up_" + str(k))
-            if k not in packs:
-                packs[k] = ops.pack_upsample(up.weight)
+            self.up_pack(k)
             t = getattr(self, "proj_" + str(k))(layers[i], done=proj.pop(k)) if k in proj else getattr(self, "proj_" + str(k))(layers[i])
             if self.training:
                 t = AG.UpsampleAddFn.apply(t, up.weight, layers[i - 1], up.stride[0])
                 layers[i] = getattr(self, "node_" + str(k))(t)
                 continue
-            t = ops.upsample_add(t, packs[k], up.stride[0], skip=layers[i - 1])
-            layers[i] = getattr(self, "node_" + str(k))(t)
+            t = ops.upsample_add(t, packs[k], up.stride[0], skip=layers[i - 1], done=t_done)
+            tail = None
+            if tails and i + 1 < endp and k + 1 in proj:
+                tail = ops.UpTail(proj[k + 1][0], self.up_pack(k + 1), getattr(self, "up_" + str(k + 1)).stride[0])
+            elif tails and i + 1 == endp:
+                tail = last_tail
+            layers[i] = getattr(self, "node_" + str(k))(t) if tail is None else getattr(self, "node_" + str(k))(t, up=tail)
+            t_done = tail.out if tail is not None else None
 
 
 def _idaup_grouped_proj(self, layers, startp, endp):
@@ -358,10 +374,15 @@
             scales[j + 1:] = scales[j]
             in_channels[j + 1:] = [channels[j] for _ in channels[j + 1:]]
 
-    def forward(self, layers):
+    def forward(self, layers, before_last=None):
         out = [layers[-1]]
-        for i in range(len(layers) - self.startp - 1):
-            getattr(self, "ida_{}".format(i))(layers, len(layers) - i - 2, len(layers))
+        n = len(layers) - self.startp - 1
+        for i in range(n):
+            ida = getattr(self, "ida_{}".format(i))
+            if i == n - 1 and before_last is not None:
+                ida(layers, len(layers) - i - 2, len(layers), last_tail=before_last(out))
+            else:
+                ida(layers, len(layers) - i - 2, len(layers))
             out.insert(0, layers[-1])
         return out
 
@@ -386,12 +407,32 @@
         x = self.base(images, self.compute_dtype, cut) if cut is not None else self.base(images, self.compute_dtype)
         if cut is not None:
             x = cut("base", list(x))
-        x = self.dla_up(list(x))
+        ahead = {}
+        x = self.dla_up(list(x), before_last=lambda out: self._ida_up_ahead(out, ahead)) if self._tails_apply(x) else self.dla_up(list(x))
         y = [x[i] for i in range(self.last_level - self.first_level)]
         if cut is not None:
             y = cut("dla_up", y)
-        self.ida_up(y, 0, len(y))
+        if ahead:
+            ahead["t1"] = ahead.pop("tail").out
+            self.ida_up(y, 0, len(y), ahead=ahead)
+        else:
+            self.ida_up(y, 0, len(y))
         return y[-1]
+
+    def _tails_apply(self, levels):
+        from .DCNv2 import dcn_v2
+        top = levels[-1]
+        return (not self.training and self.last_level - self.first_level == 3 and top.is_cuda and not PARALLEL_PROJ[0]
+                and top.dtype in (torch.bfloat16, torch.float16) and not dcn_v2.OFFSET_CONV_FP32[0] and ops.dcn_up_enabled())
+
+    def _ida_up_ahead(self, out, ahead):
+        ida = self.ida_up
+        for k in (1, 2):
+            m, xk = getattr(ida, "proj_" + str(k)), out[k - 1]
+            tag = ops.compute_tag(m.conv, xk.dtype)
+            ahead[k] = ops.dcn_module_ahead(xk, m.conv.packed_offset(tag), m.conv.packed_main(tag, m.actf[0], L.ACT_RELU))
+        ahead["tail"] = ops.UpTail(ahead[1][0], ida.up_pack(1), ida.up_1.stride[0])
+        return ahead["tail"]
 
     def forward(self, images, cut=None):
         return self.forward_nhwc(images, cut).permute(0, 3, 1, 2)
diff --git a/monoflex_amd/ops.py b/monoflex_amd/ops.py
--- a/monoflex_amd/ops.py
+++ b/monoflex_amd/ops.py
@@ -156,13 +156,45 @@
     return d
 
 
-@on_tensor_device
-def dcn(x, offmask, p: PackedConv):
+class UpTail:
+    __slots__ = ("p", "taps", "f", "out")
+
+    def __init__(self, p, taps, f):
+        self.p, self.taps, self.f, self.out = p, taps, int(f), None
+
+
+def dcn_up_enabled():
+    return bool(L.load().mfx_dcn_up_enabled())
+
+
+def _dcn_up_launch(d, x, y, up):
+    up.out = None
+    pm, taps, f = up.p, up.taps, up.f
+    B, H, W, _ = y.shape
+    if not (pm.is_cuda and pm.dim() == 4 and pm.is_contiguous() and pm.dtype == x.dtype and pm.shape[0] == B and f >= 1
+            and taps.is_cuda and taps.dtype == torch.float32 and taps.is_contiguous() and tuple(taps.shape) == (4 * f * f, pm.shape[3])):
+        return False
+    t = torch.empty((B, H, W, pm.shape[3]), dtype=x.dtype, device=x.device)
+    ut = L.UpTailDesc()
+    ut.p, ut.w, ut.t = pm.data_ptr(), taps.data_ptr(), t.data_ptr()
+    ut.f, ut.Hp, ut.Wp, ut.C = f, pm.shape[1], pm.shape[2], pm.shape[3]
+    rc = L.load().mfx_dcn_up_nhwc(ctypes.byref(d), ctypes.byref(ut), _stream())
+    if rc < 0:
+        L.check(rc, "mfx_dcn_up_nhwc")
+    if rc == 0:
+        up.out = t
+    return rc == 0
+
+
+@on_tensor_device
+def dcn(x, offmask, p: PackedConv, up=None):
     _need_cuda(x, offmask)
     B = x.shape[0]
     Ho, Wo = offmask.shape[1], offmask.shape[2]
     y = torch.empty((B, Ho, Wo, p.Cout), dtype=x.dtype, device=x.device)
     d = _dcn_desc(x, offmask, p, y)
+    if up is not None and _dcn_up_launch(d, x, y, up):
+        return y
     if B * Ho * Wo * p.Cout_pad <= SPLITK_MAX_ELEMS:
         ws = _splitk_workspace(x.device)
         d.workspace, d.workspace_bytes = ws.data_ptr(), ws.numel() * 4
@@ -201,8 +233,10 @@
 
 
 @on_tensor_device
-def dcn_module(x, p_off: PackedConv, p: PackedConv, need_offmask=False, done=None):
+def dcn_module(x, p_off: PackedConv, p: PackedConv, need_offmask=False, done=None, up=None):
     _need_cuda(x)
+    if up is not None:
+        up.out = None
     if done is not None:
         return done
     B, H, W, C = x.shape
@@ -211,12 +245,16 @@
         om = torch.empty((B, H, W, 32), dtype=torch.float32, device=x.device) if need_offmask else None
         d = _dcn_desc(x, None, p, y, off=p_off, offmask_out=om)
         if d.off_w_frag_f16 and L.load().mfx_dcn_fuses_offset_conv(ctypes.byref(d)):
-            L.check(L.load().mfx_dcn_nhwc(ctypes.byref(d), _stream()), "mfx_dcn_nhwc")
+            if up is None or not _dcn_up_launch(d, x, y, up):
+                L.check(L.load().mfx_dcn_nhwc(ctypes.byref(d), _stream()), "mfx_dcn_nhwc")
             return y, om
     om = conv2d(x, p_off, out_dtype=torch.float32)
     if dcn_ps_applies(x, p):
         return dcn_ps(x, om, p), om
-    return dcn(x, om, p), om
+    return dcn(x, om, p, up=up), om
+
+
+dcn_module_ahead = dcn_module
 
 
 @on_tensor_device
@@ -270,8 +308,10 @@
 
 
 @on_tensor_device
-def upsample_add(x, w_taps, f, skip=None):
+def upsample_add(x, w_taps, f, skip=None, done=None):
     _need_cuda(x, w_taps, skip)
+    if done is not None:
+        return done
     B, H, W, C = x.shape
     y = torch.empty((B, H * f, W * f, C), dtype=x.dtype, device=x.device)
     L.check(L.load().mfx_upsample_add_nhwc(_ptr(x), _ptr(w_taps), _ptr(skip), _ptr(y), B, H, W, C, f, _dt(x.dtype), _stream()),
```

Measured after the change: 3377 images/s, median of 6. Within noise of the previous version (+0.9%).
